# Sabarna07-tech/Multimodal-RAG-for-Image-Text-Search

Measured on NVIDIA B200. Metric: queries/sec, exact top-10 over 10Mx512 bf16 (flat cosine scan + top-k), higher is better.
Workload: dtype bf16

## Files before the change

include/mmr_b200.h:

```cpp
#ifndef MMR_B200_H_
#define MMR_B200_H_

#include <stddef.h>
#include <stdint.h>

#ifdef __cplusplus
extern "C" {
#endif

#define MMR_ABI_VERSION 2

enum mmr_status {
  MMR_OK = 0,
  MMR_ERR_INVALID = 1,
  MMR_ERR_CUDA = 2,
  MMR_ERR_UNSUPPORTED = 3,
  MMR_ERR_WORKSPACE = 4
};

enum mmr_dtype {
  MMR_BF16 = 0,
  MMR_F32 = 1,
  MMR_F16 = 2
};

enum mmr_query_precision {
  MMR_QP_AUTO = 0,
  MMR_QP_F32 = 1,
  MMR_QP_RESCORE = 2
};

#define MMR_MAX_K 64

typedef struct mmr_index mmr_index;

int mmr_abi_version(void);
const char* mmr_last_error(void);
int mmr_set_option(const char* name, const char* value);
int mmr_get_option(const char* name);

int mmr_index_create(int device, int dim, int dtype, int64_t n_rows, const void* rows_dev,
                     const int64_t* seg_offsets_host, int32_t n_segments, int64_t row_base, mmr_index** out);
int mmr_index_destroy(mmr_index* index);
int mmr_index_set_query_precision(mmr_index* index, int mode);
int mmr_index_update(mmr_index* index, int64_t n_rows, const void* rows_dev, const int64_t* seg_offsets_host,
                     int32_t n_segments);

int mmr_convert_rows_f32(const float* src_dev, void* dst_dev, int dtype, int64_t n_rows, int dim, int normalize,
                         void* stream);
int mmr_load_rows_f32_host(int device, const float* src_host, void* dst_dev, int dtype, int64_t n_rows, int dim,
                           int normalize, void* stream);

int mmr_load_rows_f32_host_scatter(int device, const float* src_host, void* dst_dev, int dtype, int64_t n_rows, int dim,
                                   int normalize, const int64_t* dst_row_host, void* stream);
int mmr_hash_strings(const uint8_t* data, const int32_t* offsets, int64_t n, uint64_t* out);

size_t mmr_search_workspace_bytes(const mmr_index* index, int32_t B, int32_t k);
size_t mmr_search_ranges_workspace_bytes(const mmr_index* index, int32_t B, int32_t k, int64_t n_ranges);
int mmr_search(const mmr_index* index, const float* queries_dev, const int32_t* query_seg_host, int32_t B,
               int32_t k, float* out_scores_dev, int64_t* out_rows_dev, void* workspace_dev, size_t workspace_bytes,
               void* stream);
int mmr_search_ranges(const mmr_index* index, const float* queries_dev, int32_t B, int32_t k,
                      const int32_t* range_off_host, const int64_t* ranges_host, float* out_scores_dev,
                      int64_t* out_rows_dev, void* workspace_dev, size_t workspace_bytes, void* stream);
int mmr_search_host(mmr_index* index, const float* queries_host, const int32_t* query_seg_host, int32_t B,
                    int32_t k, float* out_scores_host, int64_t* out_rows_host, void* stream);

int mmr_merge_topk(const float* scores_dev, const int64_t* rows_dev, int32_t G, int32_t B, int32_t k,
                   float* out_scores_dev, int64_t* out_rows_dev, void* stream);
int mmr_merge_topk_strided(const float* scores_dev, const int64_t* rows_dev, int64_t score_shard_stride,
                           int64_t row_shard_stride, int32_t G, int32_t B, int32_t k, float* out_scores_dev,
                           int64_t* out_rows_dev, void* stream);

size_t mmr_exchange_buffer_bytes(int32_t G, int32_t B, int32_t k);
size_t mmr_search_exchange_workspace_bytes(const mmr_index* index, int32_t B, int32_t k);
int mmr_search_exchange(const mmr_index* index, const float* queries_dev, const int32_t* query_seg_host, int32_t B,
                        int32_t k, const uint64_t* peer_bufs_host, int32_t G, int32_t rank, uint32_t seq,
                        float* out_scores_dev, int64_t* out_rows_dev, void* workspace_dev, size_t workspace_bytes,
                        void* stream);

int mmr_search_exchange_host(mmr_index* index, const float* queries_host, const int32_t* query_seg_host, int32_t B,
                             int32_t k, const uint64_t* peer_bufs_host, int32_t G, int32_t rank, uint32_t seq,
                             float* out_scores_host, int64_t* out_rows_host, void* stream);

typedef struct mmr_multi mmr_multi;
int mmr_multi_create(mmr_index** shards, int32_t G, mmr_multi** out);
int mmr_multi_destroy(mmr_multi* multi);
int mmr_multi_search_host(mmr_multi* multi, const float* queries_host, int32_t B, int32_t k,
                          const int32_t* range_off_host, const int64_t* ranges_host, float* out_scores_host,
                          int64_t* out_rows_host);

int mmr_fuse(const float* text_scores_dev, const int64_t* text_rows_dev, int32_t kt, const float* img_scores_dev,
             const int64_t* img_rows_dev, int32_t ki, int32_t B, int32_t final_n, double tau,
             double* out_combined_dev, double* out_score_dev, int64_t* out_rows_dev, int8_t* out_modality_dev,
             uint8_t* out_low_conf_dev, void* stream);

int mmr_fuse_f64(const double* text_scores_dev, const int32_t* text_count_dev, const double* text_rerank_dev,
                 const int32_t* rerank_count_dev, const double* img_scores_dev, const int32_t* img_count_dev,
                 int32_t kt, int32_t ki, int32_t B, int32_t final_n, double tau, double* out_combined_dev,
                 int32_t* out_index_dev, uint8_t* out_low_conf_dev, void* stream);

enum mmr_encoder_kind { MMR_ENC_MINILM = 0, MMR_ENC_CLIP_TEXT = 1, MMR_ENC_CROSS = 2 };
typedef struct mmr_encoder_config {
  int32_t kind;
  int32_t vocab_size;
  int32_t hidden;
  int32_t layers;
  int32_t heads;
  int32_t intermediate;
  int32_t max_positions;
  int32_t type_vocab;
  int32_t proj_dim;
  int32_t eos_token_id;
  float ln_eps;
} mmr_encoder_config;
typedef struct mmr_encoder mmr_encoder;
int mmr_encoder_create(int device, const mmr_encoder_config* config, mmr_encoder** out);
int mmr_encoder_destroy(mmr_encoder* encoder);
int mmr_encoder_out_dim(const mmr_encoder* encoder);
int mmr_encoder_set_weight(mmr_encoder* encoder, const char* name, const float* data_dev, int64_t numel, void* stream);
int mmr_encoder_forward(mmr_encoder* encoder, const int32_t* input_ids_host, const int32_t* attention_mask_host,
                        const int32_t* token_type_host, int32_t B, int32_t S, float* out_dev, void* stream);

int mmr_debug_umma_scores(const mmr_index* index, const float* queries_dev, int32_t B, int64_t row_begin,
                          int64_t row_end, float* out_scores_dev, int64_t out_ld, void* workspace_dev,
                          size_t workspace_bytes, void* stream);

int64_t mmr_launch_count(void);
int mmr_device_sm_count(int device, int* out_sms);
int mmr_last_kernel(void);
int64_t mmr_rescore_reruns(void);

#ifdef __cplusplus
}
#endif
#endif
```

multimodal-rag-for-image-text-search_b200/_native.py:

```python
from __future__ import annotations

import ctypes as C
import os
from typing import Optional

HERE = os.path.dirname(os.path.abspath(__file__))
LIB_PATH = os.environ.get("MMR_LIB_PATH") or os.path.join(HERE, "libmmr_b200.so")

MMR_OK = 0
MMR_BF16, MMR_F32, MMR_F16 = 0, 1, 2
MMR_MAX_K = 64
ABI_VERSION = 2
MMR_QP_AUTO, MMR_QP_F32, MMR_QP_RESCORE = 0, 1, 2

_i32, _i64, _sz, _p, _f64 = C.c_int32, C.c_int64, C.c_size_t, C.c_void_p, C.c_double
SYMBOLS = [
    ("mmr_abi_version", C.c_int, []),
    ("mmr_last_error", C.c_char_p, []),
    ("mmr_set_option", C.c_int, [C.c_char_p, C.c_char_p]),
    ("mmr_get_option", C.c_int, [C.c_char_p]),
    ("mmr_index_set_query_precision", C.c_int, [_p, C.c_int]),
    ("mmr_search_ranges_workspace_bytes", _sz, [_p, _i32, _i32, _i64]),
    ("mmr_search_exchange_host", C.c_int, [_p, _p, _p, _i32, _i32, _p, _i32, _i32, C.c_uint32, _p, _p, _p]),
    ("mmr_index_create", C.c_int, [C.c_int, C.c_int, C.c_int, _i64, _p, _p, _i32, _i64, C.POINTER(_p)]),
    ("mmr_index_destroy", C.c_int, [_p]),
    ("mmr_index_update", C.c_int, [_p, _i64, _p, _p, _i32]),
    ("mmr_convert_rows_f32", C.c_int, [_p, _p, C.c_int, _i64, C.c_int, C.c_int, _p]),
    ("mmr_load_rows_f32_host", C.c_int, [C.c_int, _p, _p, C.c_int, _i64, C.c_int, C.c_int, _p]),
    ("mmr_load_rows_f32_host_scatter", C.c_int, [C.c_int, _p, _p, C.c_int, _i64, C.c_int, C.c_int, _p, _p]),
    ("mmr_hash_strings", C.c_int, [_p, _p, _i64, _p]),
    ("mmr_search_workspace_bytes", _sz, [_p, _i32, _i32]),
    ("mmr_search", C.c_int, [_p, _p, _p, _i32, _i32, _p, _p, _p, _sz, _p]),
    ("mmr_search_ranges", C.c_int, [_p, _p, _i32, _i32, _p, _p, _p, _p, _p, _sz, _p]),
    ("mmr_search_host", C.c_int, [_p, _p, _p, _i32, _i32, _p, _p, _p]),
    ("mmr_merge_topk", C.c_int, [_p, _p, _i32, _i32, _i32, _p, _p, _p]),
    ("mmr_merge_topk_strided", C.c_int, [_p, _p, _i64, _i64, _i32, _i32, _i32, _p, _p, _p]),
    ("mmr_exchange_buffer_bytes", _sz, [_i32, _i32, _i32]),
    ("mmr_search_exchange_workspace_bytes", _sz, [_p, _i32, _i32]),
    ("mmr_search_exchange", C.c_int, [_p, _p, _p, _i32, _i32, _p, _i32, _i32, C.c_uint32, _p, _p, _p, _sz, _p]),
    ("mmr_multi_create", C.c_int, [_p, _i32, C.POINTER(_p)]),
    ("mmr_multi_destroy", C.c_int, [_p]),
    ("mmr_multi_search_host", C.c_int, [_p, _p, _i32, _i32, _p, _p, _p, _p]),
    ("mmr_encoder_create", C.c_int, [C.c_int, _p, C.POINTER(_p)]),
    ("mmr_encoder_destroy", C.c_int, [_p]),
    ("mmr_encoder_out_dim", C.c_int, [_p]),
    ("mmr_encoder_set_weight", C.c_int, [_p, C.c_char_p, _p, _i64, _p]),
    ("mmr_encoder_forward", C.c_int, [_p, _p, _p, _p, _i32, _i32, _p, _p]),
    ("mmr_fuse", C.c_int, [_p, _p, _i32, _p, _p, _i32, _i32, _i32, _f64, _p, _p, _p, _p, _p, _p]),
    ("mmr_fuse_f64", C.c_int, [_p, _p, _p, _p, _p, _p, _i32, _i32, _i32, _i32, _f64, _p, _p, _p, _p]),
    ("mmr_debug_umma_scores", C.c_int, [_p, _p, _i32, _i64, _i64, _p, _i64, _p, _sz, _p]),
    ("mmr_launch_count", _i64, []),
    ("mmr_device_sm_count", C.c_int, [C.c_int, C.POINTER(C.c_int)]),
    ("mmr_last_kernel", C.c_int, []),
    ("mmr_rescore_reruns", _i64, []),
]


MMR_ENC_MINILM, MMR_ENC_CLIP_TEXT, MMR_ENC_CROSS = 0, 1, 2


class EncoderConfig(C.Structure):
    _fields_ = [("kind", _i32), ("vocab_size", _i32), ("hidden", _i32), ("layers", _i32), ("heads", _i32),
                ("intermediate", _i32), ("max_positions", _i32), ("type_vocab", _i32), ("proj_dim", _i32),
                ("eos_token_id", _i32), ("ln_eps", C.c_float)]


class NativeError(RuntimeError):
    """Raised for every non-zero status from the C ABI (propagates like the reference's search errors,
    app/storage/lancedb_store.py:103-123 has no try/except)."""


_lib: Optional[C.CDLL] = None


def lib() -> C.CDLL:
    global _lib
    if _lib is None:
        if not os.path.exists(LIB_PATH):
            raise NativeError(
                f"{LIB_PATH} is missing. Build it with `python -c 'import __graft_entry__ as g; g.build()'` "
                "(nvcc, sm_100a). This package has no CPU or eager fallback."
            )
        handle = C.CDLL(LIB_PATH)
        for name, res, args in SYMBOLS:
            fn = getattr(handle, name)
            fn.restype = res
            fn.argtypes = args
        if handle.mmr_abi_version() != ABI_VERSION:
            raise NativeError(f"ABI version mismatch: library {handle.mmr_abi_version()} != binding {ABI_VERSION}")
        _lib = handle
    return _lib


def check(status: int) -> None:
    if status != MMR_OK:
        msg = lib().mmr_last_error()
        raise NativeError(f"mmr status {status}: {msg.decode() if msg else '?'}")


def set_option(name: str, value) -> None:
    check(lib().mmr_set_option(name.encode(), None if value is None else str(value).encode()))


def get_option(name: str) -> int:
    return int(lib().mmr_get_option(name.encode()))
```

multimodal-rag-for-image-text-search_b200/csrc/aux_kernels.cuh:

```cuda
#pragma once
#include "common.cuh"
#include "topk.cuh"

namespace mmr {

template <typename E>
__device__ __forceinline__ E cast_elem(float x);
template <>
__device__ __forceinline__ __nv_bfloat16 cast_elem<__nv_bfloat16>(float x) { return __float2bfloat16_rn(x); }
template <>
__device__ __forceinline__ __half cast_elem<__half>(float x) { return __float2half_rn(x); }
template <>
__device__ __forceinline__ float cast_elem<float>(float x) { return x; }

template <typename E>
__global__ void convert_rows_kernel(const float* __restrict__ src, E* __restrict__ dst, int64_t n_rows, int dim,
                                    int normalize, const int64_t* __restrict__ dst_row = nullptr) {
  const int lane = threadIdx.x & 31;
  const int64_t warps = int64_t(gridDim.x) * (blockDim.x >> 5);
  for (int64_t row = int64_t(blockIdx.x) * (blockDim.x >> 5) + (threadIdx.x >> 5); row < n_rows; row += warps) {
    const int64_t drow = dst_row ? dst_row[row] : row;
    if (drow < 0) continue;
    const float* s = src + row * dim;
    E* d = dst + drow * dim;
    float inv = 1.f;
    bool scale = false;
    if (normalize) {
      float ss = 0.f;
      for (int i = lane; i < dim; i += 32) {
        const float x = s[i];
        ss = fmaf(x, x, ss);
      }
      ss = warp_allreduce_sum(ss);
      const float nrm = sqrtf(ss);
      scale = nrm > 0.f;
      inv = nrm;
    }
    for (int i = lane; i < dim; i += 32) {
      const float x = s[i];
      d[i] = cast_elem<E>(scale ? x / inv : x);
    }
  }
}

template <int KPL>
__global__ void merge_shards_kernel(const float* __restrict__ scores, const int64_t* __restrict__ rows,
                                    int64_t score_stride, int64_t row_stride, int G, int B, int k,
                                    float* __restrict__ out_scores, int64_t* __restrict__ out_rows) {
  const int lane = threadIdx.x & 31;
  const int qi = blockIdx.x * (blockDim.x >> 5) + (threadIdx.x >> 5);
  if (qi >= B) return;
  WarpTopK<KPL> m;
  m.clear();
  uint64_t thr = 0ull;
  const int per = k;
  const int total = G * per;
  for (int i0 = 0; i0 < total; i0 += 32) {
    const int i = i0 + lane;
    bool valid = i < total;
    uint64_t key = 0ull;
    if (valid) {
      const int g = i / per, j = i % per;
      const size_t o = size_t(qi) * k + j;
      const int64_t r = rows[size_t(g) * row_stride + o];
      valid = r >= 0;
      if (valid) key = make_key(scores[size_t(g) * score_stride + o], uint32_t(r));
    }
    thr = m.offer_batch(key, valid, thr, k, lane);
  }
#pragma unroll
  for (int j = 0; j < KPL; ++j) {
    const int pos = j * 32 + lane;
    if (pos < k) {
      const uint64_t key = m.key[j];
      out_scores[size_t(qi) * k + pos] = key ? key_score(key) : -INFINITY;
      out_rows[size_t(qi) * k + pos] = key ? int64_t(key_row(key)) : int64_t(-1);
    }
  }
}

constexpr int MMR_XCHG_MAX_PEERS = 16;
constexpr int MMR_XCHG_HEADER = 256;

struct PeerPtrs {
  uint64_t slot[MMR_XCHG_MAX_PEERS];
  uint64_t flag[MMR_XCHG_MAX_PEERS];
};

__global__ void push_wire_kernel(const uint8_t* __restrict__ wire, uint32_t wire_bytes, const PeerPtrs peers, uint32_t seq) {
  const int g = blockIdx.x;
  const uint64_t* peer_slot = peers.slot;
  const uint64_t* peer_flag = peers.flag;
  const uint4* src = reinterpret_cast<const uint4*>(wire);
  uint4* dst = reinterpret_cast<uint4*>(peer_slot[g]);
  const uint32_t n16 = wire_bytes / 16;
  for (uint32_t i = threadIdx.x; i < n16; i += blockDim.x) dst[i] = src[i];
  for (uint32_t i = n16 * 16 + threadIdx.x; i < wire_bytes; i += blockDim.x)
    reinterpret_cast<uint8_t*>(peer_slot[g])[i] = wire[i];
  __threadfence_system();
  __syncthreads();
  if (threadIdx.x == 0) asm volatile("st.release.sys.global.u32 [%0], %1;" ::"l"(peer_flag[g]), "r"(seq) : "memory");
}

__device__ __forceinline__ uint32_t ld_acquire_sys_u32(const uint32_t* p) {
  uint32_t v;
  asm volatile("ld.acquire.sys.global.u32 %0, [%1];" : "=r"(v) : "l"(p) : "memory");
  return v;
}
__device__ __forceinline__ uint64_t globaltimer_ns() {
  uint64_t t;
  asm volatile("mov.u64 %0, %%globaltimer;" : "=l"(t));
  return t;
}

template <int KPL>
__device__ __forceinline__ void merge_wait_body(const uint8_t* __restrict__ xbuf, int parity, uint32_t seq,
                                                uint32_t wire_bytes, uint32_t score_bytes, int G, int B, int k,
                                                float* __restrict__ out_scores, int64_t* __restrict__ out_rows,
                                                uint64_t timeout_ns, int qi, int lane);

template <int KPL>
__global__ void merge_wait_kernel(const uint8_t* __restrict__ xbuf, int parity, uint32_t seq, uint32_t wire_bytes,
                                  uint32_t score_bytes, int G, int B, int k, float* __restrict__ out_scores,
                                  int64_t* __restrict__ out_rows, uint64_t timeout_ns, uint32_t* done_flag,
                                  uint32_t done_seq) {
  const int lane = threadIdx.x & 31;
  const int qi = blockIdx.x * (blockDim.x >> 5) + (threadIdx.x >> 5);
  asm volatile("griddepcontrol.launch_dependents;" ::: "memory");
  if (done_flag != nullptr) {
    merge_wait_body<KPL>(xbuf, parity, seq, wire_bytes, score_bytes, G, B, k, out_scores, out_rows, timeout_ns, qi, lane);
    __threadfence_system();
    __syncthreads();
    if (threadIdx.x == 0) asm volatile("st.release.sys.global.u32 [%0], %1;" ::"l"(done_flag), "r"(done_seq) : "memory");
    return;
  }
  merge_wait_body<KPL>(xbuf, parity, seq, wire_bytes, score_bytes, G, B, k, out_scores, out_rows, timeout_ns, qi, lane);
}

template <int KPL>
__device__ __forceinline__ void merge_wait_body(const uint8_t* __restrict__ xbuf, int parity, uint32_t seq,
                                                uint32_t wire_bytes, uint32_t score_bytes, int G, int B, int k,
                                                float* __restrict__ out_scores, int64_t* __restrict__ out_rows,
                                                uint64_t timeout_ns, int qi, int lane) {
  if (qi >= B) return;
  const uint32_t* flags = reinterpret_cast<const uint32_t*>(xbuf) + parity * MMR_XCHG_MAX_PEERS;
  bool ok = true;
  if (lane < G) {
    const uint64_t t0 = globaltimer_ns();
    while (ld_acquire_sys_u32(flags + lane) < seq) {
      if (globaltimer_ns() - t0 > timeout_ns) {
        ok = false;
        break;
      }
    }
  }
  ok = __all_sync(0xffffffffu, ok);
  if (!ok) {
    if (lane == 0) {
      out_rows[size_t(qi) * k] = -2;
      out_scores[size_t(qi) * k] = -INFINITY;
    }
    return;
  }
  const uint8_t* slots = xbuf + MMR_XCHG_HEADER + size_t(parity) * G * wire_bytes;
  WarpTopK<KPL> m;
  m.clear();
  uint64_t thr = 0ull;
  const int total = G * k;
  for (int i0 = 0; i0 < total; i0 += 32) {
    const int i = i0 + lane;
    bool valid = i < total;
    uint64_t key = 0ull;
    if (valid) {
      const int g = i / k, j = i % k;
      const uint8_t* slot = slots + size_t(g) * wire_bytes;
      const size_t o = size_t(qi) * k + j;
      const long long r = __ldcg(reinterpret_cast<const long long*>(slot + score_bytes) + o);
      valid = r >= 0;
      if (valid) key = make_key(__ldcg(reinterpret_cast<const float*>(slot) + o), uint32_t(r));
    }
    thr = m.offer_batch(key, valid, thr, k, lane);
  }
#pragma unroll
  for (int j = 0; j < KPL; ++j) {
    const int pos = j * 32 + lane;
    if (pos < k) {
      const uint64_t key = m.key[j];
      out_scores[size_t(qi) * k + pos] = key ? key_score(key) : -INFINITY;
      out_rows[size_t(qi) * k + pos] = key ? int64_t(key_row(key)) : int64_t(-1);
    }
  }
}

__device__ __forceinline__ float np_pairwise_sum_f32(const float* a, int n) {
  if (n < 8) {
    float res = 0.f;
    for (int i = 0; i < n; ++i) res = __fadd_rn(res, a[i]);
    return res;
  }
  float r[8];
#pragma unroll
  for (int j = 0; j < 8; ++j) r[j] = a[j];
  int i = 8;
  const int lim = n - (n % 8);
  for (; i < lim; i += 8) {
#pragma unroll
    for (int j = 0; j < 8; ++j) r[j] = __fadd_rn(r[j], a[i + j]);
  }
  float res = __fadd_rn(__fadd_rn(__fadd_rn(r[0], r[1]), __fadd_rn(r[2], r[3])),
                        __fadd_rn(__fadd_rn(r[4], r[5]), __fadd_rn(r[6], r[7])));
  for (; i < n; ++i) res = __fadd_rn(res, a[i]);
  return res;
}

constexpr int FUSE_MAXK = 64;

__device__ __forceinline__ void np_z_scores(const float* cos, int n, double* v, double* z) {
  float arr[FUSE_MAXK], sq[FUSE_MAXK];
  for (int i = 0; i < n; ++i) {
    const float d = __fsub_rn(1.0f, cos[i]);
    v[i] = __dsub_rn(1.0, double(d));
    arr[i] = __double2float_rn(v[i]);
  }
  const float fn = float(n);
  const float mean = __fdiv_rn(np_pairwise_sum_f32(arr, n), fn);
  for (int i = 0; i < n; ++i) {
    const float x = __fsub_rn(arr[i], mean);
    sq[i] = __fmul_rn(x, x);
  }
  const float var = __fdiv_rn(np_pairwise_sum_f32(sq, n), fn);
  const float sd = __fsqrt_rn(var);
  if (sd == 0.f) {
    for (int i = 0; i < n; ++i) z[i] = 0.0;
  } else {
    const double dm = double(mean), ds = double(sd);
    for (int i = 0; i < n; ++i) z[i] = __ddiv_rn(__dsub_rn(v[i], dm), ds);
  }
}

__device__ __forceinline__ void np_z_scores_f64(const double* v, int n, double* z) {
  float arr[FUSE_MAXK], sq[FUSE_MAXK];
  for (int i = 0; i < n; ++i) arr[i] = __double2float_rn(v[i]);
  const float fn = float(n);
  const float mean = __fdiv_rn(np_pairwise_sum_f32(arr, n), fn);
  for (int i = 0; i < n; ++i) {
    const float x = __fsub_rn(arr[i], mean);
    sq[i] = __fmul_rn(x, x);
  }
  const float sd = __fsqrt_rn(__fdiv_rn(np_pairwise_sum_f32(sq, n), fn));
  if (sd == 0.f) {
    for (int i = 0; i < n; ++i) z[i] = 0.0;
  } else {
    const double dm = double(mean), ds = double(sd);
    for (int i = 0; i < n; ++i) z[i] = __ddiv_rn(__dsub_rn(v[i], dm), ds);
  }
}

__device__ __forceinline__ void stable_desc_order(const double* key, int n, int* idx) {
  for (int i = 0; i < n; ++i) {
    int j = i;
    while (j > 0 && key[idx[j - 1]] < key[i]) {
      idx[j] = idx[j - 1];
      --j;
    }
    idx[j] = i;
  }
}

__global__ void fuse_full_kernel(const double* __restrict__ text_scores, const int32_t* __restrict__ text_count,
                                 const double* __restrict__ rerank, const int32_t* __restrict__ rr_count,
                                 const double* __restrict__ img_scores, const int32_t* __restrict__ img_count, int kt,
                                 int ki, int B, int final_n, double tau, double* __restrict__ out_combined,
                                 int32_t* __restrict__ out_index, uint8_t* __restrict__ out_low_conf) {
  const int b = blockIdx.x * blockDim.x + threadIdx.x;
  if (b >= B) return;
  const int nt = text_count ? min(text_count[b], kt) : 0;
  const int ni = img_count ? min(img_count[b], ki) : 0;
  const int nr = (rr_count && rerank) ? min(rr_count[b], nt) : 0;
  double key[FUSE_MAXK], v[FUSE_MAXK], z[FUSE_MAXK], rr[FUSE_MAXK], zr[FUSE_MAXK];
  double comb[2 * FUSE_MAXK];
  int order[FUSE_MAXK], src[2 * FUSE_MAXK], fin[2 * FUSE_MAXK];
  for (int j = 0; j < nt; ++j) {
    key[j] = j < nr ? rerank[size_t(b) * kt + j] : text_scores[size_t(b) * kt + j];
    order[j] = j;
  }
  if (nr > 0) stable_desc_order(key, nt, order);
  int nrr = 0;
  for (int j = 0; j < nt; ++j) {
    v[j] = text_scores[size_t(b) * kt + order[j]];
    if (order[j] < nr) rr[nrr++] = rerank[size_t(b) * kt + order[j]];
  }
  if (nt) np_z_scores_f64(v, nt, z);
  if (nrr) np_z_scores_f64(rr, nrr, zr);
  for (int j = 0; j < nt; ++j) {
    comb[j] = j < nrr ? __ddiv_rn(__dadd_rn(__dadd_rn(0.0, z[j]), zr[j]), 2.0) : __ddiv_rn(__dadd_rn(0.0, z[j]), 1.0);
    src[j] = order[j];
  }
  if (ni) {
    for (int j = 0; j < ni; ++j) v[j] = img_scores[size_t(b) * ki + j];
    np_z_scores_f64(v, ni, z);
    for (int j = 0; j < ni; ++j) {
      comb[nt + j] = z[j];
      src[nt + j] = kt + j;
    }
  }
  const int n = nt + ni;
  stable_desc_order(comb, n, fin);
  for (int o = 0; o < final_n; ++o) {
    const size_t oo = size_t(b) * final_n + o;
    out_combined[oo] = o < n ? comb[fin[o]] : 0.0;
    out_index[oo] = o < n ? src[fin[o]] : -1;
  }
  out_low_conf[b] = (n == 0 || final_n <= 0) ? 1 : (comb[fin[0]] < tau ? 1 : 0);
}

__global__ void fuse_kernel(const float* __restrict__ text_scores, const int64_t* __restrict__ text_rows, int kt,
                            const float* __restrict__ img_scores, const int64_t* __restrict__ img_rows, int ki, int B,
                            int final_n, double tau, double* __restrict__ out_combined,
                            double* __restrict__ out_score, int64_t* __restrict__ out_rows,
                            int8_t* __restrict__ out_modality, uint8_t* __restrict__ out_low_conf) {
  const int qi = blockIdx.x * blockDim.x + threadIdx.x;
  if (qi >= B) return;
  double v[2 * FUSE_MAXK], z[2 * FUSE_MAXK];
  int nt = 0, ni = 0;
  if (text_rows) {
    while (nt < kt && text_rows[size_t(qi) * kt + nt] >= 0) ++nt;
  }
  if (img_rows) {
    while (ni < ki && img_rows[size_t(qi) * ki + ni] >= 0) ++ni;
  }
  if (nt) np_z_scores(text_scores + size_t(qi) * kt, nt, v, z);
  if (ni) np_z_scores(img_scores + size_t(qi) * ki, ni, v + nt, z + nt);
  const int n = nt + ni;
  unsigned long long taken_lo = 0ull, taken_hi = 0ull;
  double best0 = 0.0;
  for (int o = 0; o < final_n; ++o) {
    int bi = -1;
    double bz = 0.0;
    for (int i = 0; i < n; ++i) {
      const bool taken = i < 64 ? ((taken_lo >> i) & 1ull) : ((taken_hi >> (i - 64)) & 1ull);
      if (taken) continue;
      if (bi < 0 || z[i] > bz) {
        bi = i;
        bz = z[i];
      }
    }
    const size_t oo = size_t(qi) * final_n + o;
// ... 20 lines not shown
```

multimodal-rag-for-image-text-search_b200/csrc/common.cuh:

```cuda
#pragma once
#include <cuda_runtime.h>
#include <cuda_bf16.h>
#include <cuda_fp16.h>
#include <stdint.h>

namespace mmr {

__host__ __device__ __forceinline__ uint32_t f32_orderable(float f) {
#ifdef __CUDA_ARCH__
  uint32_t u = __float_as_uint(f + 0.0f);
#else
  f = f + 0.0f;
  uint32_t u;
  memcpy(&u, &f, 4);
#endif
  return u ^ ((u >> 31) ? 0xFFFFFFFFu : 0x80000000u);
}
__host__ __device__ __forceinline__ float f32_from_orderable(uint32_t o) {
  uint32_t u = o ^ ((o >> 31) ? 0x80000000u : 0xFFFFFFFFu);
#ifdef __CUDA_ARCH__
  return __uint_as_float(u);
#else
  float f;
  memcpy(&f, &u, 4);
  return f;
#endif
}
__host__ __device__ __forceinline__ uint64_t make_key(float score, uint32_t row) {
  return (uint64_t(f32_orderable(score)) << 32) | uint64_t(0xFFFFFFFFu - row);
}
__host__ __device__ __forceinline__ float key_score(uint64_t key) { return f32_from_orderable(uint32_t(key >> 32)); }
__host__ __device__ __forceinline__ uint32_t key_row(uint64_t key) { return 0xFFFFFFFFu - uint32_t(key); }

struct Options {
  int pdl = 0;
  int umma_mode = 0;
  int umma_pair = 1;
  int umma_noprobe = 0;
  int umma_stages = 0;
  int force_family = 0;
  int umma_lockstep = 0;
  int umma_fused_probe = 0;
  int umma_skip_epi = 0;
  int enc_fuse_ln = 0;
  int enc_att_mma = 1;
  int enc_gemm_smem_kb = 100;
  int enc_narrow_tiles = 1;
  int inline_query = 1;
  int mailbox = 0;
};
inline Options& options() {
  static Options o;
  return o;
}

#ifdef __CUDACC__
__device__ __forceinline__ uint64_t shfl_u64(uint64_t v, int src) {
  uint32_t lo = __shfl_sync(0xffffffffu, uint32_t(v), src);
  uint32_t hi = __shfl_sync(0xffffffffu, uint32_t(v >> 32), src);
  return (uint64_t(hi) << 32) | lo;
}
__device__ __forceinline__ uint64_t shfl_u64_xor(uint64_t v, int mask) {
  uint32_t lo = __shfl_xor_sync(0xffffffffu, uint32_t(v), mask);
  uint32_t hi = __shfl_xor_sync(0xffffffffu, uint32_t(v >> 32), mask);
  return (uint64_t(hi) << 32) | lo;
}
__device__ __forceinline__ uint64_t shfl_up_u64(uint64_t v, int d) {
  uint32_t lo = __shfl_up_sync(0xffffffffu, uint32_t(v), d);
  uint32_t hi = __shfl_up_sync(0xffffffffu, uint32_t(v >> 32), d);
  return (uint64_t(hi) << 32) | lo;
}
__device__ __forceinline__ float warp_allreduce_sum(float v) {
#pragma unroll
  for (int o = 16; o > 0; o >>= 1) v += __shfl_xor_sync(0xffffffffu, v, o);
  return v;
}

__device__ __forceinline__ uint32_t smem_u32(const void* p) { return uint32_t(__cvta_generic_to_shared(p)); }

__device__ __forceinline__ void mbar_init(uint32_t bar, uint32_t count) {
  asm volatile("mbarrier.init.shared::cta.b64 [%0], %1;" ::"r"(bar), "r"(count) : "memory");
}
__device__ __forceinline__ void fence_mbar_init() {
  asm volatile("fence.mbarrier_init.release.cluster;" ::: "memory");
}
__device__ __forceinline__ void fence_proxy_async() {
  asm volatile("fence.proxy.async.shared::cta;" ::: "memory");
}
__device__ __forceinline__ void mbar_arrive_expect_tx(uint32_t bar, uint32_t bytes) {
  asm volatile("mbarrier.arrive.expect_tx.shared::cta.b64 _, [%0], %1;" ::"r"(bar), "r"(bytes) : "memory");
}
__device__ __forceinline__ void mbar_arrive(uint32_t bar) {
  asm volatile("mbarrier.arrive.shared::cta.b64 _, [%0];" ::"r"(bar) : "memory");
}
__device__ __forceinline__ bool mbar_try_wait(uint32_t bar, uint32_t parity) {
  uint32_t ok;
  asm volatile(
      "{\n\t.reg .pred p;\n\t"
      "mbarrier.try_wait.parity.shared::cta.b64 p, [%1], %2;\n\t"
      "selp.b32 %0, 1, 0, p;\n\t}"
      : "=r"(ok)
      : "r"(bar), "r"(parity)
      : "memory");
  return ok != 0;
}
__device__ __forceinline__ void mbar_wait(uint32_t bar, uint32_t parity) {
  while (!mbar_try_wait(bar, parity)) {
  }
}
__device__ __forceinline__ void bulk_g2s(uint32_t dst_smem, const void* src, uint32_t bytes, uint32_t bar) {
  asm volatile("cp.async.bulk.shared::cluster.global.mbarrier::complete_tx::bytes [%0], [%1], %2, [%3];" ::"r"(dst_smem),
               "l"(src), "r"(bytes), "r"(bar)
               : "memory");
}
__device__ __forceinline__ uint64_t l2_policy_evict_first() {
  uint64_t pol;
  asm volatile("createpolicy.fractional.L2::evict_first.b64 %0, 1.0;" : "=l"(pol));
  return pol;
}
__device__ __forceinline__ uint64_t l2_policy_evict_last() {
  uint64_t pol;
  asm volatile("createpolicy.fractional.L2::evict_last.b64 %0, 1.0;" : "=l"(pol));
  return pol;
}
__device__ __forceinline__ void bulk_g2s_hint(uint32_t dst_smem, const void* src, uint32_t bytes, uint32_t bar,
                                              uint64_t policy) {
  asm volatile(
      "cp.async.bulk.shared::cluster.global.mbarrier::complete_tx::bytes.L2::cache_hint [%0], [%1], %2, [%3], %4;" ::"r"(
          dst_smem),
      "l"(src), "r"(bytes), "r"(bar), "l"(policy)
      : "memory");
}

__device__ __forceinline__ void lds_v4(uint32_t addr, uint32_t (&r)[4]) {
  asm volatile("ld.shared.v4.u32 {%0,%1,%2,%3}, [%4];" : "=r"(r[0]), "=r"(r[1]), "=r"(r[2]), "=r"(r[3]) : "r"(addr));
}
__device__ __forceinline__ void lds_v2(uint32_t addr, uint32_t (&r)[2]) {
  asm volatile("ld.shared.v2.u32 {%0,%1}, [%2];" : "=r"(r[0]), "=r"(r[1]) : "r"(addr));
}
__device__ __forceinline__ void pdl_chain_prologue() {
  asm volatile("griddepcontrol.launch_dependents;" ::: "memory");
  asm volatile("griddepcontrol.wait;" ::: "memory");
}

__device__ __forceinline__ void pdl_launch_dependents() { asm volatile("griddepcontrol.launch_dependents;" ::: "memory"); }
__device__ __forceinline__ void pdl_wait_prior_grid() { asm volatile("griddepcontrol.wait;" ::: "memory"); }

template <typename... KArgs, typename... Args>
inline cudaError_t launch_pdl(void (*kernel)(KArgs...), dim3 grid, dim3 block, size_t smem, cudaStream_t st, Args&&... args) {
  cudaLaunchConfig_t cfg = {};
  cfg.gridDim = grid;
  cfg.blockDim = block;
  cfg.dynamicSmemBytes = smem;
  cfg.stream = st;
  cudaLaunchAttribute attr[1];
  attr[0].id = cudaLaunchAttributeProgrammaticStreamSerialization;
  attr[0].val.programmaticStreamSerializationAllowed = 1;
  cfg.attrs = attr;
  cfg.numAttrs = 1;
  return cudaLaunchKernelEx(&cfg, kernel, static_cast<KArgs>(args)...);
}
#endif

}
```

multimodal-rag-for-image-text-search_b200/csrc/mmr_b200.cu:

```cuda
#include "abi_common.h"

#include <algorithm>
#include <atomic>
#include <chrono>
#include <cstdarg>
#include <cstdio>
#include <cstdlib>
#include <cstring>
#include <condition_variable>
#include <map>
#include <mutex>
#include <string>
#include <thread>
#include <vector>
#if defined(__x86_64__)
#include <immintrin.h>
#endif

#include "aux_kernels.cuh"
#include "common.cuh"
#include "scan_stream.cuh"
#ifdef MMR_WITH_UMMA
#include "scan_umma2.cuh"
#endif

using namespace mmr;

thread_local std::string mmr_g_err;
std::atomic<int64_t> mmr_g_launches{0};
static thread_local int g_last_kernel = 0;
static std::atomic<int64_t> g_rescore_reruns{0};
#define g_err mmr_g_err
#define g_launches mmr_g_launches
#define fail mmr_fail

int mmr_fail(int code, const char* fmt, ...) {
  char buf[512];
  va_list ap;
  va_start(ap, fmt);
  vsnprintf(buf, sizeof(buf), fmt, ap);
  va_end(ap);
  mmr_g_err = buf;
  return code;
}

struct mmr_index {
  int device = 0;
  int dim = 0;
  int dtype = MMR_BF16;
  int64_t n_rows = 0;
  const void* rows = nullptr;
  int64_t row_base = 0;
  std::vector<int64_t> seg;
  int sm_count = 0;
  int query_precision = MMR_QP_AUTO;
  mutable uint8_t* h_flags = nullptr;
  mutable int flags_cap = 0;
  std::mutex host_mu;
  float* h_q = nullptr;
  float* d_q = nullptr;
  uint8_t* h_box = nullptr;
  uint8_t* d_box = nullptr;
  uint32_t box_seq = 0;
  void* d_ws = nullptr;
  size_t ws_bytes = 0;
  int cap_b = 0, cap_k = 0;
#ifdef MMR_WITH_UMMA
  mutable UmmaIndexState umma;
  mutable Umma2IndexState umma2;
#endif
};

static int elem_bytes(int dtype) { return dtype == MMR_F32 ? 4 : 2; }

static int set_segments(mmr_index* ix, const int64_t* seg, int32_t nseg) {
  ix->seg.clear();
  if (seg == nullptr || nseg <= 0) {
    ix->seg = {0, ix->n_rows};
    return MMR_OK;
  }
  ix->seg.assign(seg, seg + nseg + 1);
  if (ix->seg.front() < 0 || ix->seg.back() > ix->n_rows) return fail(MMR_ERR_INVALID, "segment offsets out of range");
  for (int i = 0; i < nseg; ++i)
    if (ix->seg[i] > ix->seg[i + 1]) return fail(MMR_ERR_INVALID, "segment offsets must be ascending");
  return MMR_OK;
}

static int* option_slot(const char* name) {
  Options& o = options();
  if (!name) return nullptr;
  if (!strcmp(name, "MMR_PDL")) return &o.pdl;
  if (!strcmp(name, "MMR_UMMA_MODE")) return &o.umma_mode;
  if (!strcmp(name, "MMR_UMMA_PAIR")) return &o.umma_pair;
  if (!strcmp(name, "MMR_UMMA_NOPROBE")) return &o.umma_noprobe;
  if (!strcmp(name, "MMR_FORCE_FAMILY")) return &o.force_family;
  if (!strcmp(name, "MMR_UMMA_LOCKSTEP")) return &o.umma_lockstep;
  if (!strcmp(name, "MMR_UMMA_SKIP_EPI")) return &o.umma_skip_epi;
  if (!strcmp(name, "MMR_UMMA_FUSED_PROBE")) return &o.umma_fused_probe;
  if (!strcmp(name, "MMR_UMMA_STAGES")) return &o.umma_stages;
  if (!strcmp(name, "MMR_ENC_FUSE_LN")) return &o.enc_fuse_ln;
  if (!strcmp(name, "MMR_ENC_ATT_MMA")) return &o.enc_att_mma;
  if (!strcmp(name, "MMR_ENC_GEMM_SMEM_KB")) return &o.enc_gemm_smem_kb;
  if (!strcmp(name, "MMR_ENC_NARROW_TILES")) return &o.enc_narrow_tiles;
  if (!strcmp(name, "MMR_INLINE_QUERY")) return &o.inline_query;
  if (!strcmp(name, "MMR_MAILBOX")) return &o.mailbox;
  return nullptr;
}
static int parse_option(const char* name, const char* v, int dflt) {
  if (!v || !v[0]) return dflt;
  if (!strcmp(name, "MMR_UMMA_MODE")) return v[0] == 's' ? 1 : (v[0] == 't' ? 2 : 0);
  return atoi(v);
}
static const char* kOptionNames[] = {"MMR_PDL", "MMR_UMMA_MODE", "MMR_UMMA_PAIR", "MMR_UMMA_NOPROBE", "MMR_FORCE_FAMILY",
                                     "MMR_UMMA_LOCKSTEP", "MMR_INLINE_QUERY", "MMR_MAILBOX", "MMR_UMMA_SKIP_EPI", "MMR_UMMA_FUSED_PROBE", "MMR_ENC_FUSE_LN", "MMR_ENC_ATT_MMA", "MMR_ENC_GEMM_SMEM_KB", "MMR_UMMA_STAGES", "MMR_ENC_NARROW_TILES"};
namespace {
struct OptionsFromEnv {
  OptionsFromEnv() {
    for (const char* name : kOptionNames) {
      int* slot = option_slot(name);
      *slot = parse_option(name, getenv(name), *slot);
    }
  }
} g_options_from_env;
}

extern "C" int mmr_set_option(const char* name, const char* value) {
  int* slot = option_slot(name);
  if (!slot) return fail(MMR_ERR_INVALID, "unknown option %s", name ? name : "(null)");
  Options defaults;
  Options& o = options();
  const int dflt = *(reinterpret_cast<int*>(&defaults) + (slot - reinterpret_cast<int*>(&o)));
  *slot = parse_option(name, value, dflt);
  return MMR_OK;
}
extern "C" int mmr_get_option(const char* name) {
  int* slot = option_slot(name);
  return slot ? *slot : -1;
}

extern "C" int mmr_abi_version(void) { return MMR_ABI_VERSION; }
extern "C" const char* mmr_last_error(void) { return g_err.c_str(); }
extern "C" int64_t mmr_launch_count(void) { return g_launches.load(); }
extern "C" int mmr_last_kernel(void) { return g_last_kernel; }
extern "C" int64_t mmr_rescore_reruns(void) { return g_rescore_reruns.load(); }

extern "C" int mmr_device_sm_count(int device, int* out_sms) {
  if (!out_sms) return fail(MMR_ERR_INVALID, "out_sms is NULL");
  CUDA_TRY(cudaDeviceGetAttribute(out_sms, cudaDevAttrMultiProcessorCount, device));
  return MMR_OK;
}

extern "C" int mmr_index_create(int device, int dim, int dtype, int64_t n_rows, const void* rows_dev,
                                const int64_t* seg_offsets_host, int32_t n_segments, int64_t row_base,
                                mmr_index** out) {
  if (!out) return fail(MMR_ERR_INVALID, "out is NULL");
  *out = nullptr;
  if (dtype != MMR_BF16 && dtype != MMR_F32 && dtype != MMR_F16) return fail(MMR_ERR_INVALID, "unknown dtype %d", dtype);
  if (dim <= 0 || n_rows < 0) return fail(MMR_ERR_INVALID, "bad shape [%lld, %d]", (long long)n_rows, dim);
  if (n_rows >= (int64_t(1) << 32)) return fail(MMR_ERR_UNSUPPORTED, "at most 2^32-1 rows per resident index");
  if (n_rows > 0 && rows_dev == nullptr) return fail(MMR_ERR_INVALID, "rows_dev is NULL");
  if ((reinterpret_cast<uintptr_t>(rows_dev) & 15) != 0) return fail(MMR_ERR_INVALID, "rows_dev must be 16-byte aligned");
  if (dim != 384 && dim != 512)
    return fail(MMR_ERR_UNSUPPORTED, "dim %d: kernels are built for 384 (MiniLM) and 512 (CLIP)", dim);
  int major = 0, minor = 0, sms = 0;
  CUDA_TRY(cudaDeviceGetAttribute(&major, cudaDevAttrComputeCapabilityMajor, device));
  CUDA_TRY(cudaDeviceGetAttribute(&minor, cudaDevAttrComputeCapabilityMinor, device));
  CUDA_TRY(cudaDeviceGetAttribute(&sms, cudaDevAttrMultiProcessorCount, device));
  if (major != 10) return fail(MMR_ERR_CUDA, "device %d is sm_%d%d; this library is sm_100a only", device, major, minor);
  mmr_index* ix = new mmr_index();
  ix->device = device;
  ix->dim = dim;
  ix->dtype = dtype;
  ix->n_rows = n_rows;
  ix->rows = rows_dev;
  ix->row_base = row_base;
  ix->sm_count = sms;
  int rc = set_segments(ix, seg_offsets_host, n_segments);
  if (rc != MMR_OK) {
    delete ix;
    return rc;
  }
  *out = ix;
  return MMR_OK;
}

extern "C" int mmr_index_update(mmr_index* ix, int64_t n_rows, const void* rows_dev, const int64_t* seg, int32_t nseg) {
  if (!ix) return fail(MMR_ERR_INVALID, "index is NULL");
  if (n_rows < 0 || n_rows >= (int64_t(1) << 32)) return fail(MMR_ERR_INVALID, "bad n_rows");
  if (n_rows > 0 && rows_dev == nullptr) return fail(MMR_ERR_INVALID, "rows_dev is NULL");
  if ((reinterpret_cast<uintptr_t>(rows_dev) & 15) != 0) return fail(MMR_ERR_INVALID, "rows_dev must be 16-byte aligned");
  ix->n_rows = n_rows;
  ix->rows = rows_dev;
#ifdef MMR_WITH_UMMA
  ix->umma.valid = false;
  ix->umma2.valid = false;
#endif
  return set_segments(ix, seg, nseg);
}

static void free_staging(mmr_index* ix) {
  if (ix->h_flags) cudaFreeHost(ix->h_flags);
  ix->h_flags = nullptr;
  ix->flags_cap = 0;
  if (ix->h_q) cudaFreeHost(ix->h_q);
  if (ix->h_box) cudaFreeHost(ix->h_box);
  if (ix->d_q) cudaFree(ix->d_q);
  if (ix->d_ws) cudaFree(ix->d_ws);
  ix->h_q = ix->d_q = nullptr;
  ix->h_box = ix->d_box = nullptr;
  ix->d_ws = nullptr;
  ix->cap_b = ix->cap_k = 0;
}

extern "C" int mmr_index_destroy(mmr_index* ix) {
  if (!ix) return MMR_OK;
  cudaSetDevice(ix->device);
  free_staging(ix);
  delete ix;
  return MMR_OK;
}

extern "C" int mmr_index_set_query_precision(mmr_index* ix, int mode) {
  if (!ix) return fail(MMR_ERR_INVALID, "index is NULL");
  if (mode != MMR_QP_AUTO && mode != MMR_QP_F32 && mode != MMR_QP_RESCORE)
    return fail(MMR_ERR_INVALID, "unknown query precision %d", mode);
  ix->query_precision = mode;
  return MMR_OK;
}

template <typename E>
static int launch_convert(const float* src, void* dst, int64_t n, int dim, int normalize, cudaStream_t st,
                          const int64_t* dst_row = nullptr) {
  if (n == 0) return MMR_OK;
  const int threads = 256;
  const int64_t blocks = std::min<int64_t>((n + 7) / 8, 148 * 16);
  convert_rows_kernel<E><<<(unsigned)blocks, threads, 0, st>>>(src, reinterpret_cast<E*>(dst), n, dim, normalize, dst_row);
  g_launches++;
  CUDA_TRY(cudaGetLastError());
  return MMR_OK;
}

static int convert_dispatch(const float* src_dev, void* dst_dev, int dtype, int64_t n_rows, int dim, int normalize,
                            cudaStream_t st, const int64_t* dst_row_dev) {
  switch (dtype) {
    case MMR_BF16: return launch_convert<__nv_bfloat16>(src_dev, dst_dev, n_rows, dim, normalize, st, dst_row_dev);
    case MMR_F16: return launch_convert<__half>(src_dev, dst_dev, n_rows, dim, normalize, st, dst_row_dev);
    case MMR_F32: return launch_convert<float>(src_dev, dst_dev, n_rows, dim, normalize, st, dst_row_dev);
  }
  return fail(MMR_ERR_INVALID, "unknown dtype %d", dtype);
}

extern "C" int mmr_convert_rows_f32(const float* src_dev, void* dst_dev, int dtype, int64_t n_rows, int dim,
                                    int normalize, void* stream) {
  if (n_rows < 0 || dim <= 0) return fail(MMR_ERR_INVALID, "bad shape");
  if (n_rows > 0 && (!src_dev || !dst_dev)) return fail(MMR_ERR_INVALID, "NULL buffer");
  return convert_dispatch(src_dev, dst_dev, dtype, n_rows, dim, normalize, static_cast<cudaStream_t>(stream), nullptr);
}

static void parallel_memcpy(void* dst, const void* src, size_t bytes, int threads) {
  if (threads <= 1 || bytes < (size_t(4) << 20)) {
    memcpy(dst, src, bytes);
    return;
  }
  std::vector<std::thread> pool;
  const size_t per = (bytes / threads + 4095) / 4096 * 4096;
  for (int t = 0; t < threads; ++t) {
    const size_t o = size_t(t) * per;
    if (o >= bytes) break;
    const size_t len = std::min(per, bytes - o);
    pool.emplace_back([=]() { memcpy(static_cast<uint8_t*>(dst) + o, static_cast<const uint8_t*>(src) + o, len); });
  }
  for (auto& th : pool) th.join();
}

extern "C" int mmr_load_rows_f32_host_scatter(int device, const float* src_host, void* dst_dev, int dtype, int64_t n_rows,
                                              int dim, int normalize, const int64_t* dst_row_host, void* stream) {
  if (n_rows < 0 || dim <= 0) return fail(MMR_ERR_INVALID, "bad shape");
  if (n_rows == 0) return MMR_OK;
  if (!src_host || !dst_dev) return fail(MMR_ERR_INVALID, "NULL buffer");
  if (dtype != MMR_BF16 && dtype != MMR_F32 && dtype != MMR_F16) return fail(MMR_ERR_INVALID, "unknown dtype %d", dtype);
  CUDA_TRY(cudaSetDevice(device));
  cudaStream_t st = static_cast<cudaStream_t>(stream);
  const int64_t chunk_rows = std::max<int64_t>(1, (int64_t(64) << 20) / (int64_t(dim) * 4));
  const size_t chunk_bytes = size_t(chunk_rows) * dim * 4;
  const size_t map_bytes = dst_row_host ? size_t(chunk_rows) * 8 : 0;
  uint8_t* h[2] = {nullptr, nullptr};
  uint8_t* d[2] = {nullptr, nullptr};
  cudaEvent_t done[2] = {nullptr, nullptr};
  int rc = MMR_OK;
  auto cleanup = [&]() {
    for (int i = 0; i < 2; ++i) {
      if (h[i]) cudaFreeHost(h[i]);
      if (d[i]) cudaFree(d[i]);
      if (done[i]) cudaEventDestroy(done[i]);
    }
  };
  for (int i = 0; i < 2; ++i) {
    if (cudaMallocHost(&h[i], chunk_bytes + map_bytes) != cudaSuccess ||
        cudaMalloc(&d[i], chunk_bytes + map_bytes) != cudaSuccess ||
        cudaEventCreateWithFlags(&done[i], cudaEventDisableTiming) != cudaSuccess) {
      cleanup();
      return fail(MMR_ERR_CUDA, "staging allocation of %zu bytes failed", chunk_bytes + map_bytes);
    }
  }
  const int threads = int(std::min<unsigned>(8u, std::max(1u, std::thread::hardware_concurrency() / 2)));
  int slot = 0;
  for (int64_t r0 = 0; r0 < n_rows && rc == MMR_OK; r0 += chunk_rows, slot ^= 1) {
    const int64_t nr = std::min(chunk_rows, n_rows - r0);
    const size_t bytes = size_t(nr) * dim * 4;
    cudaEventSynchronize(done[slot]);
    parallel_memcpy(h[slot], src_host + r0 * dim, bytes, threads);
    if (dst_row_host) memcpy(h[slot] + chunk_bytes, dst_row_host + r0, size_t(nr) * 8);
    const size_t copy_bytes = dst_row_host ? chunk_bytes + size_t(nr) * 8 : bytes;
    if (cudaMemcpyAsync(d[slot], h[slot], copy_bytes, cudaMemcpyHostToDevice, st) != cudaSuccess) {
      rc = fail(MMR_ERR_CUDA, "H2D copy failed");
      break;
    }
    const int64_t* map_dev = dst_row_host ? reinterpret_cast<const int64_t*>(d[slot] + chunk_bytes) : nullptr;
    const int eb = elem_bytes(dtype);
    void* dst = dst_row_host ? dst_dev : static_cast<void*>(static_cast<uint8_t*>(dst_dev) + size_t(r0) * dim * eb);
    rc = convert_dispatch(reinterpret_cast<const float*>(d[slot]), dst, dtype, nr, dim, normalize, st, map_dev);
    cudaEventRecord(done[slot], st);
  }
  cudaStreamSynchronize(st);
  cleanup();
  return rc;
}

extern "C" int mmr_load_rows_f32_host(int device, const float* src_host, void* dst_dev, int dtype, int64_t n_rows,
                                      int dim, int normalize, void* stream) {
  return mmr_load_rows_f32_host_scatter(device, src_host, dst_dev, dtype, n_rows, dim, normalize, nullptr, stream);
}

extern "C" int mmr_hash_strings(const uint8_t* data, const int32_t* offsets, int64_t n, uint64_t* out) {
  if (n < 0 || (n > 0 && (!offsets || !out))) return fail(MMR_ERR_INVALID, "bad arguments");
  for (int64_t i = 0; i < n; ++i) {
    const uint8_t* p = data + offsets[i];
    const int32_t len = offsets[i + 1] - offsets[i];
    uint64_t h = 0xcbf29ce484222325ull ^ (uint64_t(uint32_t(len)) * 0x9E3779B97F4A7C15ull);
    int32_t j = 0;
    for (; j + 8 <= len; j += 8) {
      uint64_t w;
      memcpy(&w, p + j, 8);
      h = (h ^ w) * 0x100000001b3ull;
      h ^= h >> 29;
    }
    uint64_t tail = 0;
    if (j < len) memcpy(&tail, p + j, size_t(len - j));
    h = (h ^ tail) * 0x100000001b3ull;
    h ^= h >> 32;
    h *= 0xff51afd7ed558ccdull;
    h ^= h >> 33;
    h *= 0xc4ceb9fe1a85ec53ull;
    h ^= h >> 33;
    out[i] = h;
  }
  return MMR_OK;
}

template <typename E, int D, int NQ, int KPL>
static int launch_stream_t(const StreamParams& p, int grid, cudaStream_t st) {
  using C = StreamCfg<E, D, NQ, KPL>;
  static bool attr_set[64] = {};
  int dev = 0;
  cudaGetDevice(&dev);
  if (dev >= 0 && dev < 64 && !attr_set[dev]) {
    CUDA_TRY(cudaFuncSetAttribute(scan_stream_kernel<E, D, NQ, KPL>, cudaFuncAttributeMaxDynamicSharedMemorySize,
                                  C::SMEM_BYTES));
    attr_set[dev] = true;
  }
  cudaLaunchConfig_t cfg = {};
  cfg.gridDim = dim3(grid);
  cfg.blockDim = dim3(C::THREADS);
  cfg.dynamicSmemBytes = C::SMEM_BYTES;
  cfg.stream = st;
  cudaLaunchAttribute attr[1];
  attr[0].id = cudaLaunchAttributeProgrammaticStreamSerialization;
  attr[0].val.programmaticStreamSerializationAllowed = (p.items == nullptr && options().pdl) ? 1 : 0;
  cfg.attrs = attr;
  cfg.numAttrs = 1;
  CUDA_TRY(cudaLaunchKernelEx(&cfg, scan_stream_kernel<E, D, NQ, KPL>, p));
  g_launches++;
  return MMR_OK;
}

template <typename E, int D>
static int launch_stream_ed(const StreamParams& p, int nq_pad, int kpl, int grid, cudaStream_t st) {
#define MMR_CASE(NQ_, KPL_) \
  if (nq_pad == NQ_ && kpl == KPL_) return launch_stream_t<E, D, NQ_, KPL_>(p, grid, st);
  MMR_CASE(1, 1) MMR_CASE(1, 2) MMR_CASE(2, 1) MMR_CASE(2, 2) MMR_CASE(4, 1) MMR_CASE(4, 2)
  if constexpr (sizeof(E) == 4) {
    MMR_CASE(8, 1) MMR_CASE(8, 2)
  }
#undef MMR_CASE
  return fail(MMR_ERR_UNSUPPORTED, "no stream kernel for nq=%d kpl=%d", nq_pad, kpl);
}

static int launch_stream(const mmr_index* ix, const StreamParams& p, int nq_pad, int kpl, int grid, cudaStream_t st) {
  const int key = ix->dtype * 1000 + ix->dim;
  switch (key) {
    case MMR_BF16 * 1000 + 512: return launch_stream_ed<__nv_bfloat16, 512>(p, nq_pad, kpl, grid, st);
    case MMR_BF16 * 1000 + 384: return launch_stream_ed<__nv_bfloat16, 384>(p, nq_pad, kpl, grid, st);
    case MMR_F16 * 1000 + 512: return launch_stream_ed<__half, 512>(p, nq_pad, kpl, grid, st);
    case MMR_F16 * 1000 + 384: return launch_stream_ed<__half, 384>(p, nq_pad, kpl, grid, st);
    case MMR_F32 * 1000 + 512: return launch_stream_ed<float, 512>(p, nq_pad, kpl, grid, st);
    case MMR_F32 * 1000 + 384: return launch_stream_ed<float, 384>(p, nq_pad, kpl, grid, st);
  }
  return fail(MMR_ERR_UNSUPPORTED, "no stream kernel for dtype %d dim %d", ix->dtype, ix->dim);
}

static constexpr size_t WS_CTRL = 256;
#ifndef MMR_VARLEN_ITEMS_PER_CTA
#define MMR_VARLEN_ITEMS_PER_CTA 8
#endif
static constexpr int VARLEN_ITEMS_PER_CTA = MMR_VARLEN_ITEMS_PER_CTA;
static constexpr int RANGES_PER_QUERY_BUDGET = 8;

static size_t align_up(size_t v, size_t a) { return (v + a - 1) / a * a; }

static int64_t varlen_item_cap(const mmr_index* ix, int64_t n_ranges) {
  return int64_t(ix->sm_count) * VARLEN_ITEMS_PER_CTA + n_ranges + 64;
}

static size_t rescore_extra_bytes(int B) {
  return align_up(size_t(B) * MMR_MAX_K * 4, 256) + align_up(size_t(B) * MMR_MAX_K * 8, 256) + align_up(size_t(B) * 4, 256) +
         align_up(size_t(B), 256);
}
static size_t k2_slice_bytes(const mmr_index* ix, int B) {
#ifdef MMR_WITH_UMMA
  return umma_workspace_bytes(ix->sm_count, ix->dim, B, MMR_MAX_K) + rescore_extra_bytes(B);
#else
  return 0;
#endif
}

static size_t workspace_bytes_for(const mmr_index* ix, int32_t B, int32_t k, int64_t n_ranges) {
  if (!ix || B <= 0 || k <= 0) return 0;
  const size_t kk = size_t(std::min<int32_t>(k, MMR_MAX_K));
  const size_t uniform = size_t(ix->sm_count) * 8 * kk * 8;
  const size_t items = size_t(varlen_item_cap(ix, n_ranges));
  const size_t varlen = align_up(items * K1_ITEM_NQ * kk * 8, 256) + align_up(items * sizeof(ScanItem), 256) +
                        align_up(size_t(B) * sizeof(QuerySlot), 256);
  size_t total = WS_CTRL + align_up(std::max(uniform, varlen), 256);
  total += k2_slice_bytes(ix, B);
  return total;
}

extern "C" size_t mmr_search_workspace_bytes(const mmr_index* ix, int32_t B, int32_t k) {
  return workspace_bytes_for(ix, B, k, int64_t(RANGES_PER_QUERY_BUDGET) * std::max(B, 0));
}
extern "C" size_t mmr_search_ranges_workspace_bytes(const mmr_index* ix, int32_t B, int32_t k, int64_t n_ranges) {
  return workspace_bytes_for(ix, B, k, std::max<int64_t>(n_ranges, 0));
}

struct ExchangeInfo {
  int n_peers = 0;
  uint32_t seq = 0;
  uint32_t wire_score_bytes = 0;
  uint64_t slot[MMR_MAX_PEERS] = {};
  uint64_t flag[MMR_MAX_PEERS] = {};
};

struct QuerySrc {
  const float* dev = nullptr;
  const float* host = nullptr;
};
struct Completion {
  uint32_t* flag_dev = nullptr;
  uint32_t seq = 0;
  bool armed = false;
};

static int k1_group(const mmr_index* ix) { return ix->dtype == MMR_F32 ? 8 : 4; }

static bool can_inline(const mmr_index* ix, int B) {
  return options().inline_query && B * ix->dim <= K1_INLINE_FLOATS && B <= 2;
}

static int search_uniform_stream(const mmr_index* ix, QuerySrc q, int B, int k, uint32_t r0, uint32_t r1,
                                 float* out_s, int64_t* out_r, uint8_t* ws, cudaStream_t st,
                                 const ExchangeInfo* xi = nullptr, Completion* done = nullptr) {
  const int kpl = k <= 32 ? 1 : 2;
  const int R = MMR_K1_ROWS;
  const int64_t nchunks = (int64_t(r1) - r0 + R - 1) / R;
  int grid = int(std::min<int64_t>(ix->sm_count, std::max<int64_t>(1, (nchunks + K1_NW - 1) / K1_NW)));
  const int group = k1_group(ix);
  if (q.dev == nullptr && !(q.host && can_inline(ix, B))) return fail(MMR_ERR_INVALID, "queries must be device-resident for this batch size");
  for (int q0 = 0; q0 < B; q0 += group) {
    const int nq = std::min(group, B - q0);
    const int nq_pad = nq <= 2 ? nq : (nq <= 4 ? 4 : 8);
    StreamParams p;
    memset(&p, 0, offsetof(StreamParams, qinline));
    p.rows = ix->rows;
    p.queries = q.dev;
    if (q.dev == nullptr) memcpy(p.qinline, q.host, size_t(B) * ix->dim * sizeof(float));
    p.q_first = q0;
    p.nq = nq;
    p.k = k;
    p.row_begin = r0;
    p.row_end = r1;
    p.partial = reinterpret_cast<uint64_t*>(ws + WS_CTRL);
    p.ticket = reinterpret_cast<unsigned int*>(ws);
    p.out_scores = out_s;
    p.out_rows = out_r;
    p.row_base = ix->row_base;
    if (B <= group) {
      if (xi) {
        p.n_peers = xi->n_peers;
        p.seq = xi->seq;
        p.wire_score_bytes = xi->wire_score_bytes;
        for (int g = 0; g < xi->n_peers; ++g) {
          p.peer_slot[g] = xi->slot[g];
          p.peer_flag[g] = xi->flag[g];
        }
      }
      if (done && done->flag_dev && options().mailbox) {
        p.done_flag = done->flag_dev;
        p.done_seq = done->seq;
        done->armed = true;
      }
    }
    int rc = launch_stream(ix, p, nq_pad, kpl, grid, st);
    if (rc != MMR_OK) return rc;
  }
  g_last_kernel = 1;
  return MMR_OK;
}

typedef std::vector<std::pair<uint32_t, uint32_t>> RangeList;

static int search_varlen_stream(const mmr_index* ix, const float* q, const std::vector<RangeList>& ranges, int k,
                                float* out_s, int64_t* out_r, uint8_t* ws, size_t ws_bytes, cudaStream_t st) {
  const int B = int(ranges.size());
  const int kpl = k <= 32 ? 1 : 2;
  const int R = MMR_K1_ROWS;
  std::map<RangeList, int> tenant_of;
  std::vector<std::vector<int>> members;
  std::vector<const RangeList*> tenant_ranges;
  for (int b = 0; b < B; ++b) {
    auto it = tenant_of.find(ranges[b]);
    if (it == tenant_of.end()) {
      it = tenant_of.emplace(ranges[b], int(members.size())).first;
      members.emplace_back();
      tenant_ranges.push_back(&it->first);
    }
    members[it->second].push_back(b);
  }
  int64_t total_rows = 0, n_group_ranges = 0;
  for (size_t t = 0; t < members.size(); ++t) {
    const int64_t ngroups = (int64_t(members[t].size()) + K1_ITEM_NQ - 1) / K1_ITEM_NQ;
    for (auto& r : *tenant_ranges[t]) total_rows += (int64_t(r.second) - r.first) * ngroups;
    n_group_ranges += int64_t(tenant_ranges[t]->size()) * ngroups;
  }
  const int64_t target = int64_t(ix->sm_count) * VARLEN_ITEMS_PER_CTA;
  int64_t item_rows = std::max<int64_t>(64 * K1_NW, (total_rows + target - 1) / target);
  item_rows = (item_rows + R - 1) / R * R;
  constexpr int N_CLS = 3;
  static const int cls_nq[N_CLS] = {1, 2, K1_ITEM_NQ};
  std::vector<ScanItem> cls_items[N_CLS];
  std::vector<QuerySlot> slots(B);
  std::vector<int> slot_cls(B, 0);
  cls_items[0].reserve(size_t(std::min<int64_t>(target + n_group_ranges, 1 << 22)));
  for (size_t t = 0; t < members.size(); ++t) {
    const std::vector<int>& m = members[t];
    for (size_t g0 = 0; g0 < m.size(); g0 += K1_ITEM_NQ) {
      const int nq = int(std::min<size_t>(K1_ITEM_NQ, m.size() - g0));
      const int cls = nq == 1 ? 0 : nq == 2 ? 1 : 2;
      std::vector<ScanItem>& dst = cls_items[cls];
      const int item0 = int(dst.size());
      for (auto& r : *tenant_ranges[t]) {
        for (int64_t s = r.first; s < int64_t(r.second); s += item_rows) {
          ScanItem it;
          it.row_begin = uint32_t(s);
          it.row_end = uint32_t(std::min<int64_t>(s + item_rows, r.second));
          for (int j = 0; j < K1_ITEM_NQ; ++j) it.query[j] = m[g0 + std::min(j, nq - 1)];
          it.nq = nq;
          it.out = int(dst.size());
          dst.push_back(it);
        }
      }
      for (int j = 0; j < nq; ++j) {
        slots[m[g0 + j]] = QuerySlot{item0, int(dst.size()) - item0, j, 0};
        slot_cls[m[g0 + j]] = cls;
      }
    }
  }
  int cls_first[N_CLS + 1] = {0};
  for (int c = 0; c < N_CLS; ++c) cls_first[c + 1] = cls_first[c] + int(cls_items[c].size());
  for (int b = 0; b < B; ++b) slots[b].item0 += cls_first[slot_cls[b]];
  auto by_size = [](const ScanItem& a, const ScanItem& b) { return a.row_end - a.row_begin > b.row_end - b.row_begin; };
  std::vector<ScanItem> items;
  items.reserve(size_t(cls_first[N_CLS]));
  for (int c = 0; c < N_CLS; ++c) {
    for (auto& it : cls_items[c]) it.out += cls_first[c];
    std::stable_sort(cls_items[c].begin(), cls_items[c].end(), by_size);
    items.insert(items.end(), cls_items[c].begin(), cls_items[c].end());
  }
  const int n_items = int(items.size());
  const size_t part_bytes = align_up(size_t(std::max(n_items, 1)) * K1_ITEM_NQ * k * 8, 256);
  const size_t item_bytes = align_up(size_t(std::max(n_items, 1)) * sizeof(ScanItem), 256);
  const size_t slot_bytes = align_up(size_t(B) * sizeof(QuerySlot), 256);
  const size_t k2_bytes = k2_slice_bytes(ix, B);
  if (WS_CTRL + part_bytes + item_bytes + slot_bytes + k2_bytes > ws_bytes)
    return fail(MMR_ERR_WORKSPACE,
                "workspace too small for %d work items over %lld row ranges: size it with "
                "mmr_search_ranges_workspace_bytes(index, B, k, n_ranges)", n_items, (long long)n_group_ranges);
  uint64_t* d_part = reinterpret_cast<uint64_t*>(ws + WS_CTRL);
  ScanItem* d_items = reinterpret_cast<ScanItem*>(ws + WS_CTRL + part_bytes);
  QuerySlot* d_slots = reinterpret_cast<QuerySlot*>(ws + WS_CTRL + part_bytes + item_bytes);
  if (n_items > 0) CUDA_TRY(cudaMemcpyAsync(d_items, items.data(), size_t(n_items) * sizeof(ScanItem), cudaMemcpyHostToDevice, st));
  CUDA_TRY(cudaMemcpyAsync(d_slots, slots.data(), size_t(B) * sizeof(QuerySlot), cudaMemcpyHostToDevice, st));
  for (int cls = 0; cls < N_CLS; ++cls) {
    const int first = cls_first[cls];
    const int count = cls_first[cls + 1] - first;
    if (count <= 0) continue;
    const int nq_launch = cls_nq[cls];
    StreamParams p;
    memset(&p, 0, offsetof(StreamParams, qinline));
    p.rows = ix->rows;
    p.queries = q;
    p.nq = nq_launch;
    p.k = k;
    p.partial = d_part;
    p.ticket = reinterpret_cast<unsigned int*>(ws);
    p.row_base = ix->row_base;
    p.items = d_items + first;
    p.n_items = count;
    p.item_nq = K1_ITEM_NQ;
    const int grid = int(std::min<int64_t>(ix->sm_count, count));
    int rc = launch_stream(ix, p, nq_launch, kpl, grid, st);
    if (rc != MMR_OK) return rc;
  }
  const int wpb = 4;
  if (kpl == 1)
    merge_items_kernel<1><<<(B + wpb - 1) / wpb, wpb * 32, 0, st>>>(d_part, d_slots, B, K1_ITEM_NQ, k, out_s, out_r, ix->row_base);
  else
    merge_items_kernel<2><<<(B + wpb - 1) / wpb, wpb * 32, 0, st>>>(d_part, d_slots, B, K1_ITEM_NQ, k, out_s, out_r, ix->row_base);
  g_launches++;
  CUDA_TRY(cudaGetLastError());
  g_last_kernel = 3;
  return MMR_OK;
}

#ifdef MMR_WITH_UMMA
template <typename E, int D>
static void launch_rescore_ed(const mmr_index* ix, const float* q, const float* cs, const int64_t* cr, const float* qerr, int B,
                              int kc, int k, float* out_s, int64_t* out_r, uint8_t* flags, cudaStream_t st) {
  if (k <= 32)
    rescore_kernel<E, D, 1><<<B, 256, 0, st>>>(ix->rows, q, cs, cr, qerr, kc, k, ix->row_base, out_s, out_r, flags);
  else
    rescore_kernel<E, D, 2><<<B, 256, 0, st>>>(ix->rows, q, cs, cr, qerr, kc, k, ix->row_base, out_s, out_r, flags);
}

static int search_rescored(const mmr_index* ix, const float* q, int B, int k, uint32_t r0, uint32_t r1, float* out_s,
                           int64_t* out_r, uint8_t* ws, size_t ws_total, cudaStream_t st) {
  const int kc = k <= 16 ? 32 : MMR_MAX_K;
  uint8_t* slice = ws + ws_total - k2_slice_bytes(ix, B);
  uint8_t* extra = slice + umma_workspace_bytes(ix->sm_count, ix->dim, B, MMR_MAX_K);
  float* cand_s = reinterpret_cast<float*>(extra);
  int64_t* cand_r = reinterpret_cast<int64_t*>(extra + align_up(size_t(B) * MMR_MAX_K * 4, 256));
  float* qerr = reinterpret_cast<float*>(reinterpret_cast<uint8_t*>(cand_r) + align_up(size_t(B) * MMR_MAX_K * 8, 256));
  uint8_t* flags = reinterpret_cast<uint8_t*>(qerr) + align_up(size_t(B) * 4, 256);
  int rc = umma_search(ix->umma, ix->umma2, ix->rows, ix->n_rows, ix->dim, ix->dtype, ix->sm_count, q, B, kc, r0, r1,
                       ix->row_base, cand_s, cand_r, slice, st, g_err, nullptr, 0, qerr);
  if (rc != MMR_OK) return rc;
  g_launches += umma_launches_per_search();
  if (ix->dtype == MMR_BF16 && ix->dim == 512) launch_rescore_ed<__nv_bfloat16, 512>(ix, q, cand_s, cand_r, qerr, B, kc, k, out_s, out_r, flags, st);
  else if (ix->dtype == MMR_BF16) launch_rescore_ed<__nv_bfloat16, 384>(ix, q, cand_s, cand_r, qerr, B, kc, k, out_s, out_r, flags, st);
  else if (ix->dim == 512) launch_rescore_ed<__half, 512>(ix, q, cand_s, cand_r, qerr, B, kc, k, out_s, out_r, flags, st);
  else launch_rescore_ed<__half, 384>(ix, q, cand_s, cand_r, qerr, B, kc, k, out_s, out_r, flags, st);
  g_launches++;
  CUDA_TRY(cudaGetLastError());
  if (ix->flags_cap < B) {
    if (ix->h_flags) cudaFreeHost(ix->h_flags);
    ix->h_flags = nullptr;
    CUDA_TRY(cudaMallocHost(&ix->h_flags, size_t(std::max(B, 1024))));
    ix->flags_cap = std::max(B, 1024);
  }
  CUDA_TRY(cudaMemcpyAsync(ix->h_flags, flags, size_t(B), cudaMemcpyDeviceToHost, st));
  CUDA_TRY(cudaStreamSynchronize(st));
  g_last_kernel = 2;
  int reruns = 0;
  for (int b = 0; b < B; ++b) {
    if (ix->h_flags[b]) continue;
    QuerySrc one;
    one.dev = q + size_t(b) * ix->dim;
    rc = search_uniform_stream(ix, one, 1, k, r0, r1, out_s + size_t(b) * k, out_r + size_t(b) * k, ws, st);
    if (rc != MMR_OK) return rc;
    ++reruns;
  }
  g_last_kernel = 2;
  g_rescore_reruns += reruns;
  return MMR_OK;
}
#endif

static int search_uniform(const mmr_index* ix, QuerySrc q, int B, int k, uint32_t r0, uint32_t r1, float* out_s,
                          int64_t* out_r, uint8_t* ws, size_t ws_total, cudaStream_t st, const ExchangeInfo* xi = nullptr,
                          Completion* done = nullptr) {
#ifdef MMR_WITH_UMMA
  if (q.dev != nullptr && ix->query_precision != MMR_QP_F32 &&
      umma_preferred(ix->dtype, ix->dim, B, k, int64_t(r1) - r0)) {
    if (ix->query_precision == MMR_QP_RESCORE)
      return search_rescored(ix, q.dev, B, k, r0, r1, out_s, out_r, ws, ws_total, st);
    int rc = umma_search(ix->umma, ix->umma2, ix->rows, ix->n_rows, ix->dim, ix->dtype, ix->sm_count, q.dev, B, k, r0, r1,
                         ix->row_base, out_s, out_r, ws + ws_total - k2_slice_bytes(ix, B), st, g_err);
    if (rc == MMR_OK) {
      g_launches += umma_launches_per_search();
      g_last_kernel = 2;
    }
    return rc;
  }
#endif
  return search_uniform_stream(ix, q, B, k, r0, r1, out_s, out_r, ws, st, xi, done);
}

static bool uniform_takes_k2(const mmr_index* ix, int B, int k, int64_t nrows) {
#ifdef MMR_WITH_UMMA
  return ix->query_precision != MMR_QP_F32 && umma_preferred(ix->dtype, ix->dim, B, k, nrows);
#else
  return false;
#endif
}

static int check_search_args(const mmr_index* ix, int32_t B, int32_t k) {
  if (!ix) return fail(MMR_ERR_INVALID, "index is NULL");
  if (B <= 0) return fail(MMR_ERR_INVALID, "B must be >= 1");
  if (k < 1 || k > MMR_MAX_K) return fail(MMR_ERR_INVALID, "k must be in [1, %d]", MMR_MAX_K);
  return MMR_OK;
}

static int ranges_from_segments(const mmr_index* ix, const int32_t* query_seg_host, int B, std::vector<RangeList>& out,
                                bool& uniform) {
  const int nseg = int(ix->seg.size()) - 1;
  out.assign(B, RangeList(1));
  uniform = true;
  for (int b = 0; b < B; ++b) {
    const int s = query_seg_host ? query_seg_host[b] : -1;
    if (s < -1 || s >= nseg) return fail(MMR_ERR_INVALID, "query %d: segment %d out of range [0, %d)", b, s, nseg);
    out[b][0] = s < 0 ? std::make_pair(uint32_t(0), uint32_t(ix->n_rows))
                      : std::make_pair(uint32_t(ix->seg[s]), uint32_t(ix->seg[s + 1]));
    if (out[b][0] != out[0][0]) uniform = false;
  }
  return MMR_OK;
}

extern "C" int mmr_search(const mmr_index* ix, const float* queries_dev, const int32_t* query_seg_host, int32_t B,
                          int32_t k, float* out_scores_dev, int64_t* out_rows_dev, void* workspace_dev,
                          size_t workspace_bytes, void* stream) {
  int rc = check_search_args(ix, B, k);
  if (rc != MMR_OK) return rc;
  if (!queries_dev || !out_scores_dev || !out_rows_dev || !workspace_dev) return fail(MMR_ERR_INVALID, "NULL buffer");
  const size_t need = workspace_bytes_for(ix, B, k, B);
  if (workspace_bytes < need) return fail(MMR_ERR_WORKSPACE, "workspace too small");
  cudaStream_t st = static_cast<cudaStream_t>(stream);
  uint8_t* ws = static_cast<uint8_t*>(workspace_dev);
  std::vector<RangeList> ranges;
  bool uniform = true;
  rc = ranges_from_segments(ix, query_seg_host, B, ranges, uniform);
  if (rc != MMR_OK) return rc;
  QuerySrc q;
  q.dev = queries_dev;
  if (uniform)
    return search_uniform(ix, q, B, k, ranges[0][0].first, ranges[0][0].second, out_scores_dev, out_rows_dev, ws,
                          workspace_bytes, st);
  return search_varlen_stream(ix, queries_dev, ranges, k, out_scores_dev, out_rows_dev, ws, workspace_bytes, st);
}

static int parse_ranges(const mmr_index* ix, int B, const int32_t* range_off_host, const int64_t* ranges_host,
                        std::vector<RangeList>& per_query, bool& single_shared) {
  per_query.assign(B, RangeList());
  single_shared = true;
  for (int b = 0; b < B; ++b) {
    if (range_off_host[b + 1] < range_off_host[b]) return fail(MMR_ERR_INVALID, "range offsets must be ascending");
    for (int32_t r = range_off_host[b]; r < range_off_host[b + 1]; ++r) {
      const int64_t lo = ranges_host[2 * r], hi = ranges_host[2 * r + 1];
      if (lo < 0 || hi < lo || hi > ix->n_rows)
        return fail(MMR_ERR_INVALID, "query %d: bad row range [%lld, %lld)", b, (long long)lo, (long long)hi);
      if (hi > lo) per_query[b].push_back({uint32_t(lo), uint32_t(hi)});
    }
    RangeList sorted = per_query[b];
    std::sort(sorted.begin(), sorted.end());
    for (size_t i = 1; i < sorted.size(); ++i)
      if (sorted[i].first < sorted[i - 1].second)
        return fail(MMR_ERR_INVALID, "query %d: row ranges [%u, %u) and [%u, %u) overlap", b, sorted[i - 1].first,
                    sorted[i - 1].second, sorted[i].first, sorted[i].second);
    if (per_query[b].size() != 1 || per_query[b] != per_query[0]) single_shared = false;
  }
  return MMR_OK;
}

extern "C" int mmr_search_ranges(const mmr_index* ix, const float* queries_dev, int32_t B, int32_t k,
                                 const int32_t* range_off_host, const int64_t* ranges_host, float* out_scores_dev,
                                 int64_t* out_rows_dev, void* workspace_dev, size_t workspace_bytes, void* stream) {
  int rc = check_search_args(ix, B, k);
  if (rc != MMR_OK) return rc;
  if (!queries_dev || !range_off_host || !out_scores_dev || !out_rows_dev || !workspace_dev)
    return fail(MMR_ERR_INVALID, "NULL buffer");
  if (workspace_bytes < workspace_bytes_for(ix, B, k, 0)) return fail(MMR_ERR_WORKSPACE, "workspace too small");
  std::vector<RangeList> per_query;
  bool single_shared = true;
  rc = parse_ranges(ix, B, range_off_host, ranges_host, per_query, single_shared);
  if (rc != MMR_OK) return rc;
  cudaStream_t st = static_cast<cudaStream_t>(stream);
  uint8_t* ws = static_cast<uint8_t*>(workspace_dev);
  QuerySrc q;
  q.dev = queries_dev;
  if (single_shared)
    return search_uniform(ix, q, B, k, per_query[0][0].first, per_query[0][0].second, out_scores_dev, out_rows_dev, ws,
                          workspace_bytes, st);
  return search_varlen_stream(ix, queries_dev, per_query, k, out_scores_dev, out_rows_dev, ws, workspace_bytes, st);
}

static constexpr size_t BOX_HEADER = 64;
static size_t box_rows_off(int B, int k) { return BOX_HEADER + align_up(size_t(B) * k * 4, 16); }

static int ensure_staging(mmr_index* ix, int B, int k) {
  if (B <= ix->cap_b && k <= ix->cap_k) return MMR_OK;
  free_staging(ix);
  const int cb = std::max(B, 8), ck = std::max(k, 16);
  const size_t box_bytes = box_rows_off(cb, ck) + size_t(cb) * ck * 8;
  CUDA_TRY(cudaMallocHost(&ix->h_q, size_t(cb) * ix->dim * 4));
  CUDA_TRY(cudaMalloc(&ix->d_q, size_t(cb) * ix->dim * 4));
  CUDA_TRY(cudaHostAlloc(&ix->h_box, box_bytes, cudaHostAllocMapped));
  CUDA_TRY(cudaHostGetDevicePointer(reinterpret_cast<void**>(&ix->d_box), ix->h_box, 0));
  memset(ix->h_box, 0, box_bytes);
  ix->ws_bytes = workspace_bytes_for(ix, cb, ck, int64_t(RANGES_PER_QUERY_BUDGET) * cb);
  CUDA_TRY(cudaMalloc(&ix->d_ws, ix->ws_bytes));
  CUDA_TRY(cudaMemset(ix->d_ws, 0, ix->ws_bytes));
  ix->cap_b = cb;
  ix->cap_k = ck;
  return MMR_OK;
}

static inline void cpu_relax() {
#if defined(__x86_64__)
  _mm_pause();
#endif
}

static int wait_mailbox(mmr_index* ix, uint32_t seq, cudaStream_t st) {
  volatile uint32_t* flag = reinterpret_cast<volatile uint32_t*>(ix->h_box);
  for (uint64_t spins = 1;; ++spins) {
    if (*flag == seq) break;
    if ((spins & 4095) == 0) {
      cudaError_t e = cudaStreamQuery(st);
      if (e == cudaSuccess) {
        if (*flag == seq) break;
        return fail(MMR_ERR_CUDA, "search finished without ringing its mailbox");
      }
      if (e != cudaErrorNotReady) return fail(MMR_ERR_CUDA, "search failed: %s", cudaGetErrorString(e));
    }
    cpu_relax();
  }
  std::atomic_thread_fence(std::memory_order_acquire);
  return MMR_OK;
}

static int finish_host_call(mmr_index* ix, const Completion& done, int B, int k, float* out_scores_host,
                            int64_t* out_rows_host, cudaStream_t st) {
  if (done.armed) {
    int rc = wait_mailbox(ix, done.seq, st);
    if (rc != MMR_OK) return rc;
  } else {
    CUDA_TRY(cudaStreamSynchronize(st));
  }
  memcpy(out_scores_host, ix->h_box + BOX_HEADER, size_t(B) * k * 4);
  memcpy(out_rows_host, ix->h_box + box_rows_off(B, k), size_t(B) * k * 8);
  return MMR_OK;
}

extern "C" int mmr_search_host(mmr_index* ix, const float* queries_host, const int32_t* query_seg_host, int32_t B,
                               int32_t k, float* out_scores_host, int64_t* out_rows_host, void* stream) {
  int rc = check_search_args(ix, B, k);
  if (rc != MMR_OK) return rc;
  if (!queries_host || !out_scores_host || !out_rows_host) return fail(MMR_ERR_INVALID, "NULL buffer");
  std::lock_guard<std::mutex> guard(ix->host_mu);
  CUDA_TRY(cudaSetDevice(ix->device));
  rc = ensure_staging(ix, B, k);
  if (rc != MMR_OK) return rc;
  cudaStream_t st = static_cast<cudaStream_t>(stream);
  std::vector<RangeList> ranges;
  bool uniform = true;
  rc = ranges_from_segments(ix, query_seg_host, B, ranges, uniform);
  if (rc != MMR_OK) return rc;
  float* box_s = reinterpret_cast<float*>(ix->d_box + BOX_HEADER);
  int64_t* box_r = reinterpret_cast<int64_t*>(ix->d_box + box_rows_off(B, k));
  Completion done;
  done.flag_dev = reinterpret_cast<uint32_t*>(ix->d_box);
  done.seq = ++ix->box_seq ? ix->box_seq : ++ix->box_seq;
  const uint32_t r0 = ranges[0][0].first, r1 = ranges[0][0].second;
  if (uniform && can_inline(ix, B) && !uniform_takes_k2(ix, B, k, int64_t(r1) - r0)) {
    QuerySrc q;
    q.host = queries_host;
    rc = search_uniform_stream(ix, q, B, k, r0, r1, box_s, box_r, static_cast<uint8_t*>(ix->d_ws), st, nullptr, &done);
  } else {
    memcpy(ix->h_q, queries_host, size_t(B) * ix->dim * 4);
    CUDA_TRY(cudaMemcpyAsync(ix->d_q, ix->h_q, size_t(B) * ix->dim * 4, cudaMemcpyHostToDevice, st));
    QuerySrc q;
    q.dev = ix->d_q;
    if (uniform)
      rc = search_uniform(ix, q, B, k, r0, r1, box_s, box_r, static_cast<uint8_t*>(ix->d_ws), ix->ws_bytes, st, nullptr, &done);
    else
      rc = search_varlen_stream(ix, ix->d_q, ranges, k, box_s, box_r, static_cast<uint8_t*>(ix->d_ws), ix->ws_bytes, st);
  }
  if (rc != MMR_OK) return rc;
  return finish_host_call(ix, done, B, k, out_scores_host, out_rows_host, st);
}

static uint32_t xchg_score_bytes(int B, int k) { return uint32_t((size_t(B) * k * 4 + 7) / 8 * 8); }
static uint32_t xchg_wire_bytes(int B, int k) { return uint32_t((xchg_score_bytes(B, k) + size_t(B) * k * 8 + 15) / 16 * 16); }

extern "C" size_t mmr_exchange_buffer_bytes(int32_t G, int32_t B, int32_t k) {
  if (G <= 0 || G > MMR_XCHG_MAX_PEERS || B <= 0 || k <= 0) return 0;
  return size_t(MMR_XCHG_HEADER) + size_t(2) * G * xchg_wire_bytes(B, k);
}

extern "C" size_t mmr_search_exchange_workspace_bytes(const mmr_index* ix, int32_t B, int32_t k) {
  const size_t base = mmr_search_workspace_bytes(ix, B, k);
  return base ? base + align_up(xchg_wire_bytes(B, std::min<int32_t>(k, MMR_MAX_K)), 256) : 0;
}

static int exchange_impl(const mmr_index* ix, QuerySrc q, int B, int k, bool uniform, uint32_t r0, uint32_t r1,
                         const std::vector<RangeList>* per_query, const uint64_t* peer_bufs, int G, int rank, uint32_t seq,
                         uint32_t push_mask, bool do_merge, float* out_s, int64_t* out_r, uint8_t* ws, size_t base_ws,
                         cudaStream_t st, Completion* done) {
  const uint32_t score_bytes = xchg_score_bytes(B, k), wire_bytes = xchg_wire_bytes(B, k);
  const int parity = int(seq & 1u);
  uint8_t* wire = ws + base_ws;
  float* w_scores = reinterpret_cast<float*>(wire);
  int64_t* w_rows = reinterpret_cast<int64_t*>(wire + score_bytes);
  ExchangeInfo xi;
  xi.seq = seq;
  xi.wire_score_bytes = score_bytes;
  for (int g = 0; g < G; ++g) {
    if (!(push_mask >> g & 1u)) continue;
    xi.slot[xi.n_peers] = peer_bufs[g] + MMR_XCHG_HEADER + (size_t(parity) * G + rank) * wire_bytes;
    xi.flag[xi.n_peers] = peer_bufs[g] + (size_t(parity) * MMR_XCHG_MAX_PEERS + rank) * 4;
    ++xi.n_peers;
  }
  bool pushed = false;
  const bool k2 = uniform && q.dev != nullptr && uniform_takes_k2(ix, B, k, int64_t(r1) - r0);
  if (uniform && !k2 && B <= k1_group(ix) && (q.dev != nullptr || can_inline(ix, B))) {
    int rc = search_uniform_stream(ix, q, B, k, r0, r1, w_scores, w_rows, ws, st, &xi);
    if (rc != MMR_OK) return rc;
    pushed = true;
  } else {
    if (q.dev == nullptr) return fail(MMR_ERR_INVALID, "this batch needs device-resident queries");
    int rc = uniform ? search_uniform(ix, q, B, k, r0, r1, w_scores, w_rows, ws, base_ws, st)
                     : search_varlen_stream(ix, q.dev, *per_query, k, w_scores, w_rows, ws, base_ws, st);
    if (rc != MMR_OK) return rc;
  }
  if (!pushed && xi.n_peers > 0) {
    PeerPtrs pp;
    for (int g = 0; g < MMR_XCHG_MAX_PEERS; ++g) {
      pp.slot[g] = g < xi.n_peers ? xi.slot[g] : 0;
      pp.flag[g] = g < xi.n_peers ? xi.flag[g] : 0;
    }
    push_wire_kernel<<<xi.n_peers, 256, 0, st>>>(wire, wire_bytes, pp, seq);
    g_launches++;
  }
  if (!do_merge) return MMR_OK;
  const uint8_t* local = reinterpret_cast<const uint8_t*>(peer_bufs[rank]);
  const int wpb = 4;
  const uint64_t timeout_ns = 5000000000ull;
  cudaLaunchConfig_t cfg = {};
  cfg.gridDim = dim3((B + wpb - 1) / wpb);
  cfg.blockDim = dim3(wpb * 32);
  cfg.dynamicSmemBytes = 0;
  cfg.stream = st;
  cudaLaunchAttribute attr[1];
  attr[0].id = cudaLaunchAttributeProgrammaticStreamSerialization;
  attr[0].val.programmaticStreamSerializationAllowed = (pushed && options().pdl) ? 1 : 0;
  cfg.attrs = attr;
  cfg.numAttrs = 1;
  uint32_t* done_flag = nullptr;
  uint32_t done_seq = 0;
  if (done && done->flag_dev && cfg.gridDim.x == 1 && options().mailbox) {
    done_flag = done->flag_dev;
    done_seq = done->seq;
    done->armed = true;
  }
  if (k <= 32)
    CUDA_TRY(cudaLaunchKernelEx(&cfg, merge_wait_kernel<1>, local, parity, seq, wire_bytes, score_bytes, int(G), int(B),
                                int(k), out_s, out_r, timeout_ns, done_flag, done_seq));
  else
    CUDA_TRY(cudaLaunchKernelEx(&cfg, merge_wait_kernel<2>, local, parity, seq, wire_bytes, score_bytes, int(G), int(B),
                                int(k), out_s, out_r, timeout_ns, done_flag, done_seq));
  g_launches++;
  return MMR_OK;
}

static int check_exchange_args(const mmr_index* ix, int B, int k, const uint64_t* peer_bufs_host, int G, int rank, uint32_t seq) {
  int rc = check_search_args(ix, B, k);
  if (rc != MMR_OK) return rc;
  if (!peer_bufs_host || G < 1 || G > MMR_XCHG_MAX_PEERS || rank < 0 || rank >= G)
    return fail(MMR_ERR_INVALID, "bad peer table (G=%d, rank=%d)", G, rank);
  if (seq == 0) return fail(MMR_ERR_INVALID, "seq must start at 1 and grow by 1 per search");
  return MMR_OK;
}

extern "C" int mmr_search_exchange(const mmr_index* ix, const float* queries_dev, const int32_t* query_seg_host,
                                   int32_t B, int32_t k, const uint64_t* peer_bufs_host, int32_t G, int32_t rank,
                                   uint32_t seq, float* out_scores_dev, int64_t* out_rows_dev, void* workspace_dev,
                                   size_t workspace_bytes, void* stream) {
  int rc = check_exchange_args(ix, B, k, peer_bufs_host, G, rank, seq);
  if (rc != MMR_OK) return rc;
  if (!queries_dev || !out_scores_dev || !out_rows_dev || !workspace_dev) return fail(MMR_ERR_INVALID, "NULL buffer");
  const size_t base_ws = mmr_search_workspace_bytes(ix, B, k);
  if (workspace_bytes < mmr_search_exchange_workspace_bytes(ix, B, k)) return fail(MMR_ERR_WORKSPACE, "workspace too small");
  std::vector<RangeList> ranges;
  bool uniform = true;
  rc = ranges_from_segments(ix, query_seg_host, B, ranges, uniform);
  if (rc != MMR_OK) return rc;
  QuerySrc q;
  q.dev = queries_dev;
  return exchange_impl(ix, q, B, k, uniform, ranges[0][0].first, ranges[0][0].second, &ranges, peer_bufs_host, G, rank, seq,
                       (G >= 32 ? 0xFFFFFFFFu : ((1u << G) - 1u)), true, out_scores_dev, out_rows_dev,
                       static_cast<uint8_t*>(workspace_dev), base_ws, static_cast<cudaStream_t>(stream), nullptr);
}

extern "C" int mmr_search_exchange_host(mmr_index* ix, const float* queries_host, const int32_t* query_seg_host, int32_t B,
                                        int32_t k, const uint64_t* peer_bufs_host, int32_t G, int32_t rank, uint32_t seq,
                                        float* out_scores_host, int64_t* out_rows_host, void* stream) {
  int rc = check_exchange_args(ix, B, k, peer_bufs_host, G, rank, seq);
  if (rc != MMR_OK) return rc;
  if (!queries_host || !out_scores_host || !out_rows_host) return fail(MMR_ERR_INVALID, "NULL buffer");
  std::lock_guard<std::mutex> guard(ix->host_mu);
  CUDA_TRY(cudaSetDevice(ix->device));
  rc = ensure_staging(ix, B, k);
  if (rc != MMR_OK) return rc;
  cudaStream_t st = static_cast<cudaStream_t>(stream);
  std::vector<RangeList> ranges;
  bool uniform = true;
  rc = ranges_from_segments(ix, query_seg_host, B, ranges, uniform);
  if (rc != MMR_OK) return rc;
  const size_t base_ws = workspace_bytes_for(ix, ix->cap_b, ix->cap_k, int64_t(RANGES_PER_QUERY_BUDGET) * ix->cap_b);
  const size_t need = base_ws + align_up(xchg_wire_bytes(ix->cap_b, ix->cap_k), 256);
  if (ix->ws_bytes < need) {
    if (ix->d_ws) cudaFree(ix->d_ws);
    ix->d_ws = nullptr;
    CUDA_TRY(cudaMalloc(&ix->d_ws, need));
    CUDA_TRY(cudaMemset(ix->d_ws, 0, need));
    ix->ws_bytes = need;
  }
  float* box_s = reinterpret_cast<float*>(ix->d_box + BOX_HEADER);
  int64_t* box_r = reinterpret_cast<int64_t*>(ix->d_box + box_rows_off(B, k));
  Completion done;
  done.flag_dev = reinterpret_cast<uint32_t*>(ix->d_box);
  done.seq = ++ix->box_seq ? ix->box_seq : ++ix->box_seq;
  QuerySrc q;
  const uint32_t r0 = ranges[0][0].first, r1 = ranges[0][0].second;
  if (uniform && can_inline(ix, B) && !uniform_takes_k2(ix, B, k, int64_t(r1) - r0)) {
    q.host = queries_host;
  } else {
    memcpy(ix->h_q, queries_host, size_t(B) * ix->dim * 4);
    CUDA_TRY(cudaMemcpyAsync(ix->d_q, ix->h_q, size_t(B) * ix->dim * 4, cudaMemcpyHostToDevice, st));
    q.dev = ix->d_q;
  }
  rc = exchange_impl(ix, q, B, k, uniform, r0, r1, &ranges, peer_bufs_host, G, rank, seq,
                     (G >= 32 ? 0xFFFFFFFFu : ((1u << G) - 1u)), true, box_s, box_r, static_cast<uint8_t*>(ix->d_ws),
                     base_ws, st, &done);
  if (rc != MMR_OK) return rc;
  return finish_host_call(ix, done, B, k, out_scores_host, out_rows_host, st);
}

struct mmr_multi {
  int G = 0;
  std::vector<mmr_index*> shard;
  std::vector<cudaStream_t> stream;
  std::vector<uint8_t*> xbuf;
  std::vector<uint64_t> peer_ptrs;
  int cap_b = 0, cap_k = 0;
  uint32_t seq = 0;
  uint32_t mail_seq = 0;
  std::mutex call_mu;
  std::vector<std::thread> workers;
  std::mutex mu;
  std::condition_variable cv;
  std::atomic<uint64_t> job_seq{0};
  std::atomic<int> pending{0};
  std::atomic<bool> stop{false};
  const float* q_host = nullptr;
  const std::vector<RangeList>* ranges = nullptr;
  int B = 0, k = 0;
  std::vector<int> rc;
  std::vector<std::string> err;
};

static void multi_free_xbuf(mmr_multi* m) {
  for (int g = 0; g < m->G; ++g) {
    if (m->xbuf[g]) {
      cudaSetDevice(m->shard[g]->device);
      cudaFree(m->xbuf[g]);
      m->xbuf[g] = nullptr;
    }
  }
}

static int multi_run_shard(mmr_multi* m, int g) {
  mmr_index* ix = m->shard[g];
  const int B = m->B, k = m->k;
  std::lock_guard<std::mutex> guard(ix->host_mu);
  int rc = ensure_staging(ix, std::max(B, m->cap_b), std::max(k, m->cap_k));
  if (rc != MMR_OK) return rc;
  const size_t base_ws = workspace_bytes_for(ix, ix->cap_b, ix->cap_k, int64_t(RANGES_PER_QUERY_BUDGET) * ix->cap_b);
  const size_t need = base_ws + align_up(xchg_wire_bytes(ix->cap_b, ix->cap_k), 256);
  if (ix->ws_bytes < need) {
    if (ix->d_ws) cudaFree(ix->d_ws);
    ix->d_ws = nullptr;
    CUDA_TRY(cudaMalloc(&ix->d_ws, need));
    CUDA_TRY(cudaMemset(ix->d_ws, 0, need));
    ix->ws_bytes = need;
  }
  const int64_t lo_g = ix->row_base, hi_g = ix->row_base + ix->n_rows;
  std::vector<RangeList> local(B);
  bool uniform = true;
  for (int b = 0; b < B; ++b) {
    for (auto& r : (*m->ranges)[b]) {
      const int64_t lo = std::max<int64_t>(r.first, lo_g), hi = std::min<int64_t>(r.second, hi_g);
      if (hi > lo) local[b].push_back({uint32_t(lo - lo_g), uint32_t(hi - lo_g)});
    }
    if (local[b].size() > 1 || local[b] != local[0]) uniform = false;
  }
  const uint32_t r0 = (uniform && !local[0].empty()) ? local[0][0].first : 0u;
  const uint32_t r1 = (uniform && !local[0].empty()) ? local[0][0].second : 0u;
  cudaStream_t st = m->stream[g];
  QuerySrc q;
  if (uniform && can_inline(ix, B) && !uniform_takes_k2(ix, B, k, int64_t(r1) - r0)) {
    q.host = m->q_host;
  } else {
    memcpy(ix->h_q, m->q_host, size_t(B) * ix->dim * 4);
    CUDA_TRY(cudaMemcpyAsync(ix->d_q, ix->h_q, size_t(B) * ix->dim * 4, cudaMemcpyHostToDevice, st));
    q.dev = ix->d_q;
  }
  Completion done;
  float* box_s = nullptr;
  int64_t* box_r = nullptr;
  if (g == 0) {
    box_s = reinterpret_cast<float*>(ix->d_box + BOX_HEADER);
    box_r = reinterpret_cast<int64_t*>(ix->d_box + box_rows_off(B, k));
    done.flag_dev = reinterpret_cast<uint32_t*>(ix->d_box);
    done.seq = m->mail_seq;
  }
  rc = exchange_impl(ix, q, B, k, uniform, r0, r1, &local, m->peer_ptrs.data(), m->G, g, m->seq, 1u ,
                     g == 0, box_s, box_r, static_cast<uint8_t*>(ix->d_ws), base_ws, st, g == 0 ? &done : nullptr);
  if (rc == MMR_OK && g == 0 && !done.armed) {
    CUDA_TRY(cudaStreamSynchronize(st));
    *reinterpret_cast<volatile uint32_t*>(ix->h_box) = m->mail_seq;
  }
  return rc;
}

static void multi_worker(mmr_multi* m, int g) {
  cudaSetDevice(m->shard[g]->device);
  uint64_t seen = 0;
  for (;;) {
    int spins = 0;
    while (m->job_seq.load(std::memory_order_acquire) == seen && !m->stop.load(std::memory_order_relaxed)) {
      if (++spins < 20000) {
        cpu_relax();
      } else {
        std::unique_lock<std::mutex> lk(m->mu);
        m->cv.wait_for(lk, std::chrono::milliseconds(50), [&] {
          return m->job_seq.load(std::memory_order_acquire) != seen || m->stop.load(std::memory_order_relaxed);
        });
      }
    }
    if (m->stop.load(std::memory_order_relaxed)) return;
    seen = m->job_seq.load(std::memory_order_acquire);
    m->rc[g] = multi_run_shard(m, g);
    if (m->rc[g] != MMR_OK) m->err[g] = g_err;
    m->pending.fetch_sub(1, std::memory_order_acq_rel);
  }
}

extern "C" int mmr_multi_create(mmr_index** shards, int32_t G, mmr_multi** out) {
  if (!out) return fail(MMR_ERR_INVALID, "out is NULL");
  *out = nullptr;
  if (!shards || G < 1 || G > MMR_XCHG_MAX_PEERS) return fail(MMR_ERR_INVALID, "need 1..%d shards", MMR_XCHG_MAX_PEERS);
  for (int g = 0; g < G; ++g) {
    if (!shards[g]) return fail(MMR_ERR_INVALID, "shard %d is NULL", g);
    if (shards[g]->dim != shards[0]->dim || shards[g]->dtype != shards[0]->dtype)
      return fail(MMR_ERR_INVALID, "shards must share dim and dtype");
    for (int h = 0; h < g; ++h)
      if (shards[h]->device == shards[g]->device) return fail(MMR_ERR_INVALID, "one shard per device");
  }
  mmr_multi* m = new mmr_multi();
  m->G = G;
  m->shard.assign(shards, shards + G);
  m->stream.assign(G, nullptr);
  m->xbuf.assign(G, nullptr);
  m->peer_ptrs.assign(G, 0);
  m->rc.assign(G, MMR_OK);
  m->err.assign(G, std::string());
  const int collector = shards[0]->device;
  for (int g = 0; g < G; ++g) {
    const int dev = shards[g]->device;
// ... 204 lines not shown
```

multimodal-rag-for-image-text-search_b200/csrc/scan_stream.cuh:

```cuda
#pragma once
#include "common.cuh"
#include "topk.cuh"

namespace mmr {

#ifndef MMR_K1_NW
#define MMR_K1_NW 8
#endif
#ifndef MMR_K1_STAGES
#define MMR_K1_STAGES 2
#endif
#ifndef MMR_K1_ROWS
#define MMR_K1_ROWS 4
#endif
#ifndef MMR_K1_STAGES_NQ2
#define MMR_K1_STAGES_NQ2 3
#endif
#ifndef MMR_K1_STAGES_NQ4
#define MMR_K1_STAGES_NQ4 MMR_K1_STAGES
#endif
#ifndef MMR_K1_NW_NQ4
#define MMR_K1_NW_NQ4 12
#endif
constexpr int K1_NW = MMR_K1_NW;
constexpr int MMR_MAX_PEERS = 16;

constexpr int MMR_MAX_K_DEVICE = 64;
constexpr int K1_ITEM_NQ = 4;
constexpr int K1_INLINE_FLOATS = 1024;

struct ScanItem {
  uint32_t row_begin;
  uint32_t row_end;
  int32_t query[K1_ITEM_NQ];
  int32_t nq;
  int32_t out;
};

struct QuerySlot {
  int32_t item0;
  int32_t n_items;
  int32_t slot;
  int32_t pad;
};

struct StreamParams {
  const void* rows;
  const float* queries;
  int32_t q_first;
  int32_t nq;
  int32_t k;
  uint32_t row_begin, row_end;
  uint64_t* partial;
  unsigned int* ticket;
  float* out_scores;
  int64_t* out_rows;
  int64_t row_base;
  const ScanItem* items;
  int32_t n_items;
  int32_t item_nq;
  int32_t n_peers;
  uint32_t seq;
  uint32_t wire_score_bytes;
  uint64_t peer_slot[MMR_MAX_PEERS];
  uint64_t peer_flag[MMR_MAX_PEERS];
  uint32_t* done_flag;
  uint32_t done_seq;
  float qinline[K1_INLINE_FLOATS];
};

template <typename E>
struct ElemTraits;
template <>
struct ElemTraits<__nv_bfloat16> {
  static constexpr int BYTES = 2;
  static __device__ __forceinline__ void unpack(uint32_t w, float& a, float& b) {
    a = __uint_as_float(w << 16);
    b = __uint_as_float(w & 0xFFFF0000u);
  }
};
template <>
struct ElemTraits<__half> {
  static constexpr int BYTES = 2;
  static __device__ __forceinline__ void unpack(uint32_t w, float& a, float& b) {
    const __half2 h = *reinterpret_cast<const __half2*>(&w);
    const float2 f = __half22float2(h);
    a = f.x;
    b = f.y;
  }
};
template <>
struct ElemTraits<float> {
  static constexpr int BYTES = 4;
};

template <int N, int OFF>
__device__ __forceinline__ void transpose_reduce_step(float* v, int lane) {
  if constexpr (OFF >= 1) {
    if constexpr (N > 1) {
      constexpr int H = N / 2;
      const bool upper = (lane & OFF) != 0;
#pragma unroll
      for (int i = 0; i < H; ++i) {
        const float send = upper ? v[i] : v[i + H];
        const float keep = upper ? v[i + H] : v[i];
        v[i] = keep + __shfl_xor_sync(0xffffffffu, send, OFF);
      }
      transpose_reduce_step<H, OFF / 2>(v, lane);
    } else {
      v[0] += __shfl_xor_sync(0xffffffffu, v[0], OFF);
      transpose_reduce_step<1, OFF / 2>(v, lane);
    }
  }
}
template <int V>
__device__ __forceinline__ float transpose_reduce(float (&v)[V], int lane) {
  static_assert(V >= 1 && V <= 32 && (V & (V - 1)) == 0, "V must be a power of two <= 32");
  transpose_reduce_step<V, 16>(v, lane);
  return v[0];
}

template <typename E, int D, int NQ, int KPL>
struct StreamCfg {
  static constexpr int EB = ElemTraits<E>::BYTES;
  static constexpr int ROW_BYTES = D * EB;
  static constexpr int R = MMR_K1_ROWS;
  static constexpr int V = R * NQ;
  static constexpr int STAGE_BYTES = R * ROW_BYTES;
  static constexpr int S_WANT = NQ >= 4 ? MMR_K1_STAGES_NQ4 : NQ >= 2 ? MMR_K1_STAGES_NQ2 : MMR_K1_STAGES;
  static constexpr int NW = (NQ >= 4 && EB == 2) ? MMR_K1_NW_NQ4 : K1_NW;
  static constexpr int THREADS = NW * 32;
  static constexpr int S_FIT = (160 * 1024) / (NW * STAGE_BYTES);
  static constexpr int S = S_WANT < S_FIT ? S_WANT : (S_FIT < 2 ? 2 : S_FIT);
  static constexpr int VECB = (ROW_BYTES % 512 == 0) ? 16 : 8;
  static constexpr int NV = ROW_BYTES / (32 * VECB);
  static constexpr int RPV = VECB / 4;
  static constexpr int EPR = 4 / EB;
  static constexpr int EPL = D / 32;
  static constexpr int KSLOTS = 32 * KPL;
  static constexpr int RING_BYTES = NW * S * STAGE_BYTES;
  static constexpr int SMEM_BYTES = RING_BYTES + NW * S * 8 + 64;
  static_assert(ROW_BYTES % (32 * 8) == 0, "D * sizeof(elem) must be a multiple of 256 bytes");
  static_assert(S >= 2, "ring too shallow");
  static_assert(V <= 32, "too many dot products per stage");
  static_assert(NW * NQ * KSLOTS * 8 <= RING_BYTES, "merge scratch must fit in the ring");
};

template <typename E, int D, int NQ, int KPL>
__global__ void __launch_bounds__((StreamCfg<E, D, NQ, KPL>::THREADS), 1) scan_stream_kernel(const __grid_constant__ StreamParams p) {
  using C = StreamCfg<E, D, NQ, KPL>;
  extern __shared__ __align__(1024) uint8_t smem[];
  uint64_t* bars = reinterpret_cast<uint64_t*>(smem + C::RING_BYTES);
  __shared__ int s_last;

  const int lane = threadIdx.x & 31;
  const int warp = threadIdx.x >> 5;
  const int k = p.k;

  asm volatile("griddepcontrol.launch_dependents;" ::: "memory");
  if (p.items != nullptr) asm volatile("griddepcontrol.wait;" ::: "memory");

  const uint32_t ring0 = smem_u32(smem) + uint32_t(warp) * (C::S * C::STAGE_BYTES);
  const uint32_t bar0 = smem_u32(bars) + uint32_t(warp) * (C::S * 8);
  if (lane == 0) {
#pragma unroll
    for (int s = 0; s < C::S; ++s) mbar_init(bar0 + s * 8, 1);
    fence_mbar_init();
  }
  __syncwarp();

  float q[NQ][C::EPL];
#pragma unroll
  for (int qi = 0; qi < NQ; ++qi) {
    const bool live = qi < p.nq;
    const float* qbase = p.queries ? p.queries : p.qinline;
    const float* qsrc = qbase + size_t(p.items ? 0 : (p.q_first + (live ? qi : 0))) * D;
    float ss = 0.f;
#pragma unroll
    for (int t = 0; t < C::NV; ++t)
#pragma unroll
      for (int j = 0; j < C::RPV * C::EPR; ++j) {
        const int e = (t * 32 + lane) * (C::RPV * C::EPR) + j;
        const float x = (live && !p.items) ? qsrc[e] : 0.f;
        q[qi][t * C::RPV * C::EPR + j] = x;
        ss += x * x;
      }
    ss = warp_allreduce_sum(ss);
    const float nrm = sqrtf(ss);
    if (nrm > 0.f) {
#pragma unroll
      for (int e = 0; e < C::EPL; ++e) q[qi][e] = q[qi][e] / nrm;
    }
  }

  WarpTopK<KPL> list[NQ];
  uint64_t thr[NQ];
#pragma unroll
  for (int qi = 0; qi < NQ; ++qi) {
    list[qi].clear();
    thr[qi] = 0ull;
  }

  const int gwarp = blockIdx.x * C::NW + warp;
  const int twarps = gridDim.x * C::NW;
  const uint8_t* rows8 = reinterpret_cast<const uint8_t*>(p.rows);

  int stage = 0;
  uint32_t phase = 0;
  int nq_live = p.nq;

  auto scan_range = [&](uint32_t row_begin, uint32_t row_end, int first, int stride) {
    const uint32_t nrows = row_end > row_begin ? row_end - row_begin : 0u;
    const int nchunks = int((nrows + C::R - 1) / C::R);
    auto issue = [&](int c, int s) {
      const uint32_t r0 = row_begin + uint32_t(c) * C::R;
      const uint32_t nr = min(uint32_t(C::R), row_end - r0);
      const uint32_t bytes = nr * C::ROW_BYTES;
      const uint32_t bar = bar0 + s * 8;
      mbar_arrive_expect_tx(bar, bytes);
      bulk_g2s(ring0 + s * C::STAGE_BYTES, rows8 + size_t(r0) * C::ROW_BYTES, bytes, bar);
    };
    if (lane == 0) {
      int sj = stage;
#pragma unroll
      for (int j = 0; j < C::S; ++j) {
        const int c = first + j * stride;
        if (c < nchunks) issue(c, sj);
        sj = (sj + 1 == C::S) ? 0 : sj + 1;
      }
    }
    for (int c = first; c < nchunks; c += stride) {
      const int s = stage;
      mbar_wait(bar0 + s * 8, phase);

      const uint32_t base = ring0 + s * C::STAGE_BYTES + lane * C::VECB;
      float acc[C::V];
#pragma unroll
      for (int i = 0; i < C::V; ++i) acc[i] = 0.f;
#pragma unroll
      for (int r = 0; r < C::R; ++r) {
#pragma unroll
        for (int t = 0; t < C::NV; ++t) {
          uint32_t w[C::RPV];
          const uint32_t addr = base + r * C::ROW_BYTES + t * (32 * C::VECB);
          if constexpr (C::VECB == 16) {
            lds_v4(addr, reinterpret_cast<uint32_t(&)[4]>(w));
          } else {
            lds_v2(addr, reinterpret_cast<uint32_t(&)[2]>(w));
          }
#pragma unroll
          for (int j = 0; j < C::RPV; ++j) {
            if constexpr (C::EB == 2) {
              float a, b;
              ElemTraits<E>::unpack(w[j], a, b);
#pragma unroll
              for (int qi = 0; qi < NQ; ++qi) {
                acc[r * NQ + qi] = fmaf(a, q[qi][(t * C::RPV + j) * 2 + 0], acc[r * NQ + qi]);
                acc[r * NQ + qi] = fmaf(b, q[qi][(t * C::RPV + j) * 2 + 1], acc[r * NQ + qi]);
              }
            } else {
              const float a = __uint_as_float(w[j]);
#pragma unroll
              for (int qi = 0; qi < NQ; ++qi)
                acc[r * NQ + qi] = fmaf(a, q[qi][t * C::RPV + j], acc[r * NQ + qi]);
            }
          }
        }
      }
      __syncwarp();
      if (lane == 0) {
        const int cn = c + C::S * stride;
        if (cn < nchunks) {
          fence_proxy_async();
          issue(cn, s);
        }
      }

      const float score = transpose_reduce<C::V>(acc, lane);
      constexpr int LPV = 32 / C::V;
      const int vi = lane / LPV;
      const int r = vi / NQ;
      const int myq = vi % NQ;
      const uint32_t row = row_begin + uint32_t(c) * C::R + uint32_t(r);
      const bool owner = (lane % LPV == 0) && row < row_end && score == score;
      const uint64_t key = make_key(score, row);
#pragma unroll
      for (int qi = 0; qi < NQ; ++qi) {
        if (qi < nq_live) thr[qi] = list[qi].offer(key, owner && myq == qi, thr[qi], k, lane);
      }
      if (++stage == C::S) {
        stage = 0;
        phase ^= 1u;
      }
    }
  };

  if (p.items == nullptr) {
    scan_range(p.row_begin, p.row_end, gwarp, twarps);

    asm volatile("griddepcontrol.wait;" ::: "memory");
    __syncthreads();
    uint64_t* wk = reinterpret_cast<uint64_t*>(smem);
#pragma unroll
    for (int qi = 0; qi < NQ; ++qi) {
#pragma unroll
      for (int j = 0; j < KPL; ++j) wk[(warp * NQ + qi) * C::KSLOTS + j * 32 + lane] = list[qi].key[j];
    }
    __syncthreads();
    if (warp < p.nq) {
      const int qi = warp;
      WarpTopK<KPL> m;
      m.clear();
      uint64_t t = 0ull;
      t = m.template merge_batched<4>(
          [&](int i) -> uint64_t { return wk[((i % C::NW) * NQ + qi) * C::KSLOTS + i / C::NW]; }, C::NW * k, t, k, lane);
      m.store(p.partial + (size_t(blockIdx.x) * NQ + qi) * k, k, lane);
    }
    __threadfence();
    __syncthreads();
    if (threadIdx.x == 0) {
      const unsigned int prev = atomicAdd(p.ticket, 1u);
      s_last = (prev == gridDim.x - 1);
    }
    __syncthreads();
    if (!s_last) return;
    __threadfence();
    const int nparts = gridDim.x;
    for (int qi = 0; qi < p.nq; ++qi) {
      WarpTopK<KPL> m;
      m.clear();
      uint64_t t = 0ull;
      {
        const int nmine = (nparts - warp + C::NW - 1) / C::NW;
        const uint64_t* base = p.partial;
        t = m.template merge_batched<8>(
            [&](int i) -> uint64_t {
              const int pos = i / nmine, part = warp + (i % nmine) * C::NW;
              return __ldcg(reinterpret_cast<const unsigned long long*>(base) + (size_t(part) * NQ + qi) * k + pos);
            },
            nmine * k, t, k, lane);
      }
      __syncthreads();
#pragma unroll
      for (int j = 0; j < KPL; ++j) wk[warp * C::KSLOTS + j * 32 + lane] = m.key[j];
      __syncthreads();
      if (warp == 0) {
        WarpTopK<KPL> f;
        f.clear();
        uint64_t tf = 0ull;
        tf = f.template merge_batched<4>(
            [&](int i) -> uint64_t { return wk[(i % C::NW) * C::KSLOTS + i / C::NW]; }, C::NW * k, tf, k, lane);
#pragma unroll
        for (int j = 0; j < KPL; ++j) {
          const int pos = j * 32 + lane;
          if (pos < k) {
            const uint64_t key = f.key[j];
            const size_t o = size_t(p.q_first + qi) * k + pos;
            const float sc = key ? key_score(key) : -INFINITY;
            const int64_t rw = key ? int64_t(key_row(key)) + p.row_base : int64_t(-1);
            p.out_scores[o] = sc;
            p.out_rows[o] = rw;
            for (int g = 0; g < p.n_peers; ++g) {
              reinterpret_cast<float*>(p.peer_slot[g])[o] = sc;
              reinterpret_cast<int64_t*>(p.peer_slot[g] + p.wire_score_bytes)[o] = rw;
            }
          }
        }
      }
    }
    if (threadIdx.x == 0) *p.ticket = 0u;
    if (p.n_peers > 0 || p.done_flag != nullptr) {
      __threadfence_system();
      __syncthreads();
      if (int(threadIdx.x) < p.n_peers)
        asm volatile("st.release.sys.global.u32 [%0], %1;" ::"l"(p.peer_flag[threadIdx.x]), "r"(p.seq) : "memory");
      if (threadIdx.x == 0 && p.done_flag != nullptr)
        asm volatile("st.release.sys.global.u32 [%0], %1;" ::"l"(p.done_flag), "r"(p.done_seq) : "memory");
    }
  } else {
    uint64_t* wk = reinterpret_cast<uint64_t*>(smem);
    __shared__ int s_claim[2];
    int it = blockIdx.x;
    for (int round = 0; it < p.n_items; ++round) {
      if (threadIdx.x == 0) s_claim[round & 1] = int(gridDim.x + atomicAdd(p.ticket, 1u));
      const ScanItem item = p.items[it];
      nq_live = min(item.nq, NQ);
#pragma unroll
      for (int qi = 0; qi < NQ; ++qi) {
        const float* qsrc = p.queries + size_t(item.query[qi < nq_live ? qi : 0]) * D;
        float ss = 0.f;
#pragma unroll
        for (int t = 0; t < C::NV; ++t)
#pragma unroll
          for (int j = 0; j < C::RPV * C::EPR; ++j) {
            const float x = qsrc[(t * 32 + lane) * (C::RPV * C::EPR) + j];
            q[qi][t * C::RPV * C::EPR + j] = x;
            ss += x * x;
          }
        ss = warp_allreduce_sum(ss);
        const float nrm = sqrtf(ss);
        if (nrm > 0.f) {
#pragma unroll
          for (int e = 0; e < C::EPL; ++e) q[qi][e] = q[qi][e] / nrm;
        }
        list[qi].clear();
        thr[qi] = 0ull;
      }
      scan_range(item.row_begin, item.row_end, warp, C::NW);
      __syncthreads();
#pragma unroll
      for (int qi = 0; qi < NQ; ++qi) {
#pragma unroll
        for (int j = 0; j < KPL; ++j) wk[(warp * NQ + qi) * C::KSLOTS + j * 32 + lane] = list[qi].key[j];
      }
      __syncthreads();
      if (warp < nq_live) {
        const int qi = warp;
        WarpTopK<KPL> m;
        m.clear();
        uint64_t t = 0ull;
        t = m.template merge_batched<4>(
            [&](int i) -> uint64_t { return wk[((i % C::NW) * NQ + qi) * C::KSLOTS + i / C::NW]; }, C::NW * k, t, k, lane);
        m.store(p.partial + (size_t(item.out) * p.item_nq + qi) * k, k, lane);
      }
      __syncthreads();
      it = s_claim[round & 1];
    }
    if (threadIdx.x == 0) {
      __threadfence();
      if (atomicAdd(p.ticket + 1, 1u) == gridDim.x - 1) {
        p.ticket[0] = 0u;
        p.ticket[1] = 0u;
      }
    }
  }
}

template <typename E, int D>
__device__ __forceinline__ void k1_load_unit_query(const float* __restrict__ qsrc, int lane, float (&q)[D / 32]) {
  using C = StreamCfg<E, D, 1, 1>;
  float ss = 0.f;
#pragma unroll
  for (int t = 0; t < C::NV; ++t)
#pragma unroll
    for (int j = 0; j < C::RPV * C::EPR; ++j) {
      const float x = qsrc[(t * 32 + lane) * (C::RPV * C::EPR) + j];
      q[t * C::RPV * C::EPR + j] = x;
      ss += x * x;
    }
  ss = warp_allreduce_sum(ss);
  const float nrm = sqrtf(ss);
  if (nrm > 0.f) {
#pragma unroll
    for (int e = 0; e < C::EPL; ++e) q[e] = q[e] / nrm;
  }
}

template <typename E, int D>
__device__ __forceinline__ float k1_row_score(const uint8_t* __restrict__ row, const float (&q)[D / 32], int lane) {
  using C = StreamCfg<E, D, 1, 1>;
  float acc = 0.f;
#pragma unroll
  for (int t = 0; t < C::NV; ++t) {
    uint32_t w[C::RPV];
    const uint8_t* src = row + lane * C::VECB + t * (32 * C::VECB);
    if constexpr (C::VECB == 16) {
      const uint4 v = __ldg(reinterpret_cast<const uint4*>(src));
      w[0] = v.x; w[1] = v.y; w[2] = v.z; w[3] = v.w;
    } else {
      const uint2 v = __ldg(reinterpret_cast<const uint2*>(src));
      w[0] = v.x; w[1] = v.y;
    }
#pragma unroll
    for (int j = 0; j < C::RPV; ++j) {
      if constexpr (C::EB == 2) {
        float a, b;
        ElemTraits<E>::unpack(w[j], a, b);
        acc = fmaf(a, q[(t * C::RPV + j) * 2 + 0], acc);
        acc = fmaf(b, q[(t * C::RPV + j) * 2 + 1], acc);
      } else {
        acc = fmaf(__uint_as_float(w[j]), q[t * C::RPV + j], acc);
      }
    }
  }
#pragma unroll
  for (int o = 16; o > 0; o >>= 1) acc += __shfl_xor_sync(0xffffffffu, acc, o);
  return acc;
}

template <typename E, int D, int KPL>
__global__ void __launch_bounds__(256) rescore_kernel(const void* __restrict__ rows, const float* __restrict__ queries,
                                                      const float* __restrict__ cand_scores, const int64_t* __restrict__ cand_rows,
                                                      const float* __restrict__ qerr, int kc, int k, int64_t row_base,
                                                      float* __restrict__ out_scores, int64_t* __restrict__ out_rows,
                                                      uint8_t* __restrict__ exact_flag) {
  __shared__ uint64_t keys[MMR_MAX_K_DEVICE];
  const int b = blockIdx.x, lane = threadIdx.x & 31, warp = threadIdx.x >> 5;
  float q[D / 32];
  k1_load_unit_query<E, D>(queries + size_t(b) * D, lane, q);
  const uint8_t* rows8 = reinterpret_cast<const uint8_t*>(rows);
  for (int c = warp; c < kc; c += 8) {
    const int64_t r = cand_rows[size_t(b) * kc + c];
    uint64_t key = 0ull;
    if (r >= 0) {
      const uint32_t local = uint32_t(r - row_base);
      const float s = k1_row_score<E, D>(rows8 + size_t(local) * (D * sizeof(E)), q, lane);
      key = make_key(s, local);
    }
    if (lane == 0) keys[c] = key;
  }
  __syncthreads();
  if (warp == 0) {
    WarpTopK<KPL> m;
    m.clear();
    uint64_t thr = 0ull;
    thr = m.template merge_batched<2>([&](int i) -> uint64_t { return keys[i]; }, kc, thr, k, lane);
#pragma unroll
    for (int j = 0; j < KPL; ++j) {
      const int pos = j * 32 + lane;
      if (pos < k) {
        const uint64_t key = m.key[j];
        out_scores[size_t(b) * k + pos] = key ? key_score(key) : -INFINITY;
        out_rows[size_t(b) * k + pos] = key ? int64_t(key_row(key)) + row_base : int64_t(-1);
      }
    }
    if (lane == 0) {
      const bool all_rows = cand_rows[size_t(b) * kc + kc - 1] < 0;
      const float c_min = cand_scores[size_t(b) * kc + kc - 1];
      const float eps = 1.01f * qerr[b] + 2e-5f;
      const float kth32 = thr ? key_score(thr) : -INFINITY;
      exact_flag[b] = (all_rows || (thr != 0ull && kth32 > c_min + eps)) ? 1 : 0;
    }
  }
}

template <int KPL>
__global__ void merge_items_kernel(const uint64_t* __restrict__ partial, const QuerySlot* __restrict__ slots, int nq,
                                   int nq_per_item, int k, float* __restrict__ out_scores,
                                   int64_t* __restrict__ out_rows, int64_t row_base) {
  const int lane = threadIdx.x & 31;
  const int qi = blockIdx.x * (blockDim.x >> 5) + (threadIdx.x >> 5);
  if (qi >= nq) return;
  WarpTopK<KPL> m;
  m.clear();
  uint64_t t = 0ull;
  const QuerySlot sl = slots[qi];
  const uint64_t* base = partial + (size_t(sl.item0) * nq_per_item + sl.slot) * k;
  const size_t item_stride = size_t(nq_per_item) * k;
  t = m.template merge_batched<4>(
      [&](int i) -> uint64_t {
        const int item = i % sl.n_items, pos = i / sl.n_items;
        return __ldcg(reinterpret_cast<const unsigned long long*>(base) + size_t(item) * item_stride + pos);
      },
      sl.n_items * k, t, k, lane);
#pragma unroll
  for (int j = 0; j < KPL; ++j) {
    const int pos = j * 32 + lane;
    if (pos < k) {
      const uint64_t key = m.key[j];
      out_scores[size_t(qi) * k + pos] = key ? key_score(key) : -INFINITY;
      out_rows[size_t(qi) * k + pos] = key ? int64_t(key_row(key)) + row_base : int64_t(-1);
    }
  }
}

}
```

multimodal-rag-for-image-text-search_b200/index.py:

```python
from __future__ import annotations

import ctypes as C
from typing import Optional, Sequence, Tuple

import numpy as np
import torch

from . import _native as N

_DTYPES = {
    "bf16": (N.MMR_BF16, torch.bfloat16),
    "f16": (N.MMR_F16, torch.float16),
    "f32": (N.MMR_F32, torch.float32),
}


def _ptr(t: Optional[torch.Tensor]) -> Optional[int]:
    return None if t is None else t.data_ptr()


def _stream_ptr(device: torch.device) -> int:
    return torch.cuda.current_stream(device).cuda_stream


class ResidentIndex:

    def __init__(self, rows: torch.Tensor, seg_offsets: Optional[Sequence[int]] = None, row_base: int = 0):
        if not rows.is_cuda:
            raise N.NativeError("ResidentIndex needs CUDA rows: this package has no CPU path")
        if rows.dim() != 2 or not rows.is_contiguous():
            raise ValueError("rows must be a contiguous [n, dim] tensor")
        kinds = {v[1]: (k, v[0]) for k, v in _DTYPES.items()}
        if rows.dtype not in kinds:
            raise ValueError(f"unsupported row dtype {rows.dtype}")
        self.dtype_name, self._dtype_code = kinds[rows.dtype]
        self.rows = rows
        self.device = rows.device
        self.n_rows, self.dim = int(rows.shape[0]), int(rows.shape[1])
        self.row_base = int(row_base)
        self.seg_offsets = None if seg_offsets is None else np.ascontiguousarray(seg_offsets, dtype=np.int64)
        self._handle = C.c_void_p()
        self._ws: Optional[torch.Tensor] = None
        self._one: dict = {}
        self._ws_key = (0, 0, 0)
        lib = N.lib()
        nseg = 0 if self.seg_offsets is None else len(self.seg_offsets) - 1
        segp = None if self.seg_offsets is None else self.seg_offsets.ctypes.data
        N.check(lib.mmr_index_create(self.device.index or 0, self.dim, self._dtype_code, self.n_rows,
                                     rows.data_ptr() if self.n_rows else None, segp, nseg, self.row_base,
                                     C.byref(self._handle)))

    @classmethod
    def from_f32(cls, rows_f32, seg_offsets=None, dtype: str = "bf16", device="cuda:0", normalize: bool = False,
                 row_base: int = 0) -> "ResidentIndex":
        code, tdt = _DTYPES[dtype]
        device = torch.device(device)
        lib = N.lib()
        if isinstance(rows_f32, np.ndarray):
            src = np.ascontiguousarray(rows_f32, dtype=np.float32)
            n, d = src.shape
            dst = torch.empty((n, d), dtype=tdt, device=device)
            with torch.cuda.device(device):
                N.check(lib.mmr_load_rows_f32_host(device.index or 0, src.ctypes.data, _ptr(dst) if n else None, code,
                                                   n, d, int(normalize), _stream_ptr(device)))
        else:
            src = rows_f32.to(device=device, dtype=torch.float32).contiguous()
            n, d = src.shape
            dst = torch.empty((n, d), dtype=tdt, device=device)
            with torch.cuda.device(device):
                N.check(lib.mmr_convert_rows_f32(_ptr(src) if n else None, _ptr(dst) if n else None, code, n, d,
                                                 int(normalize), _stream_ptr(device)))
        return cls(dst, seg_offsets, row_base)

    @staticmethod
    def alloc_rows(n: int, dim: int, dtype: str, device) -> torch.Tensor:
        return torch.empty((int(n), int(dim)), dtype=_DTYPES[dtype][1], device=torch.device(device))

    @staticmethod
    def load_rows_into(buf: torch.Tensor, src_f32: np.ndarray, dst_rows: Optional[np.ndarray] = None,
                       dst_offset: int = 0, normalize: bool = False) -> None:
        kinds = {v[1]: v[0] for v in _DTYPES.values()}
        src = np.ascontiguousarray(src_f32, dtype=np.float32)
        n, d = src.shape
        if n == 0:
            return
        if d != buf.shape[1]:
            raise ValueError(f"row length {d} != resident row length {buf.shape[1]}")
        dev = buf.device
        esize = buf.element_size()
        if dst_rows is not None:
            m = np.ascontiguousarray(dst_rows, dtype=np.int64)
            if m.shape != (n,) or (m.size and int(m.max()) >= buf.shape[0]):
                raise ValueError("dst_rows must hold one in-range resident row per source row")
            dst_ptr, mp = buf.data_ptr(), m.ctypes.data
        else:
            if dst_offset < 0 or dst_offset + n > buf.shape[0]:
                raise ValueError("rows do not fit the resident buffer")
            dst_ptr, mp = buf.data_ptr() + dst_offset * d * esize, None
        with torch.cuda.device(dev):
            N.check(N.lib().mmr_load_rows_f32_host_scatter(dev.index or 0, src.ctypes.data, dst_ptr, kinds[buf.dtype], n, d,
                                                           int(normalize), mp, _stream_ptr(dev)))

    def update(self, rows: torch.Tensor, n_rows: Optional[int] = None, seg_offsets=None) -> None:
        if rows.dtype != self.rows.dtype or rows.shape[1] != self.dim or not rows.is_contiguous():
            raise ValueError("update needs a contiguous tensor of the same dtype and dim")
        n = int(rows.shape[0]) if n_rows is None else int(n_rows)
        self.seg_offsets = None if seg_offsets is None else np.ascontiguousarray(seg_offsets, dtype=np.int64)
        nseg = 0 if self.seg_offsets is None else len(self.seg_offsets) - 1
        segp = None if self.seg_offsets is None else self.seg_offsets.ctypes.data
        N.check(N.lib().mmr_index_update(self._handle, n, rows.data_ptr() if n else None, segp, nseg))
        self.rows, self.n_rows = rows, n

    def search_ranges(self, queries: torch.Tensor, k: int, ranges) -> Tuple[torch.Tensor, torch.Tensor]:
        if queries.dim() == 1:
            queries = queries[None, :]
        b = int(queries.shape[0])
        k = max(int(k), 1)
        off = np.zeros(b + 1, dtype=np.int32)
        flat = []
        for i, rq in enumerate(ranges):
            flat.extend(rq)
            off[i + 1] = len(flat)
        arr = np.ascontiguousarray(flat, dtype=np.int64).reshape(-1, 2) if flat else np.zeros((1, 2), np.int64)
        scores = torch.empty((b, k), dtype=torch.float32, device=self.device)
        rows = torch.empty((b, k), dtype=torch.int64, device=self.device)
        ws = self._workspace(b, k, n_ranges=len(flat))
        with torch.cuda.device(self.device):
            N.check(N.lib().mmr_search_ranges(self._handle, queries.data_ptr(), b, k, off.ctypes.data, arr.ctypes.data,
                                              scores.data_ptr(), rows.data_ptr(), ws.data_ptr(), ws.numel(),
                                              _stream_ptr(self.device)))
        return scores, rows

    def close(self) -> None:
        if self._handle:
            N.lib().mmr_index_destroy(self._handle)
            self._handle = C.c_void_p()

    def __del__(self):
        try:
            self.close()
        except Exception:
            pass

    def _workspace(self, b: int, k: int, n_ranges: int = 0) -> torch.Tensor:
        key = (b, k, n_ranges)
        if key != self._ws_key or self._ws is None:
            lib = N.lib()
            need = max(lib.mmr_search_workspace_bytes(self._handle, b, k),
                       lib.mmr_search_ranges_workspace_bytes(self._handle, b, k, n_ranges) if n_ranges else 0)
            if self._ws is None or self._ws.numel() < need:
                self._ws = torch.zeros(int(need), dtype=torch.uint8, device=self.device)
            self._ws_key = key
        return self._ws

    def set_query_precision(self, mode: str) -> None:
        N.check(N.lib().mmr_index_set_query_precision(
            self._handle, {"auto": N.MMR_QP_AUTO, "f32": N.MMR_QP_F32, "rescore": N.MMR_QP_RESCORE}[mode]))

    def search(self, queries: torch.Tensor, k: int, segments: Optional[Sequence[int]] = None,
               out: Optional[Tuple[torch.Tensor, torch.Tensor]] = None) -> Tuple[torch.Tensor, torch.Tensor]:
        if queries.dim() == 1:
            queries = queries[None, :]
        if not queries.is_cuda or queries.dtype != torch.float32 or not queries.is_contiguous():
            raise ValueError("queries must be a contiguous float32 CUDA tensor")
        if queries.shape[1] != self.dim:
            raise ValueError(f"query dim {queries.shape[1]} != index dim {self.dim}")
        b = int(queries.shape[0])
        k = max(int(k), 1)
        if out is None:
            scores = torch.empty((b, k), dtype=torch.float32, device=self.device)
            rows = torch.empty((b, k), dtype=torch.int64, device=self.device)
        else:
            scores, rows = out
        seg_arr = None
        if segments is not None:
            seg_arr = np.ascontiguousarray(segments, dtype=np.int32)
            if seg_arr.shape != (b,):
                raise ValueError("segments must have one entry per query")
        ws = self._workspace(b, k)
        args = (self._handle, queries.data_ptr(), None if seg_arr is None else seg_arr.ctypes.data, b, k, scores.data_ptr(),
                rows.data_ptr(), ws.data_ptr(), ws.numel(), _stream_ptr(self.device))
        if torch.cuda.current_device() == (self.device.index or 0):
            N.check(N.lib().mmr_search(*args))
        else:
            with torch.cuda.device(self.device):
                N.check(N.lib().mmr_search(*args))
        return scores, rows

    def debug_umma_scores(self, queries: torch.Tensor, row_begin: int, row_end: int) -> torch.Tensor:
        b = int(queries.shape[0])
        n = int(row_end - row_begin)
        out = torch.full((b, n), float("nan"), dtype=torch.float32, device=self.device)
        ws = self._workspace(max(b, 8), 10)
        with torch.cuda.device(self.device):
            N.check(N.lib().mmr_debug_umma_scores(self._handle, queries.contiguous().data_ptr(), b, int(row_begin),
                                                  int(row_end), out.data_ptr(), n, ws.data_ptr(), ws.numel(),
                                                  _stream_ptr(self.device)))
        return out

    def search_host(self, queries: np.ndarray, k: int, segments: Optional[Sequence[int]] = None):
        q = np.ascontiguousarray(np.atleast_2d(queries), dtype=np.float32)
        if q.shape[1] != self.dim:
            raise ValueError(f"query dim {q.shape[1]} != index dim {self.dim}")
        b = q.shape[0]
        k = max(int(k), 1)
        scores = np.empty((b, k), dtype=np.float32)
        rows = np.empty((b, k), dtype=np.int64)
        seg_arr = None if segments is None else np.ascontiguousarray(segments, dtype=np.int32)
        if torch.cuda.current_device() == (self.device.index or 0):
            N.check(N.lib().mmr_search_host(self._handle, q.ctypes.data, None if seg_arr is None else seg_arr.ctypes.data,
                                            b, k, scores.ctypes.data, rows.ctypes.data, _stream_ptr(self.device)))
        else:
            with torch.cuda.device(self.device):
                N.check(N.lib().mmr_search_host(self._handle, q.ctypes.data, None if seg_arr is None else seg_arr.ctypes.data,
                                                b, k, scores.ctypes.data, rows.ctypes.data, _stream_ptr(self.device)))
        return scores, rows


    def search_host_one(self, q: np.ndarray, k: int, segment: int = 0):
        k = max(int(k), 1)
        slot = self._one.get(k)
        if slot is None:
            scores = np.empty((1, k), dtype=np.float32)
            rows = np.empty((1, k), dtype=np.int64)
            seg = np.zeros(1, dtype=np.int32)
            slot = self._one[k] = (scores, rows, seg, scores.ctypes.data, rows.ctypes.data, seg.ctypes.data)
        scores, rows, seg, p_s, p_r, p_seg = slot
        if q.dtype != np.float32 or not q.flags.c_contiguous or q.size != self.dim:
            raise ValueError(f"search_host_one needs one contiguous float32 query of dim {self.dim}")
        seg[0] = segment
        fn = N.lib().mmr_search_host
        if torch.cuda.current_device() == (self.device.index or 0):
            N.check(fn(self._handle, q.ctypes.data, p_seg, 1, k, p_s, p_r, _stream_ptr(self.device)))
        else:
            with torch.cuda.device(self.device):
                N.check(fn(self._handle, q.ctypes.data, p_seg, 1, k, p_s, p_r, _stream_ptr(self.device)))
        return scores, rows


class MultiIndex:

    def __init__(self, shards: Sequence[ResidentIndex]) -> None:
        self.shards = list(shards)
        self._handle = C.c_void_p()
        arr = (C.c_void_p * len(self.shards))(*[s._handle for s in self.shards])
        N.check(N.lib().mmr_multi_create(arr, len(self.shards), C.byref(self._handle)))
        self.dim = self.shards[0].dim
        self.n_rows = max(s.row_base + s.n_rows for s in self.shards)

    def search_host(self, queries: np.ndarray, k: int, ranges=None):
        q = np.ascontiguousarray(np.atleast_2d(queries), dtype=np.float32)
        if q.shape[1] != self.dim:
            raise ValueError(f"query dim {q.shape[1]} != index dim {self.dim}")
        b = q.shape[0]
        k = max(int(k), 1)
        if ranges is None:
            ranges = [[(0, self.n_rows)]] * b
        off = np.zeros(b + 1, dtype=np.int32)
        flat = []
        for i, rq in enumerate(ranges):
            flat.extend(rq)
            off[i + 1] = len(flat)
        arr = np.ascontiguousarray(flat, dtype=np.int64).reshape(-1, 2) if flat else np.zeros((1, 2), np.int64)
        scores = np.empty((b, k), dtype=np.float32)
        rows = np.empty((b, k), dtype=np.int64)
        with torch.cuda.device(self.shards[0].device):
            N.check(N.lib().mmr_multi_search_host(self._handle, q.ctypes.data, b, k, off.ctypes.data, arr.ctypes.data,
                                                  scores.ctypes.data, rows.ctypes.data))
        return scores, rows

    def close(self) -> None:
        if self._handle:
            N.lib().mmr_multi_destroy(self._handle)
            self._handle = C.c_void_p()

    def __del__(self):
        try:
            self.close()
        except Exception:
            pass


def merge_topk(scores: torch.Tensor, rows: torch.Tensor) -> Tuple[torch.Tensor, torch.Tensor]:
    g, b, k = scores.shape
    out_s = torch.empty((b, k), dtype=torch.float32, device=scores.device)
    out_r = torch.empty((b, k), dtype=torch.int64, device=scores.device)
    with torch.cuda.device(scores.device):
        N.check(N.lib().mmr_merge_topk(scores.contiguous().data_ptr(), rows.contiguous().data_ptr(), g, b, k,
                                       out_s.data_ptr(), out_r.data_ptr(), _stream_ptr(scores.device)))
    return out_s, out_r


def fuse(text: Optional[Tuple[torch.Tensor, torch.Tensor]], image: Optional[Tuple[torch.Tensor, torch.Tensor]],
         final_n: int, tau: float):
    ref = text if text is not None else image
    if ref is None:
        raise ValueError("need at least one modality")
    dev = ref[0].device
    b = int(ref[0].shape[0])
    kt = 0 if text is None else int(text[0].shape[1])
    ki = 0 if image is None else int(image[0].shape[1])
    comb = torch.empty((b, final_n), dtype=torch.float64, device=dev)
    score = torch.empty((b, final_n), dtype=torch.float64, device=dev)
    rows = torch.empty((b, final_n), dtype=torch.int64, device=dev)
    mod = torch.empty((b, final_n), dtype=torch.int8, device=dev)
    low = torch.empty((b,), dtype=torch.uint8, device=dev)
    with torch.cuda.device(dev):
        N.check(N.lib().mmr_fuse(_ptr(text[0].contiguous()) if kt else None, _ptr(text[1].contiguous()) if kt else None, kt,
                                 _ptr(image[0].contiguous()) if ki else None, _ptr(image[1].contiguous()) if ki else None, ki,
                                 b, int(final_n), float(tau), comb.data_ptr(), score.data_ptr(), rows.data_ptr(),
                                 mod.data_ptr(), low.data_ptr(), _stream_ptr(dev)))
    return {"combined": comb, "score": score, "rows": rows, "modality": mod, "low_conf": low}


def fuse_f64(text_scores, text_count, img_scores, img_count, final_n: int, tau: float, rerank=None, rerank_count=None):
    ref = text_scores if text_scores is not None else img_scores
    dev = ref.device
    b = int(ref.shape[0])
    kt = 0 if text_scores is None else int(text_scores.shape[1])
    ki = 0 if img_scores is None else int(img_scores.shape[1])
    comb = torch.empty((b, final_n), dtype=torch.float64, device=dev)
    index = torch.empty((b, final_n), dtype=torch.int32, device=dev)
    low = torch.empty((b,), dtype=torch.uint8, device=dev)

    def p(t, dt):
        return None if t is None else t.to(device=dev, dtype=dt).contiguous()

    ts, tc, rr, rc = p(text_scores, torch.float64), p(text_count, torch.int32), p(rerank, torch.float64), p(rerank_count, torch.int32)
    is_, ic = p(img_scores, torch.float64), p(img_count, torch.int32)
    with torch.cuda.device(dev):
        N.check(N.lib().mmr_fuse_f64(_ptr(ts), _ptr(tc), _ptr(rr), _ptr(rc), _ptr(is_), _ptr(ic), kt, ki, b, int(final_n),
                                     float(tau), comb.data_ptr(), index.data_ptr(), low.data_ptr(), _stream_ptr(dev)))
    return {"combined": comb, "index": index, "low_conf": low}
```

multimodal-rag-for-image-text-search_b200/store.py:

```python
from __future__ import annotations

import json
from array import array
import os
import threading
from dataclasses import dataclass
from typing import Any, Dict, Iterable, List, Optional, Sequence

import numpy as np
import torch

from . import _native as N
from .durable import DurableLog
from .hosttable import HostTable, make_arrow_table, rows_to_arrow
from .index import MultiIndex, ResidentIndex
from .versions import VersionFile


@dataclass
class VectorRow:

    chunk_id: str
    user_id: str
    document_id: str
    modality: str
    embedding: Sequence[float]
    meta: Dict[str, Any]


def _unit_f32(vector: Sequence[float]) -> np.ndarray:
    arr = np.asarray(vector, dtype=np.float32)
    norm = np.linalg.norm(arr)
    if norm <= 0:
        return arr
    return arr / norm


def _grow_filled(arr: np.ndarray, need: int, fill) -> np.ndarray:
    if need <= arr.shape[0]:
        return arr
    out = np.full(max(need, int(arr.shape[0] * 1.5) + 1024), fill, dtype=arr.dtype)
    out[: arr.shape[0]] = arr
    return out


class _Collection:

    MAX_RANGES = 8
    MAX_TOMB_FRACTION = 0.25

    def __init__(self, name: str, device: torch.device, dtype: str, log: Optional[DurableLog] = None,
                 query_precision: str = "f32", devices: Optional[Sequence[torch.device]] = None) -> None:
        self.devices = [torch.device(d) for d in devices] if devices else [device]
        self.query_precision = query_precision
        self.name = name
        self.device = device
        self.dtype = dtype
        self.host = HostTable(name)
        self._lock = threading.RLock()
        self._log = log
        self._gen: Optional[int] = None
        self._n_deltas = 0
        self._stamp = None
        self.rebuilds = 0
        self.appends = 0
        self.refreshes = 0
        self.last_load_gbs: Optional[float] = None
        self._reset_resident()

    def _reset_resident(self) -> None:
        old = getattr(self, "_resident", None)
        if old is not None:
            old.close()
        for sh in getattr(self, "_shards", []) or []:
            sh.close()
        multi = getattr(self, "_multi", None)
        if multi is not None:
            multi.close()
        self._multi: Optional[MultiIndex] = None
        self._shards: List[ResidentIndex] = []
        self._bufs: List[torch.Tensor] = []
        self._bounds: List[int] = []
        self._resident: Optional[ResidentIndex] = None
        self._buf: Optional[torch.Tensor] = None
        self._n_res = 0
        self._perm = np.empty(0, np.int64)
        self._res_of = np.empty(0, np.int64)
        self._ranges: Dict[str, List[List[int]]] = {}
        self._tomb = 0
        self._synced_upto = 0
        self._pending_tomb: List[int] = []
        self._force_rebuild = True
        self._seg_key = None

    def __len__(self) -> int:
        return len(self.host)

    def host_row_of(self, chunk_id: str) -> int:
        return int(self.host.find_alive([chunk_id])[0])

    def _host_rows(self, idx: np.ndarray) -> np.ndarray:
        return self.host.gather(np.asarray(idx, dtype=np.int64))

    def _ingest(self, table) -> List[str]:
        _, n, killed, users = self.host.append_table(table)
        if n == 0:
            return []
        self._res_of = _grow_filled(self._res_of, self.host.n_total, -1)
        if killed.size:
            res = self._res_of[killed]
            self._pending_tomb.extend(int(r) for r in res[res >= 0])
            self._res_of[killed] = -1
        return users

    def upsert(self, rows: Iterable[VectorRow]) -> List[str]:
        rows = list(rows)
        if not rows:
            return []
        try:
            table = rows_to_arrow(rows, _unit_f32)
        except ValueError as exc:
            raise ValueError(f"{self.name}: {exc}") from None
        return self.add_table(table)

    def add_table(self, table) -> List[str]:
        if table.num_rows == 0:
            return []
        with self._lock:
            if self._log is None:
                return self._ingest(table)
            with self._log.locked():
                self.refresh()
                users = self._ingest(table)
                self._log.append_delta(table)
                self._n_deltas += 1
                self._stamp = self._log.stamp()
            return users

    def refresh(self, force: bool = False, _depth: int = 0) -> List[str]:
        if self._log is None:
            return []
        stamp = self._log.stamp()
        if stamp == self._stamp and not force and self._gen is not None:
            return []
        users: List[str] = []
        with self._lock:
            m = self._log.manifest()
            try:
                if m["generation"] != self._gen:
                    if self._gen is not None or self.host.n_total:
                        self.host = HostTable(self.name)
                        self._reset_resident()
                    if m["base"]:
                        users += self._ingest(self._log.read_table(m["base"]))
                    self._gen, self._n_deltas = m["generation"], 0
                for fname in m["deltas"][self._n_deltas:]:
                    users += self._ingest(self._log.read_table(fname))
                    self._n_deltas += 1
            except FileNotFoundError:
                if _depth >= 3:
                    raise
                self._gen = None
                return self.refresh(force=True, _depth=_depth + 1)
            self._stamp = stamp
            self.refreshes += 1
        return sorted(set(users))

    def persist(self) -> None:
        if self._log is None:
            raise ValueError("collection has no durable log")
        with self._lock, self._log.locked():
            self.refresh()
            m = self._log.write_base(self.host.to_arrow())
            self._gen, self._n_deltas = m["generation"], 0
            self._stamp = self._log.stamp()

    def _rebuild(self) -> None:
        import time

        host = self.host
        alive = host.alive_rows()
        self._reset_resident()
        self._force_rebuild = False
        self._synced_upto = host.n_total
        self._res_of = np.full(host.n_total, -1, dtype=np.int64)
        n = int(alive.size)
        if n == 0:
            return
        tenant = host.tenant[alive]
        order = np.argsort(tenant, kind="stable")
        perm = alive[order]
        counts = np.bincount(tenant, minlength=len(host.tenants))
        seg = np.zeros(len(host.tenants) + 1, dtype=np.int64)
        np.cumsum(counts, out=seg[1:])
        self._res_of[perm] = np.arange(n, dtype=np.int64)
        cap = max(n + 4096, int(n * 1.25))
        self._perm = np.full(cap, -1, dtype=np.int64)
        self._perm[:n] = perm
        G = len(self.devices)
        self._bounds = [int(round(g * n / G)) for g in range(G)] + [n]
        self._bufs = [ResidentIndex.alloc_rows((self._bounds[g + 1] - self._bounds[g]) if g < G - 1 else cap - self._bounds[g],
                                               host.dim, self.dtype, self.devices[g]) for g in range(G)]
        self._buf = self._bufs[-1]
        t0 = time.perf_counter()
        moved = 0
        jobs = []
        for blk in host.blocks:
            dst = self._res_of[blk.start:blk.start + blk.n]
            if G == 1:
                if (dst >= 0).any():
                    jobs.append((0, blk.emb, dst))
            else:
                for g in range(G):
                    lo, hi = self._bounds[g], self._bounds[g + 1]
                    hit = np.nonzero((dst >= lo) & (dst < hi))[0]
                    if hit.size == 0:
                        continue
                    i0, i1 = int(hit[0]), int(hit[-1]) + 1
                    sub = dst[i0:i1]
                    jobs.append((g, blk.emb[i0:i1], np.where((sub >= lo) & (sub < hi), sub - lo, -1)))
            moved += blk.n
        if G == 1:
            for g, src, local in jobs:
                ResidentIndex.load_rows_into(self._bufs[g], src, dst_rows=local)
        else:
            from concurrent.futures import ThreadPoolExecutor

            def upload(g):
                for gg, src, local in jobs:
                    if gg == g:
                        ResidentIndex.load_rows_into(self._bufs[g], src, dst_rows=local)

            with ThreadPoolExecutor(G) as pool:
                list(pool.map(upload, range(G)))
        dt = time.perf_counter() - t0
        self.last_load_gbs = moved * host.dim * 4 / dt / 1e9 if dt > 0 else None
        self._n_res = n
        self._shards = []
        for g in range(G):
            ng = self._bounds[g + 1] - self._bounds[g]
            sh = ResidentIndex(self._bufs[g][:ng], row_base=self._bounds[g])
            sh.update(self._bufs[g], ng)
            sh.set_query_precision(self.query_precision)
            self._shards.append(sh)
        self._resident = self._shards[-1]
        self._multi = MultiIndex(self._shards) if G > 1 else None
        self._ranges = {host.tenants[i]: [[int(seg[i]), int(seg[i + 1])]] for i in range(len(host.tenants)) if counts[i]}
        self.rebuilds += 1

    def _pending_rows(self) -> np.ndarray:
        lo, hi = self._synced_upto, self.host.n_total
        return np.nonzero(self.host.alive[lo:hi])[0] + lo

    def _apply_deltas(self) -> None:
        if self._pending_tomb:
            tomb = np.asarray(self._pending_tomb, dtype=np.int64)
            G = len(self._bufs)
            which = np.minimum(np.searchsorted(np.asarray(self._bounds[:G]), tomb, side="right") - 1, G - 1)
            for g in np.unique(which):
                idx = torch.as_tensor(tomb[which == g] - self._bounds[int(g)], dtype=torch.int64, device=self._bufs[int(g)].device)
                self._bufs[int(g)].index_fill_(0, idx, float("nan"))
            self._tomb += len(self._pending_tomb)
            self._pending_tomb = []
        rows = self._pending_rows()
        self._synced_upto = self.host.n_total
        if rows.size:
            tenant = self.host.tenant[rows]
            order = np.argsort(tenant, kind="stable")
            rows, tenant = rows[order], tenant[order]
            m = int(rows.size)
            lo = self._n_res
            ResidentIndex.load_rows_into(self._buf, self.host.gather(rows), dst_offset=lo - self._bounds[-2])
            self._perm[lo:lo + m] = rows
            self._res_of[rows] = lo + np.arange(m, dtype=np.int64)
            cuts = np.nonzero(np.diff(tenant))[0] + 1
            for start, end in zip(np.concatenate([[0], cuts]), np.concatenate([cuts, [m]])):
                rl = self._ranges.setdefault(self.host.tenants[int(tenant[start])], [])
                if rl and rl[-1][1] == lo + int(start):
                    rl[-1][1] = lo + int(end)
                else:
                    rl.append([lo + int(start), lo + int(end)])
            self._n_res = lo + m
            self.appends += 1
        self._resident.update(self._buf, self._n_res - self._bounds[-2])
        self._seg_key = None

    def resident(self) -> Optional[ResidentIndex]:
        with self._lock:
            dirty = self._synced_upto != self.host.n_total or self._pending_tomb
            if not self._force_rebuild and not dirty:
                return self._resident
            n_new = int(self.host.alive[self._synced_upto:self.host.n_total].sum())
            need_rebuild = (
                self._force_rebuild or self._resident is None or self._buf is None
                or self._n_res + n_new > self._bounds[-2] + self._buf.shape[0]
                or (self._tomb + len(self._pending_tomb)) > self.MAX_TOMB_FRACTION * max(self._n_res, 1)
                or any(len(r) >= self.MAX_RANGES for r in self._ranges.values())
            )
            if need_rebuild:
                self._rebuild()
            else:
                self._apply_deltas()
            return self._resident

    def search_device(self, user_ids: Sequence[str], vectors: np.ndarray, top_k: int):
        limit = max(int(top_k), 1)
        if limit > N.MMR_MAX_K:
            raise N.NativeError(f"top_k {limit} > {N.MMR_MAX_K}: not supported by the resident-index kernels")
        with self._lock:
            res = self.resident()
            if res is None:
                return None
            ranges = [self._ranges.get(str(u)) or [] for u in user_ids]
            on_device = isinstance(vectors, torch.Tensor)
            if self._multi is not None:
                host_q = vectors.detach().float().cpu().numpy() if on_device else vectors
                s, r = self._multi.search_host(np.ascontiguousarray(host_q, dtype=np.float32), limit, ranges)
                return torch.from_numpy(s).to(self.devices[0]), torch.from_numpy(r).to(self.devices[0])
            if on_device:
                q = vectors.to(device=self.device, dtype=torch.float32).contiguous()
            else:
                q = torch.from_numpy(np.ascontiguousarray(vectors, dtype=np.float32)).to(self.device)
            return res.search_ranges(q, limit, ranges)

    def row_identity(self, resident_row: int) -> int:
        return int(self._perm[resident_row])

    def chunk_id_of(self, resident_row: int) -> str:
        return self.host.chunk_id_at(int(self._perm[resident_row]))

    def search(self, user_ids: Sequence[str], vectors: np.ndarray, top_k: int) -> List[List[Dict[str, Any]]]:
        limit = max(int(top_k), 1)
        if limit > N.MMR_MAX_K:
            raise N.NativeError(f"top_k {limit} > {N.MMR_MAX_K}: not supported by the resident-index kernels")
        with self._lock:
            res = self.resident()
            out: List[List[Dict[str, Any]]] = [[] for _ in user_ids]
            if res is None:
                return out
            ranges = [self._ranges.get(str(u)) for u in user_ids]
            live = [i for i, r in enumerate(ranges) if r]
            if not live:
                return out
            q = vectors if len(live) == len(ranges) else vectors[live]
            if q.dtype != np.float32 or not q.flags.c_contiguous:
                q = np.ascontiguousarray(q, dtype=np.float32)
            first = ranges[live[0]]
            if self._multi is not None:
                scores, rows = self._multi.search_host(q, limit, [ranges[i] for i in live])
            elif len(first) == 1 and all(ranges[i] == first for i in live):
                lo, hi = first[0]
                if self._seg_key != (lo, hi, self._n_res):
                    res.update(self._buf, self._n_res, seg_offsets=[lo, hi])
                    self._seg_key = (lo, hi, self._n_res)
                if len(live) == 1 and hasattr(res, "search_host_one"):
                    scores, rows = res.search_host_one(q, limit, 0)
                else:
                    scores, rows = res.search_host(q, limit, [0] * len(live))
            else:
                s_dev, r_dev = res.search_ranges(torch.from_numpy(q).to(self.device), limit, [ranges[i] for i in live])
                scores, rows = s_dev.cpu().numpy(), r_dev.cpu().numpy()
            one = np.float32(1.0)
            sims = (1.0 - (one - scores).astype(np.float64)).tolist()
            hit_rows = rows.tolist()
            host, perm = self.host, self._perm
            for j, i in enumerate(live):
                rr = hit_rows[j]
                n = len(rr) if rr[-1] >= 0 else rr.index(-1)
                hrows = [perm[r] for r in rr[:n]]
                ids, metas = host.hits_at(hrows)
                sj = sims[j]
                out[i] = [{"chunk_id": ids[p], "score": sj[p], "meta": metas[p]} for p in range(n)]
            return out


class B200Store:

    def __init__(self, db_path: Optional[str] = None, device: Any = "cuda:0", dtype: str = "bf16",
                 devices: Optional[Sequence[Any]] = None, query_precision: str = "rescore") -> None:
        N.lib()
        if not torch.cuda.is_available():
            raise N.NativeError("no CUDA device: B200Store has no CPU fallback")
        devs = [torch.device("cuda", d) if isinstance(d, int) else torch.device(d) for d in devices] if devices else None
        self._init_state(db_path, devs[0] if devs else torch.device(device), dtype, devs, query_precision)

    def _init_state(self, db_path: Optional[str], device: torch.device, dtype: str, devices=None,
                    query_precision: str = "rescore") -> None:
        self._device = device
        self._db_path = db_path
        if db_path:
            os.makedirs(db_path, exist_ok=True)

        def log(name):
            return DurableLog(db_path, name) if db_path else None

        self._text_table = _Collection("text_collection", device, dtype, log("text_collection"), query_precision, devices)
        self._image_table = _Collection("image_collection", device, dtype, log("image_collection"), query_precision, devices)
        self._versions = VersionFile(os.path.join(db_path, "index_versions.json") if db_path else None)
        self._sync()

    def _sync(self) -> None:
        self._text_table.refresh()
        self._image_table.refresh()

    def _collection(self, name: str) -> _Collection:
        return {"text_collection": self._text_table, "image_collection": self._image_table}[name]

    def load_arrow_ipc(self, collection: str, path: str) -> None:
        import pyarrow as pa
        import pyarrow.ipc as ipc

        self.load_arrow(collection, ipc.open_file(pa.memory_map(path, "r")).read_all())

    def persist(self) -> None:
        if not self._db_path:
            raise ValueError("B200Store was created without a db_path")
        for coll in (self._text_table, self._image_table):
            coll.persist()

    def upsert_text_vectors(self, rows: Iterable[VectorRow]) -> None:
        for user in self._text_table.upsert(rows):
            self._versions.bump(user)

    def upsert_image_vectors(self, rows: Iterable[VectorRow]) -> None:
        for user in self._image_table.upsert(rows):
            self._versions.bump(user)

    def get_index_version(self, user_id: str) -> int:
        return self._versions.get(user_id)

    def load_arrow(self, collection: str, table) -> None:
        for user in self._collection(collection).add_table(table):
            self._versions.bump(user)

    def search_text(self, user_id: str, query_vec: Sequence[float], top_k: int) -> List[Dict[str, Any]]:
        self._text_table.refresh()
        return self._text_table.search([user_id], _query_row(query_vec), top_k)[0]

    def search_image(self, user_id: str, query_vec: Sequence[float], top_k: int) -> List[Dict[str, Any]]:
        self._image_table.refresh()
        return self._image_table.search([user_id], _query_row(query_vec), top_k)[0]

    def search_text_batch(self, user_ids: Sequence[str], query_vecs, top_k: int) -> List[List[Dict[str, Any]]]:
        self._text_table.refresh()
        return self._text_table.search(list(user_ids), np.asarray(query_vecs, dtype=np.float32), top_k)

    def search_image_batch(self, user_ids: Sequence[str], query_vecs, top_k: int) -> List[List[Dict[str, Any]]]:
        self._image_table.refresh()
        return self._image_table.search(list(user_ids), np.asarray(query_vecs, dtype=np.float32), top_k)

    def fused_search_batch(self, user_ids: Sequence[str], text_vecs, image_vecs, top_k_text: int, top_k_image: int,
                           final_n: int, tau: float):
        self._sync()
        return _fused_batch(self, list(user_ids), text_vecs, image_vecs, top_k_text, top_k_image, final_n, tau)

    def fused_search_batch_rerank(self, user_ids: Sequence[str], queries: Sequence[str], text_vecs, image_vecs,
                                  top_k_text: int, top_k_image: int, rerank_topk: int, final_n: int, tau: float,
                                  cross_encoder, metadata_store):
        self._sync()
        return _fused_batch_rerank(self, list(user_ids), list(queries), text_vecs, image_vecs, top_k_text, top_k_image,
                                   rerank_topk, final_n, tau, cross_encoder, metadata_store)


def _query_row(query_vec) -> np.ndarray:
    if isinstance(query_vec, (list, tuple)):
        try:
            return np.frombuffer(array("f", query_vec), dtype=np.float32)[None, :]
        except (TypeError, OverflowError):
            pass
    return np.asarray(query_vec, dtype=np.float32)[None, :]


def _as_queries(v):
    return v if isinstance(v, torch.Tensor) else np.asarray(v, dtype=np.float32)


def _fused_batch_rerank(store: "B200Store", user_ids, queries, text_vecs, image_vecs, kt: int, ki: int, rerank_topk: int,
                        final_n: int, tau: float, cross_encoder, metadata_store):
    from .index import fuse_f64

    n = len(user_ids)
    t = store._text_table.search_device(user_ids, _as_queries(text_vecs), kt)
    i = store._image_table.search_device(user_ids, _as_queries(image_vecs), ki)
    if t is None and i is None:
        return [([], True) for _ in user_ids]
    dev = (t if t is not None else i)[0].device
    one = torch.tensor(1.0, dtype=torch.float32, device=dev)

    def py_scores(pair, k):
        if pair is None:
            return torch.zeros((n, max(k, 1)), dtype=torch.float64, device=dev), torch.zeros(n, dtype=torch.int32, device=dev), None
        s, r = pair
        return 1.0 - (one - s).double(), (r >= 0).sum(dim=1).to(torch.int32), r

    ts, tc, tr = py_scores(t, kt)
    is_, ic, ir = py_scores(i, ki)
    head = min(rerank_topk, ts.shape[1])
    tr_host = tr[:, :head].cpu().numpy() if tr is not None else np.full((n, 0), -1)
    cand_ids = [[store._text_table.chunk_id_of(int(r)) for r in row if r >= 0] for row in tr_host]
    flat = [c for row in cand_ids for c in row]
    bulk = getattr(metadata_store, "get_chunks", None)
    found = bulk(flat) if (bulk and flat) else {c: metadata_store.get_chunk(c) for c in flat}
    pairs, owner, broken = [], [], set()
    for b, row in enumerate(cand_ids):
        for c in row:
            chunk = found.get(c)
            if not chunk or not chunk.text:
                broken.add(b)
                break
        if b not in broken:
            for c in row:
                pairs.append((queries[b], found[c].text))
                owner.append(b)
    rr = torch.zeros((n, ts.shape[1]), dtype=torch.float64, device=dev)
    rc = torch.zeros(n, dtype=torch.int32, device=dev)
    if pairs:
        logits = cross_encoder.predict_device(pairs).to(dev).double()
        counts = np.bincount(np.asarray(owner), minlength=n)
        rows_idx = torch.as_tensor(owner, device=dev, dtype=torch.int64)
        pos = torch.as_tensor(np.concatenate([np.arange(c) for c in counts]) if len(owner) else [], device=dev, dtype=torch.int64)
        rr[rows_idx, pos] = logits
        rc = torch.as_tensor(counts, dtype=torch.int32, device=dev)
    out = fuse_f64(ts if t is not None else None, tc if t is not None else None, is_ if i is not None else None,
                   ic if i is not None else None, final_n, tau, rerank=rr if t is not None else None,
                   rerank_count=rc if t is not None else None)
    comb, index, low = out["combined"].cpu().numpy(), out["index"].cpu().numpy(), out["low_conf"].cpu().numpy()
    ts_h = ts.cpu().numpy() if t is not None else None
    is_h = is_.cpu().numpy() if i is not None else None
    tr_all = tr.cpu().numpy() if tr is not None else None
    ir_all = ir.cpu().numpy() if ir is not None else None
    rr_h, rc_h = rr.cpu().numpy(), rc.cpu().numpy()
    kt_eff = ts.shape[1] if t is not None else 0
    results = []
    for b in range(n):
        if b in broken:
            results.append(None)
            continue
        items = []
        for o in range(final_n):
            ix = int(index[b, o])
            if ix < 0:
                break
            if ix < kt_eff and t is not None:
                it = {"chunk_id": store._text_table.chunk_id_of(int(tr_all[b, ix])), "modality": "text",
                      "score": float(ts_h[b, ix])}
                if ix < rc_h[b]:
                    it["rerank_score"] = float(rr_h[b, ix])
            else:
                j = ix - kt_eff
                it = {"chunk_id": store._image_table.chunk_id_of(int(ir_all[b, j])), "modality": "image", "score": float(is_h[b, j])}
            it["combined_score"] = float(comb[b, o])
            items.append(it)
        results.append((items, bool(low[b])))
    return results


def _fused_batch(store: "B200Store", user_ids, text_vecs, image_vecs, kt: int, ki: int, final_n: int, tau: float):
    from .index import fuse

    t = store._text_table.search_device(user_ids, _as_queries(text_vecs), kt)
    i = store._image_table.search_device(user_ids, _as_queries(image_vecs), ki)
    if t is None and i is None:
        return [([], True) for _ in user_ids]
    out = fuse(t, i, final_n, tau)
    comb, score = out["combined"].cpu().numpy(), out["score"].cpu().numpy()
    rows, mod, low = out["rows"].cpu().numpy(), out["modality"].cpu().numpy(), out["low_conf"].cpu().numpy()
    results = []
    for b in range(len(user_ids)):
        items = []
        for o in range(final_n):
            if rows[b, o] < 0:
                break
            coll = store._text_table if mod[b, o] == 0 else store._image_table
            items.append({"chunk_id": coll.chunk_id_of(int(rows[b, o])), "modality": "text" if mod[b, o] == 0 else "image",
                          "score": float(score[b, o]), "combined_score": float(comb[b, o])})
# ... 3 lines not shown
```

Measured before the change: 724.7.

## Add int8 shadow index with provable error bounds to prune exact bf16 rescoring

Builds an int8 quantized copy of the rows with per-row scale, error bound and norm. Small-batch searches (B<=2, k<=32) on a single-GPU index scan this shadow first, then rescore from bf16 only the rows whose upper bound can still enter the top-k. If that cannot be proven, the search falls back to the exact scan. The aim is to roughly halve the bytes streamed per query, at the cost of extra memory, shadow maintenance on every update, and a fallback path when the bounds are loose.

```diff
diff --git a/include/mmr_b200.h b/include/mmr_b200.h
--- a/include/mmr_b200.h
+++ b/include/mmr_b200.h
@@ -8,7 +8,7 @@
 extern "C" {
 #endif
 
-#define MMR_ABI_VERSION 2
+#define MMR_ABI_VERSION 3
 
 enum mmr_status {
   MMR_OK = 0,
@@ -45,6 +45,13 @@
 int mmr_index_set_query_precision(mmr_index* index, int mode);
 int mmr_index_update(mmr_index* index, int64_t n_rows, const void* rows_dev, const int64_t* seg_offsets_host,
                      int32_t n_segments);
+
+int mmr_index_attach_shadow(mmr_index* index, int8_t* q8_dev, float* side_dev, int64_t cap_rows, void* stream);
+int mmr_index_shadow_refresh(mmr_index* index, int64_t lo, int64_t hi, void* stream);
+int mmr_index_shadow_refresh_rows(mmr_index* index, const int64_t* rows_dev, int64_t n, void* stream);
+int mmr_index_shadow_stats(const mmr_index* index, int64_t* searches, int64_t* fallbacks);
+int mmr_debug_shadow_bounds(const mmr_index* index, const float* queries_dev, int32_t B, int64_t row_begin,
+                            int64_t row_end, float* out_bound_dev, float* out_score_dev, void* stream);
 
 int mmr_convert_rows_f32(const float* src_dev, void* dst_dev, int dtype, int64_t n_rows, int dim, int normalize,
                          void* stream);
diff --git a/multimodal-rag-for-image-text-search_b200/_native.py b/multimodal-rag-for-image-text-search_b200/_native.py
--- a/multimodal-rag-for-image-text-search_b200/_native.py
+++ b/multimodal-rag-for-image-text-search_b200/_native.py
@@ -10,7 +10,7 @@
 MMR_OK = 0
 MMR_BF16, MMR_F32, MMR_F16 = 0, 1, 2
 MMR_MAX_K = 64
-ABI_VERSION = 2
+ABI_VERSION = 3
 MMR_QP_AUTO, MMR_QP_F32, MMR_QP_RESCORE = 0, 1, 2
 
 _i32, _i64, _sz, _p, _f64 = C.c_int32, C.c_int64, C.c_size_t, C.c_void_p, C.c_double
@@ -53,6 +53,11 @@
     ("mmr_device_sm_count", C.c_int, [C.c_int, C.POINTER(C.c_int)]),
     ("mmr_last_kernel", C.c_int, []),
     ("mmr_rescore_reruns", _i64, []),
+    ("mmr_index_attach_shadow", C.c_int, [_p, _p, _p, _i64, _p]),
+    ("mmr_index_shadow_refresh", C.c_int, [_p, _i64, _i64, _p]),
+    ("mmr_index_shadow_refresh_rows", C.c_int, [_p, _p, _i64, _p]),
+    ("mmr_index_shadow_stats", C.c_int, [_p, C.POINTER(_i64), C.POINTER(_i64)]),
+    ("mmr_debug_shadow_bounds", C.c_int, [_p, _p, _i32, _i64, _i64, _p, _p, _p]),
 ]
 
 
diff --git a/multimodal-rag-for-image-text-search_b200/csrc/aux_kernels.cuh b/multimodal-rag-for-image-text-search_b200/csrc/aux_kernels.cuh
--- a/multimodal-rag-for-image-text-search_b200/csrc/aux_kernels.cuh
+++ b/multimodal-rag-for-image-text-search_b200/csrc/aux_kernels.cuh
@@ -1,4 +1,6 @@
 #pragma once
+#include <float.h>
+
 #include "common.cuh"
 #include "topk.cuh"
 
@@ -43,6 +45,71 @@
   }
 }
 
+template <typename E, int D>
+__global__ void shadow_quantize_kernel(const E* __restrict__ rows, int8_t* __restrict__ q8, float4* __restrict__ side,
+                                       int64_t lo, int64_t n, const int64_t* __restrict__ ids, int64_t cap) {
+  constexpr int EPL = D / 32;
+  const int lane = threadIdx.x & 31;
+  const int64_t warps = int64_t(gridDim.x) * (blockDim.x >> 5);
+  for (int64_t i = int64_t(blockIdx.x) * (blockDim.x >> 5) + (threadIdx.x >> 5); i < n; i += warps) {
+    const int64_t row = ids ? ids[i] : lo + i;
+    if (row < 0 || row >= cap) continue;
+    const E* src = rows + row * D;
+    int8_t* dst = q8 + row * D;
+    float x[EPL];
+    float m = 0.f;
+    bool nan = false;
+    double ss = 0.0;
+#pragma unroll
+    for (int j = 0; j < EPL; ++j) {
+      x[j] = float(src[j * 32 + lane]);
+      nan |= x[j] != x[j];
+      m = fmaxf(m, fabsf(x[j]));
+      ss += double(x[j]) * double(x[j]);
+    }
+    nan = __any_sync(0xffffffffu, nan);
+#pragma unroll
+    for (int o = 16; o > 0; o >>= 1) {
+      m = fmaxf(m, __shfl_xor_sync(0xffffffffu, m, o));
+      ss += __shfl_xor_sync(0xffffffffu, ss, o);
+    }
+    const double xnorm = sqrt(ss);
+    float4 rec = make_float4(0.f, 0.f, 0.f, 0.f);
+    if (nan) {
+      rec.x = __int_as_float(0x7fffffff);
+    } else if (!(m <= FLT_MAX) || xnorm > 1e37) {
+      rec.y = INFINITY;
+    } else if (m > 0.f) {
+      const float s = m / 127.f;
+      double ee = 0.0, nn = 0.0;
+#pragma unroll
+      for (int j = 0; j < EPL; ++j) {
+        const float v = fminf(fmaxf(rintf(x[j] / s), -127.f), 127.f);
+        dst[j * 32 + lane] = int8_t(v);
+        const double xt = double(s) * double(v);
+        const double d = double(x[j]) - xt;
+        ee += d * d;
+        nn += xt * xt;
+      }
+#pragma unroll
+      for (int o = 16; o > 0; o >>= 1) {
+        ee += __shfl_xor_sync(0xffffffffu, ee, o);
+        nn += __shfl_xor_sync(0xffffffffu, nn, o);
+      }
+      constexpr double up = 1.0 + 1e-9;
+      const double e = sqrt(ee) * up;
+      rec.x = s;
+      rec.y = __double2float_ru((e + 512.0 * 5.9604644775390625e-08 * xnorm) * up);
+      rec.z = __double2float_ru(sqrt(nn) * up);
+      if (lane == 0) side[row] = rec;
+      continue;
+    }
+#pragma unroll
+    for (int j = 0; j < EPL; ++j) dst[j * 32 + lane] = 0;
+    if (lane == 0) side[row] = rec;
+  }
+}
+
 template <int KPL>
 __global__ void merge_shards_kernel(const float* __restrict__ scores, const int64_t* __restrict__ rows,
                                     int64_t score_stride, int64_t row_stride, int G, int B, int k,
diff --git a/multimodal-rag-for-image-text-search_b200/csrc/common.cuh b/multimodal-rag-for-image-text-search_b200/csrc/common.cuh
--- a/multimodal-rag-for-image-text-search_b200/csrc/common.cuh
+++ b/multimodal-rag-for-image-text-search_b200/csrc/common.cuh
@@ -48,6 +48,7 @@
   int enc_narrow_tiles = 1;
   int inline_query = 1;
   int mailbox = 0;
+  int shadow = 1;
 };
 inline Options& options() {
   static Options o;
diff --git a/multimodal-rag-for-image-text-search_b200/csrc/mmr_b200.cu b/multimodal-rag-for-image-text-search_b200/csrc/mmr_b200.cu
--- a/multimodal-rag-for-image-text-search_b200/csrc/mmr_b200.cu
+++ b/multimodal-rag-for-image-text-search_b200/csrc/mmr_b200.cu
@@ -19,6 +19,7 @@
 
 #include "aux_kernels.cuh"
 #include "common.cuh"
+#include "scan_shadow.cuh"
 #include "scan_stream.cuh"
 #ifdef MMR_WITH_UMMA
 #include "scan_umma2.cuh"
@@ -65,6 +66,11 @@
   void* d_ws = nullptr;
   size_t ws_bytes = 0;
   int cap_b = 0, cap_k = 0;
+  const int8_t* sh_q8 = nullptr;
+  const float4* sh_side = nullptr;
+  int64_t sh_cap = 0;
+  int64_t sh_valid = 0;
+  unsigned long long* sh_stats = nullptr;
 #ifdef MMR_WITH_UMMA
   mutable UmmaIndexState umma;
   mutable Umma2IndexState umma2;
@@ -104,6 +110,7 @@
   if (!strcmp(name, "MMR_ENC_NARROW_TILES")) return &o.enc_narrow_tiles;
   if (!strcmp(name, "MMR_INLINE_QUERY")) return &o.inline_query;
   if (!strcmp(name, "MMR_MAILBOX")) return &o.mailbox;
+  if (!strcmp(name, "MMR_SHADOW")) return &o.shadow;
   return nullptr;
 }
 static int parse_option(const char* name, const char* v, int dflt) {
@@ -112,7 +119,7 @@
   return atoi(v);
 }
 static const char* kOptionNames[] = {"MMR_PDL", "MMR_UMMA_MODE", "MMR_UMMA_PAIR", "MMR_UMMA_NOPROBE", "MMR_FORCE_FAMILY",
-                                     "MMR_UMMA_LOCKSTEP", "MMR_INLINE_QUERY", "MMR_MAILBOX", "MMR_UMMA_SKIP_EPI", "MMR_UMMA_FUSED_PROBE", "MMR_ENC_FUSE_LN", "MMR_ENC_ATT_MMA", "MMR_ENC_GEMM_SMEM_KB", "MMR_UMMA_STAGES", "MMR_ENC_NARROW_TILES"};
+                                     "MMR_UMMA_LOCKSTEP", "MMR_INLINE_QUERY", "MMR_MAILBOX", "MMR_UMMA_SKIP_EPI", "MMR_UMMA_FUSED_PROBE", "MMR_ENC_FUSE_LN", "MMR_ENC_ATT_MMA", "MMR_ENC_GEMM_SMEM_KB", "MMR_UMMA_STAGES", "MMR_ENC_NARROW_TILES", "MMR_SHADOW"};
 namespace {
 struct OptionsFromEnv {
   OptionsFromEnv() {
@@ -189,6 +196,11 @@
   if (n_rows < 0 || n_rows >= (int64_t(1) << 32)) return fail(MMR_ERR_INVALID, "bad n_rows");
   if (n_rows > 0 && rows_dev == nullptr) return fail(MMR_ERR_INVALID, "rows_dev is NULL");
   if ((reinterpret_cast<uintptr_t>(rows_dev) & 15) != 0) return fail(MMR_ERR_INVALID, "rows_dev must be 16-byte aligned");
+  if (rows_dev != ix->rows) {
+    ix->sh_q8 = nullptr;
+    ix->sh_side = nullptr;
+    ix->sh_cap = ix->sh_valid = 0;
+  }
   ix->n_rows = n_rows;
   ix->rows = rows_dev;
 #ifdef MMR_WITH_UMMA
@@ -216,6 +228,7 @@
   if (!ix) return MMR_OK;
   cudaSetDevice(ix->device);
   free_staging(ix);
+  if (ix->sh_stats) cudaFree(ix->sh_stats);
   delete ix;
   return MMR_OK;
 }
@@ -225,6 +238,108 @@
   if (mode != MMR_QP_AUTO && mode != MMR_QP_F32 && mode != MMR_QP_RESCORE)
     return fail(MMR_ERR_INVALID, "unknown query precision %d", mode);
   ix->query_precision = mode;
+  return MMR_OK;
+}
+
+template <typename E, int D>
+static void launch_quantize_t(const mmr_index* ix, int64_t lo, int64_t n, const int64_t* ids, cudaStream_t st) {
+  const int64_t blocks = std::min<int64_t>((n + 7) / 8, int64_t(ix->sm_count) * 16);
+  shadow_quantize_kernel<E, D><<<(unsigned)blocks, 256, 0, st>>>(static_cast<const E*>(ix->rows), const_cast<int8_t*>(ix->sh_q8),
+                                                                  const_cast<float4*>(ix->sh_side), lo, n, ids, ix->sh_cap);
+}
+
+static int shadow_quantize(const mmr_index* ix, int64_t lo, int64_t n, const int64_t* ids_dev, cudaStream_t st) {
+  if (n <= 0) return MMR_OK;
+  CUDA_TRY(cudaSetDevice(ix->device));
+  const int key = ix->dtype * 1000 + ix->dim;
+  switch (key) {
+    case MMR_BF16 * 1000 + 512: launch_quantize_t<__nv_bfloat16, 512>(ix, lo, n, ids_dev, st); break;
+    case MMR_BF16 * 1000 + 384: launch_quantize_t<__nv_bfloat16, 384>(ix, lo, n, ids_dev, st); break;
+    case MMR_F16 * 1000 + 512: launch_quantize_t<__half, 512>(ix, lo, n, ids_dev, st); break;
+    case MMR_F16 * 1000 + 384: launch_quantize_t<__half, 384>(ix, lo, n, ids_dev, st); break;
+    default: return fail(MMR_ERR_UNSUPPORTED, "the shadow needs bf16 or fp16 rows");
+  }
+  g_launches++;
+  CUDA_TRY(cudaGetLastError());
+  CUDA_TRY(cudaStreamSynchronize(st));
+  return MMR_OK;
+}
+
+extern "C" int mmr_index_attach_shadow(mmr_index* ix, int8_t* q8_dev, float* side_dev, int64_t cap_rows, void* stream) {
+  if (!ix) return fail(MMR_ERR_INVALID, "index is NULL");
+  if (ix->dtype == MMR_F32) return fail(MMR_ERR_UNSUPPORTED, "the shadow needs bf16 or fp16 rows");
+  if (!q8_dev || !side_dev) return fail(MMR_ERR_INVALID, "NULL buffer");
+  if ((reinterpret_cast<uintptr_t>(q8_dev) & 15) != 0 || (reinterpret_cast<uintptr_t>(side_dev) & 15) != 0)
+    return fail(MMR_ERR_INVALID, "shadow buffers must be 16-byte aligned");
+  if (cap_rows < ix->n_rows || cap_rows >= (int64_t(1) << 32))
+    return fail(MMR_ERR_INVALID, "cap_rows %lld must cover the %lld rows of the index", (long long)cap_rows, (long long)ix->n_rows);
+  CUDA_TRY(cudaSetDevice(ix->device));
+  if (!ix->sh_stats) {
+    CUDA_TRY(cudaMalloc(&ix->sh_stats, 2 * sizeof(unsigned long long)));
+    CUDA_TRY(cudaMemset(ix->sh_stats, 0, 2 * sizeof(unsigned long long)));
+  }
+  ix->sh_q8 = q8_dev;
+  ix->sh_side = reinterpret_cast<const float4*>(side_dev);
+  ix->sh_cap = cap_rows;
+  ix->sh_valid = 0;
+  int rc = shadow_quantize(ix, 0, ix->n_rows, nullptr, static_cast<cudaStream_t>(stream));
+  if (rc != MMR_OK) return rc;
+  ix->sh_valid = ix->n_rows;
+  return MMR_OK;
+}
+
+extern "C" int mmr_index_shadow_refresh(mmr_index* ix, int64_t lo, int64_t hi, void* stream) {
+  if (!ix) return fail(MMR_ERR_INVALID, "index is NULL");
+  if (!ix->sh_q8) return fail(MMR_ERR_INVALID, "the index has no shadow");
+  if (lo < 0 || hi < lo || hi > ix->sh_cap) return fail(MMR_ERR_INVALID, "bad row range [%lld, %lld)", (long long)lo, (long long)hi);
+  int rc = shadow_quantize(ix, lo, hi - lo, nullptr, static_cast<cudaStream_t>(stream));
+  if (rc != MMR_OK) return rc;
+  if (lo <= ix->sh_valid) ix->sh_valid = std::max(ix->sh_valid, hi);
+  return MMR_OK;
+}
+
+extern "C" int mmr_index_shadow_refresh_rows(mmr_index* ix, const int64_t* rows_dev, int64_t n, void* stream) {
+  if (!ix) return fail(MMR_ERR_INVALID, "index is NULL");
+  if (!ix->sh_q8) return fail(MMR_ERR_INVALID, "the index has no shadow");
+  if (n < 0 || (n > 0 && !rows_dev)) return fail(MMR_ERR_INVALID, "bad row list");
+  return shadow_quantize(ix, 0, n, rows_dev, static_cast<cudaStream_t>(stream));
+}
+
+extern "C" int mmr_index_shadow_stats(const mmr_index* ix, int64_t* searches, int64_t* fallbacks) {
+  if (!ix || !searches || !fallbacks) return fail(MMR_ERR_INVALID, "NULL argument");
+  unsigned long long h[2] = {0ull, 0ull};
+  if (ix->sh_stats) {
+    CUDA_TRY(cudaSetDevice(ix->device));
+    CUDA_TRY(cudaMemcpy(h, ix->sh_stats, sizeof(h), cudaMemcpyDeviceToHost));
+  }
+  *searches = int64_t(h[0]);
+  *fallbacks = int64_t(h[1]);
+  return MMR_OK;
+}
+
+extern "C" int mmr_debug_shadow_bounds(const mmr_index* ix, const float* queries_dev, int32_t B, int64_t row_begin,
+                                       int64_t row_end, float* out_bound_dev, float* out_score_dev, void* stream) {
+  if (!ix || !queries_dev || !out_bound_dev || !out_score_dev) return fail(MMR_ERR_INVALID, "NULL argument");
+  if (!ix->sh_q8) return fail(MMR_ERR_INVALID, "the index has no shadow");
+  if (B <= 0 || B > 65535 || row_begin < 0 || row_end > ix->sh_valid || row_end <= row_begin)
+    return fail(MMR_ERR_INVALID, "bad range");
+  cudaStream_t st = static_cast<cudaStream_t>(stream);
+  const int64_t n = row_end - row_begin;
+  const dim3 grid(unsigned(std::min<int64_t>((n + 7) / 8, int64_t(ix->sm_count) * 16)), unsigned(B));
+  const int key = ix->dtype * 1000 + ix->dim;
+#define MMR_BOUNDS(E_, D_) \
+  shadow_bounds_kernel<E_, D_><<<grid, 256, 0, st>>>(ix->rows, ix->sh_q8, ix->sh_side, queries_dev, B, row_begin, row_end, \
+                                                      out_bound_dev, out_score_dev)
+  switch (key) {
+    case MMR_BF16 * 1000 + 512: MMR_BOUNDS(__nv_bfloat16, 512); break;
+    case MMR_BF16 * 1000 + 384: MMR_BOUNDS(__nv_bfloat16, 384); break;
+    case MMR_F16 * 1000 + 512: MMR_BOUNDS(__half, 512); break;
+    case MMR_F16 * 1000 + 384: MMR_BOUNDS(__half, 384); break;
+    default: return fail(MMR_ERR_UNSUPPORTED, "the shadow needs bf16 or fp16 rows");
+  }
+#undef MMR_BOUNDS
+  g_launches++;
+  CUDA_TRY(cudaGetLastError());
   return MMR_OK;
 }
 
@@ -437,7 +552,7 @@
 static size_t workspace_bytes_for(const mmr_index* ix, int32_t B, int32_t k, int64_t n_ranges) {
   if (!ix || B <= 0 || k <= 0) return 0;
   const size_t kk = size_t(std::min<int32_t>(k, MMR_MAX_K));
-  const size_t uniform = size_t(ix->sm_count) * 8 * kk * 8;
+  const size_t uniform = size_t(ix->sm_count) * std::max(8 * kk, size_t(2 * SHADOW_KC)) * 8;
   const size_t items = size_t(varlen_item_cap(ix, n_ranges));
   const size_t varlen = align_up(items * K1_ITEM_NQ * kk * 8, 256) + align_up(items * sizeof(ScanItem), 256) +
                         align_up(size_t(B) * sizeof(QuerySlot), 256);
@@ -695,9 +810,104 @@
 }
 #endif
 
+static constexpr size_t WS_PROVEN = 8;
+
+template <typename E, int D, int NQ>
+static int launch_shadow_t(const ShadowParams& p, int grid, cudaStream_t st) {
+  using C = ShadowCfg<D>;
+  static bool attr_set[64] = {};
+  int dev = 0;
+  cudaGetDevice(&dev);
+  if (dev >= 0 && dev < 64 && !attr_set[dev]) {
+    CUDA_TRY(cudaFuncSetAttribute(shadow_scan_kernel<E, D, NQ>, cudaFuncAttributeMaxDynamicSharedMemorySize, C::SMEM_BYTES));
+    attr_set[dev] = true;
+  }
+  cudaLaunchConfig_t cfg = {};
+  cfg.gridDim = dim3(grid);
+  cfg.blockDim = dim3(C::THREADS);
+  cfg.dynamicSmemBytes = C::SMEM_BYTES;
+  cfg.stream = st;
+  cudaLaunchAttribute attr[1];
+  attr[0].id = cudaLaunchAttributeProgrammaticStreamSerialization;
+  attr[0].val.programmaticStreamSerializationAllowed = options().pdl ? 1 : 0;
+  cfg.attrs = attr;
+  cfg.numAttrs = 1;
+  CUDA_TRY(cudaLaunchKernelEx(&cfg, shadow_scan_kernel<E, D, NQ>, p));
+  g_launches++;
+  return MMR_OK;
+}
+
+template <typename E, int D>
+static int launch_shadow_ed(const ShadowParams& p, int grid, cudaStream_t st) {
+  return p.nq == 1 ? launch_shadow_t<E, D, 1>(p, grid, st) : launch_shadow_t<E, D, 2>(p, grid, st);
+}
+
+static bool shadow_applies(const mmr_index* ix, int B, int k, uint32_t r0, uint32_t r1) {
+  return ix->sh_q8 != nullptr && options().shadow && B <= 2 && k <= 32 && ix->dtype != MMR_F32 &&
+         int64_t(r1) - r0 > SHADOW_KC && int64_t(r1) <= ix->sh_valid;
+}
+
+static int search_uniform_shadow(const mmr_index* ix, QuerySrc q, int B, int k, uint32_t r0, uint32_t r1, float* out_s,
+                                 int64_t* out_r, uint8_t* ws, cudaStream_t st) {
+  if (q.dev == nullptr && !(q.host && can_inline(ix, B))) return fail(MMR_ERR_INVALID, "queries must be device-resident for this batch size");
+  ShadowParams p;
+  memset(&p, 0, offsetof(ShadowParams, qinline));
+  p.rows = ix->rows;
+  p.q8 = ix->sh_q8;
+  p.side = ix->sh_side;
+  p.queries = q.dev;
+  if (q.dev == nullptr) memcpy(p.qinline, q.host, size_t(B) * ix->dim * sizeof(float));
+  p.nq = B;
+  p.k = k;
+  p.row_begin = r0;
+  p.row_end = r1;
+  p.partial = reinterpret_cast<uint64_t*>(ws + WS_CTRL);
+  p.ticket = reinterpret_cast<unsigned int*>(ws);
+  p.proven = reinterpret_cast<unsigned int*>(ws + WS_PROVEN);
+  p.stats = ix->sh_stats;
+  p.out_scores = out_s;
+  p.out_rows = out_r;
+  p.row_base = ix->row_base;
+  const int64_t nchunks = (int64_t(r1) - r0 + MMR_SHADOW_ROWS - 1) / MMR_SHADOW_ROWS;
+  const int grid = int(std::min<int64_t>(ix->sm_count, std::max<int64_t>(1, (nchunks + 7) / 8)));
+  int rc = MMR_ERR_UNSUPPORTED;
+  const int key = ix->dtype * 1000 + ix->dim;
+  switch (key) {
+    case MMR_BF16 * 1000 + 512: rc = launch_shadow_ed<__nv_bfloat16, 512>(p, grid, st); break;
+    case MMR_BF16 * 1000 + 384: rc = launch_shadow_ed<__nv_bfloat16, 384>(p, grid, st); break;
+    case MMR_F16 * 1000 + 512: rc = launch_shadow_ed<__half, 512>(p, grid, st); break;
+    case MMR_F16 * 1000 + 384: rc = launch_shadow_ed<__half, 384>(p, grid, st); break;
+    default: return fail(MMR_ERR_UNSUPPORTED, "no shadow kernel for dtype %d dim %d", ix->dtype, ix->dim);
+  }
+  if (rc != MMR_OK) return rc;
+  StreamParams g;
+  memset(&g, 0, offsetof(StreamParams, qinline));
+  g.rows = ix->rows;
+  g.queries = q.dev;
+  if (q.dev == nullptr) memcpy(g.qinline, q.host, size_t(B) * ix->dim * sizeof(float));
+  g.nq = B;
+  g.k = k;
+  g.row_begin = r0;
+  g.row_end = r1;
+  g.partial = p.partial;
+  g.ticket = p.ticket;
+  g.out_scores = out_s;
+  g.out_rows = out_r;
+  g.row_base = ix->row_base;
+  g.skip_if = p.proven;
+  const int64_t k1_chunks = (int64_t(r1) - r0 + MMR_K1_ROWS - 1) / MMR_K1_ROWS;
+  const int k1_grid = int(std::min<int64_t>(ix->sm_count, std::max<int64_t>(1, (k1_chunks + K1_NW - 1) / K1_NW)));
+  rc = launch_stream(ix, g, B, 1, k1_grid, st);
+  if (rc != MMR_OK) return rc;
+  g_last_kernel = 4;
+  return MMR_OK;
+}
+
 static int search_uniform(const mmr_index* ix, QuerySrc q, int B, int k, uint32_t r0, uint32_t r1, float* out_s,
                           int64_t* out_r, uint8_t* ws, size_t ws_total, cudaStream_t st, const ExchangeInfo* xi = nullptr,
                           Completion* done = nullptr) {
+  if (xi == nullptr && shadow_applies(ix, B, k, r0, r1))
+    return search_uniform_shadow(ix, q, B, k, r0, r1, out_s, out_r, ws, st);
 #ifdef MMR_WITH_UMMA
   if (q.dev != nullptr && ix->query_precision != MMR_QP_F32 &&
       umma_preferred(ix->dtype, ix->dim, B, k, int64_t(r1) - r0)) {
@@ -893,7 +1103,7 @@
   if (uniform && can_inline(ix, B) && !uniform_takes_k2(ix, B, k, int64_t(r1) - r0)) {
     QuerySrc q;
     q.host = queries_host;
-    rc = search_uniform_stream(ix, q, B, k, r0, r1, box_s, box_r, static_cast<uint8_t*>(ix->d_ws), st, nullptr, &done);
+    rc = search_uniform(ix, q, B, k, r0, r1, box_s, box_r, static_cast<uint8_t*>(ix->d_ws), ix->ws_bytes, st, nullptr, &done);
   } else {
     memcpy(ix->h_q, queries_host, size_t(B) * ix->dim * 4);
     CUDA_TRY(cudaMemcpyAsync(ix->d_q, ix->h_q, size_t(B) * ix->dim * 4, cudaMemcpyHostToDevice, st));
diff --git a/multimodal-rag-for-image-text-search_b200/csrc/scan_shadow.cuh b/multimodal-rag-for-image-text-search_b200/csrc/scan_shadow.cuh
--- /dev/null
+++ b/multimodal-rag-for-image-text-search_b200/csrc/scan_shadow.cuh
@@ -0,0 +1,385 @@
+#pragma once
+#include <float.h>
+
+#include "common.cuh"
+#include "scan_stream.cuh"
+#include "topk.cuh"
+
+namespace mmr {
+
+constexpr int SHADOW_KC = 64;
+
+#ifndef MMR_SHADOW_ROWS
+#define MMR_SHADOW_ROWS 8
+#endif
+#ifndef MMR_SHADOW_STAGES
+#define MMR_SHADOW_STAGES 2
+#endif
+
+struct ShadowParams {
+  const void* rows;
+  const int8_t* q8;
+  const float4* side;
+  const float* queries;
+  int32_t nq;
+  int32_t k;
+  uint32_t row_begin, row_end;
+  uint64_t* partial;
+  unsigned int* ticket;
+  unsigned int* proven;
+  unsigned long long* stats;
+  float* out_scores;
+  int64_t* out_rows;
+  int64_t row_base;
+  float qinline[K1_INLINE_FLOATS];
+};
+
+template <int D>
+struct ShadowCfg {
+  static constexpr int R = MMR_SHADOW_ROWS;
+  static constexpr int NW = 8;
+  static constexpr int S = MMR_SHADOW_STAGES;
+  static constexpr int THREADS = NW * 32;
+  static constexpr int SIDE_OFF = R * D;
+  static constexpr int STAGE_BYTES = R * D + R * 16;
+  static constexpr int VECB = (D % 512 == 0) ? 16 : 4;
+  static constexpr int NV = D / (32 * VECB);
+  static constexpr int RPV = VECB / 4;
+  static constexpr int WPL = D / 128;
+  static constexpr int RING_BYTES = NW * S * STAGE_BYTES;
+  static constexpr int SMEM_BYTES = RING_BYTES + NW * S * 8 + 64;
+  static_assert(D % 128 == 0, "int8 rows are read as 32-bit words, 32 lanes wide");
+  static_assert(int64_t(D) * 127 * 32767 < (int64_t(1) << 31), "the int32 row sum could overflow");
+  static_assert(STAGE_BYTES % 16 == 0, "bulk copies move multiples of 16 bytes");
+};
+
+__device__ __forceinline__ void lds_u32(uint32_t addr, uint32_t& r) {
+  asm volatile("ld.shared.u32 %0, [%1];" : "=r"(r) : "r"(addr));
+}
+__device__ __forceinline__ float4 lds_f4(uint32_t addr) {
+  float4 v;
+  asm volatile("ld.shared.v4.f32 {%0,%1,%2,%3}, [%4];" : "=f"(v.x), "=f"(v.y), "=f"(v.z), "=f"(v.w) : "r"(addr));
+  return v;
+}
+
+template <typename E, int D>
+__device__ __forceinline__ void shadow_query(const float* __restrict__ qsrc, int lane, uint32_t (&qlo)[D / 128],
+                                             uint32_t (&qhi)[D / 128], float& s_q, float& e_q, float& nq) {
+  using C = ShadowCfg<D>;
+  float qk[D / 32];
+  const float nrm = k1_load_unit_query<E, D>(qsrc, lane, qk);
+  float qh[C::WPL * 4];
+  float m = 0.f;
+  bool bad = false;
+#pragma unroll
+  for (int w = 0; w < C::WPL; ++w)
+#pragma unroll
+    for (int b = 0; b < 4; ++b) {
+      const int t = w / C::RPV, j = w % C::RPV;
+      const int e = t * 32 * C::VECB + lane * C::VECB + 4 * j + b;
+      const float x = qsrc[e];
+      const float v = nrm > 0.f ? x / nrm : x;
+      qh[w * 4 + b] = v;
+      m = fmaxf(m, fabsf(v));
+      bad |= v != v;
+    }
+#pragma unroll
+  for (int o = 16; o > 0; o >>= 1) m = fmaxf(m, __shfl_xor_sync(0xffffffffu, m, o));
+  bad = __any_sync(0xffffffffu, bad) || !(m <= FLT_MAX);
+  s_q = bad ? __int_as_float(0x7fffffff) : m / 32767.f;
+  float ssd = 0.f, ssq = 0.f;
+#pragma unroll
+  for (int w = 0; w < C::WPL; ++w) {
+    int qi[4];
+#pragma unroll
+    for (int b = 0; b < 4; ++b) {
+      const float x = qh[w * 4 + b];
+      const float v = (s_q > 0.f) ? fminf(fmaxf(rintf(x / s_q), -32767.f), 32767.f) : 0.f;
+      qi[b] = int(v);
+      const float d = fmaf(-s_q, v, x);
+      ssd = fmaf(d, d, ssd);
+      ssq = fmaf(x, x, ssq);
+    }
+    qlo[w] = (uint32_t(qi[0]) & 0xFFFFu) | (uint32_t(qi[1]) << 16);
+    qhi[w] = (uint32_t(qi[2]) & 0xFFFFu) | (uint32_t(qi[3]) << 16);
+  }
+  ssd = warp_allreduce_sum(ssd);
+  ssq = warp_allreduce_sum(ssq);
+  e_q = __fsqrt_ru(__fmaf_ru(ssd, 1.001f, 1e-30f));
+  nq = __fsqrt_ru(__fmaf_ru(ssq, 1.001f, 1e-30f));
+}
+
+__device__ __forceinline__ float shadow_bound(int I, float4 sd, float s_q, float e_q, float nq) {
+  const float a = (sd.x * s_q) * __int2float_rn(I);
+  float slack = __fmaf_ru(2.3841858e-07f, fabsf(a), 1e-25f);
+  slack = __fmaf_ru(sd.z, e_q, slack);
+  slack = __fmaf_ru(sd.y, nq, slack);
+  return __fadd_ru(a, slack);
+}
+
+template <int D>
+__device__ __forceinline__ int shadow_row_dot(const int8_t* __restrict__ row, const uint32_t (&qlo)[D / 128],
+                                              const uint32_t (&qhi)[D / 128], int lane) {
+  using C = ShadowCfg<D>;
+  int acc = 0;
+#pragma unroll
+  for (int w = 0; w < C::WPL; ++w) {
+    const int t = w / C::RPV, j = w % C::RPV;
+    const uint32_t x = *reinterpret_cast<const uint32_t*>(row + t * 32 * C::VECB + lane * C::VECB + 4 * j);
+    acc = __dp2a_lo(int(qlo[w]), int(x), acc);
+    acc = __dp2a_hi(int(qhi[w]), int(x), acc);
+  }
+#pragma unroll
+  for (int o = 16; o > 0; o >>= 1) acc += __shfl_xor_sync(0xffffffffu, acc, o);
+  return acc;
+}
+
+template <typename E, int D, int NQ>
+__global__ void __launch_bounds__(ShadowCfg<D>::THREADS, 1) shadow_scan_kernel(const __grid_constant__ ShadowParams p) {
+  using C = ShadowCfg<D>;
+  constexpr int KPL = SHADOW_KC / 32;
+  extern __shared__ __align__(1024) uint8_t smem[];
+  uint64_t* bars = reinterpret_cast<uint64_t*>(smem + C::RING_BYTES);
+  __shared__ int s_last;
+  __shared__ uint64_t s_cand[NQ][SHADOW_KC];
+  __shared__ uint64_t s_resc[SHADOW_KC];
+  __shared__ unsigned int s_proven;
+
+  const int lane = threadIdx.x & 31;
+  const int warp = threadIdx.x >> 5;
+  asm volatile("griddepcontrol.launch_dependents;" ::: "memory");
+
+  const uint32_t ring0 = smem_u32(smem) + uint32_t(warp) * (C::S * C::STAGE_BYTES);
+  const uint32_t bar0 = smem_u32(bars) + uint32_t(warp) * (C::S * 8);
+  if (lane == 0) {
+#pragma unroll
+    for (int s = 0; s < C::S; ++s) mbar_init(bar0 + s * 8, 1);
+    fence_mbar_init();
+  }
+  __syncwarp();
+
+  const float* qbase = p.queries ? p.queries : p.qinline;
+  uint32_t qlo[NQ][C::WPL], qhi[NQ][C::WPL];
+  float s_q[NQ], e_q[NQ], n_q[NQ];
+#pragma unroll
+  for (int qi = 0; qi < NQ; ++qi)
+    shadow_query<E, D>(qbase + size_t(qi < p.nq ? qi : 0) * D, lane, qlo[qi], qhi[qi], s_q[qi], e_q[qi], n_q[qi]);
+
+  WarpTopK<KPL> list[NQ];
+  uint64_t thr[NQ];
+#pragma unroll
+  for (int qi = 0; qi < NQ; ++qi) {
+    list[qi].clear();
+    thr[qi] = 0ull;
+  }
+
+  const int first = blockIdx.x * C::NW + warp;
+  const int stride = gridDim.x * C::NW;
+  const uint32_t row_begin = p.row_begin, row_end = p.row_end;
+  const int nchunks = int((row_end - row_begin + C::R - 1) / C::R);
+  const uint8_t* q8 = reinterpret_cast<const uint8_t*>(p.q8);
+  auto issue = [&](int c, int s) {
+    const uint32_t r0 = row_begin + uint32_t(c) * C::R;
+    const uint32_t nr = min(uint32_t(C::R), row_end - r0);
+    const uint32_t bar = bar0 + s * 8;
+    mbar_arrive_expect_tx(bar, nr * (D + 16));
+    bulk_g2s(ring0 + s * C::STAGE_BYTES, q8 + size_t(r0) * D, nr * D, bar);
+    bulk_g2s(ring0 + s * C::STAGE_BYTES + C::SIDE_OFF, p.side + r0, nr * 16, bar);
+  };
+  int stage = 0;
+  uint32_t phase = 0;
+  if (lane == 0) {
+#pragma unroll
+    for (int j = 0; j < C::S; ++j) {
+      const int c = first + j * stride;
+      if (c < nchunks) issue(c, j);
+    }
+  }
+  constexpr int V = C::R * NQ;
+  constexpr int LPV = 32 / V;
+  const int vi = lane / LPV;
+  const int my_r = vi / NQ, myq = vi % NQ;
+  const float my_sq = NQ == 1 ? s_q[0] : (myq == 0 ? s_q[0] : s_q[NQ - 1]);
+  const float my_eq = NQ == 1 ? e_q[0] : (myq == 0 ? e_q[0] : e_q[NQ - 1]);
+  const float my_nq = NQ == 1 ? n_q[0] : (myq == 0 ? n_q[0] : n_q[NQ - 1]);
+  for (int c = first; c < nchunks; c += stride) {
+    const int s = stage;
+    mbar_wait(bar0 + s * 8, phase);
+    const uint32_t sbase = ring0 + s * C::STAGE_BYTES;
+    int acc[V];
+#pragma unroll
+    for (int i = 0; i < V; ++i) acc[i] = 0;
+#pragma unroll
+    for (int r = 0; r < C::R; ++r) {
+#pragma unroll
+      for (int t = 0; t < C::NV; ++t) {
+        uint32_t w[C::RPV];
+        const uint32_t addr = sbase + r * D + t * (32 * C::VECB) + lane * C::VECB;
+        if constexpr (C::VECB == 16) lds_v4(addr, reinterpret_cast<uint32_t(&)[4]>(w));
+        else lds_u32(addr, w[0]);
+#pragma unroll
+        for (int j = 0; j < C::RPV; ++j)
+#pragma unroll
+          for (int qi = 0; qi < NQ; ++qi) {
+            acc[r * NQ + qi] = __dp2a_lo(int(qlo[qi][t * C::RPV + j]), int(w[j]), acc[r * NQ + qi]);
+            acc[r * NQ + qi] = __dp2a_hi(int(qhi[qi][t * C::RPV + j]), int(w[j]), acc[r * NQ + qi]);
+          }
+      }
+    }
+    const float4 sd = lds_f4(sbase + C::SIDE_OFF + my_r * 16);
+    __syncwarp();
+    if (lane == 0) {
+      const int cn = c + C::S * stride;
+      if (cn < nchunks) {
+        fence_proxy_async();
+        issue(cn, s);
+      }
+    }
+    const int I = transpose_reduce<V>(acc, lane);
+    const uint32_t row = row_begin + uint32_t(c) * C::R + uint32_t(my_r);
+    const float u = shadow_bound(I, sd, my_sq, my_eq, my_nq);
+    const bool owner = (lane % LPV == 0) && row < row_end && u == u;
+    const uint64_t key = make_key(u, row);
+#pragma unroll
+    for (int qi = 0; qi < NQ; ++qi)
+      if (qi < p.nq) thr[qi] = list[qi].offer(key, owner && myq == qi, thr[qi], SHADOW_KC, lane);
+    if (++stage == C::S) {
+      stage = 0;
+      phase ^= 1u;
+    }
+  }
+
+  asm volatile("griddepcontrol.wait;" ::: "memory");
+  __syncthreads();
+  constexpr int KSLOTS = SHADOW_KC;
+  uint64_t* wk = reinterpret_cast<uint64_t*>(smem);
+#pragma unroll
+  for (int qi = 0; qi < NQ; ++qi)
+#pragma unroll
+    for (int j = 0; j < KPL; ++j) wk[(warp * NQ + qi) * KSLOTS + j * 32 + lane] = list[qi].key[j];
+  __syncthreads();
+  if (warp < p.nq) {
+    const int qi = warp;
+    WarpTopK<KPL> m;
+    m.clear();
+    uint64_t t = 0ull;
+    t = m.template merge_batched<4>(
+        [&](int i) -> uint64_t { return wk[((i % C::NW) * NQ + qi) * KSLOTS + i / C::NW]; }, C::NW * SHADOW_KC, t,
+        SHADOW_KC, lane);
+    m.store(p.partial + (size_t(blockIdx.x) * NQ + qi) * SHADOW_KC, SHADOW_KC, lane);
+  }
+  __threadfence();
+  __syncthreads();
+  if (threadIdx.x == 0) s_last = (atomicAdd(p.ticket, 1u) == gridDim.x - 1);
+  __syncthreads();
+  if (!s_last) return;
+  __threadfence();
+  const int nparts = gridDim.x;
+  for (int qi = 0; qi < p.nq; ++qi) {
+    WarpTopK<KPL> m;
+    m.clear();
+    uint64_t t = 0ull;
+    const int nmine = (nparts - warp + C::NW - 1) / C::NW;
+    t = m.template merge_batched<8>(
+        [&](int i) -> uint64_t {
+          const int pos = i / nmine, part = warp + (i % nmine) * C::NW;
+          return __ldcg(reinterpret_cast<const unsigned long long*>(p.partial) + (size_t(part) * NQ + qi) * SHADOW_KC + pos);
+        },
+        nmine * SHADOW_KC, t, SHADOW_KC, lane);
+    __syncthreads();
+#pragma unroll
+    for (int j = 0; j < KPL; ++j) wk[warp * KSLOTS + j * 32 + lane] = m.key[j];
+    __syncthreads();
+    if (warp == 0) {
+      WarpTopK<KPL> f;
+      f.clear();
+      uint64_t tf = 0ull;
+      tf = f.template merge_batched<4>([&](int i) -> uint64_t { return wk[(i % C::NW) * KSLOTS + i / C::NW]; },
+                                       C::NW * SHADOW_KC, tf, SHADOW_KC, lane);
+#pragma unroll
+      for (int j = 0; j < KPL; ++j) s_cand[qi][j * 32 + lane] = f.key[j];
+    }
+  }
+  if (threadIdx.x == 0) {
+    s_proven = 1u;
+    *p.ticket = 0u;
+  }
+  __syncthreads();
+
+  const int k = p.k;
+  const uint8_t* rows8 = reinterpret_cast<const uint8_t*>(p.rows);
+  constexpr int PER_WARP = SHADOW_KC / C::NW;
+  for (int qi = 0; qi < p.nq; ++qi) {
+    float qk[D / 32];
+    k1_load_unit_query<E, D>(qbase + size_t(qi) * D, lane, qk);
+    uint32_t w[PER_WARP][k1_row_words<E, D>()];
+#pragma unroll
+    for (int i = 0; i < PER_WARP; ++i) {
+      const uint64_t key = s_cand[qi][warp + i * C::NW];
+      if (key) k1_row_load<E, D>(rows8 + size_t(key_row(key)) * (D * sizeof(E)), lane, w[i]);
+    }
+#pragma unroll
+    for (int i = 0; i < PER_WARP; ++i) {
+      const int c = warp + i * C::NW;
+      const uint64_t key = s_cand[qi][c];
+      uint64_t rk = 0ull;
+      if (key) {
+        const float sc = k1_row_dot<E, D>(w[i], qk, lane);
+        if (sc == sc) rk = make_key(sc, key_row(key));
+      }
+      if (lane == 0) s_resc[c] = rk;
+    }
+    __syncthreads();
+    if (warp == 0) {
+      WarpTopK<1> m;
+      m.clear();
+      uint64_t kth = 0ull;
+      kth = m.template merge_batched<2>([&](int i) -> uint64_t { return s_resc[i]; }, SHADOW_KC, kth, k, lane);
+      if (lane < k) {
+        const uint64_t key = m.key[0];
+        const size_t o = size_t(qi) * k + lane;
+        p.out_scores[o] = key ? key_score(key) : -INFINITY;
+        p.out_rows[o] = key ? int64_t(key_row(key)) + p.row_base : int64_t(-1);
+      }
+      if (lane == 0) {
+        const uint64_t last = s_cand[qi][SHADOW_KC - 1];
+        const bool ok = kth != 0ull && (last == 0ull || key_score(kth) > key_score(last));
+        if (!ok) s_proven = 0u;
+      }
+    }
+    __syncthreads();
+  }
+  if (threadIdx.x == 0) {
+    *p.proven = s_proven;
+    atomicAdd(p.stats, 1ull);
+    if (!s_proven) atomicAdd(p.stats + 1, 1ull);
+  }
+}
+
+template <typename E, int D>
+__global__ void shadow_bounds_kernel(const void* __restrict__ rows, const int8_t* __restrict__ q8,
+                                     const float4* __restrict__ side, const float* __restrict__ queries, int B,
+                                     int64_t row_begin, int64_t row_end, float* __restrict__ out_u,
+                                     float* __restrict__ out_s) {
+  const int lane = threadIdx.x & 31;
+  const int b = blockIdx.y;
+  uint32_t qlo[D / 128], qhi[D / 128];
+  float s_q, e_q, nq;
+  shadow_query<E, D>(queries + size_t(b) * D, lane, qlo, qhi, s_q, e_q, nq);
+  float qk[D / 32];
+  k1_load_unit_query<E, D>(queries + size_t(b) * D, lane, qk);
+  const int64_t n = row_end - row_begin;
+  const int64_t warps = int64_t(gridDim.x) * (blockDim.x >> 5);
+  for (int64_t i = int64_t(blockIdx.x) * (blockDim.x >> 5) + (threadIdx.x >> 5); i < n; i += warps) {
+    const int64_t row = row_begin + i;
+    const int I = shadow_row_dot<D>(q8 + row * D, qlo, qhi, lane);
+    const float u = shadow_bound(I, side[row], s_q, e_q, nq);
+    const float sc = k1_row_score<E, D>(reinterpret_cast<const uint8_t*>(rows) + row * (D * sizeof(E)), qk, lane);
+    if (lane == 0) {
+      out_u[size_t(b) * n + i] = u;
+      out_s[size_t(b) * n + i] = sc;
+    }
+  }
+}
+
+}
diff --git a/multimodal-rag-for-image-text-search_b200/csrc/scan_stream.cuh b/multimodal-rag-for-image-text-search_b200/csrc/scan_stream.cuh
--- a/multimodal-rag-for-image-text-search_b200/csrc/scan_stream.cuh
+++ b/multimodal-rag-for-image-text-search_b200/csrc/scan_stream.cuh
@@ -66,6 +66,7 @@
   uint64_t peer_flag[MMR_MAX_PEERS];
   uint32_t* done_flag;
   uint32_t done_seq;
+  const unsigned int* skip_if;
   float qinline[K1_INLINE_FLOATS];
 };
 
@@ -94,16 +95,16 @@
   static constexpr int BYTES = 4;
 };
 
-template <int N, int OFF>
-__device__ __forceinline__ void transpose_reduce_step(float* v, int lane) {
+template <int N, int OFF, typename T>
+__device__ __forceinline__ void transpose_reduce_step(T* v, int lane) {
   if constexpr (OFF >= 1) {
     if constexpr (N > 1) {
       constexpr int H = N / 2;
       const bool upper = (lane & OFF) != 0;
 #pragma unroll
       for (int i = 0; i < H; ++i) {
-        const float send = upper ? v[i] : v[i + H];
-        const float keep = upper ? v[i + H] : v[i];
+        const T send = upper ? v[i] : v[i + H];
+        const T keep = upper ? v[i + H] : v[i];
         v[i] = keep + __shfl_xor_sync(0xffffffffu, send, OFF);
       }
       transpose_reduce_step<H, OFF / 2>(v, lane);
@@ -113,8 +114,8 @@
     }
   }
 }
-template <int V>
-__device__ __forceinline__ float transpose_reduce(float (&v)[V], int lane) {
+template <int V, typename T>
+__device__ __forceinline__ T transpose_reduce(T (&v)[V], int lane) {
   static_assert(V >= 1 && V <= 32 && (V & (V - 1)) == 0, "V must be a power of two <= 32");
   transpose_reduce_step<V, 16>(v, lane);
   return v[0];
@@ -158,6 +159,10 @@
   const int k = p.k;
 
   asm volatile("griddepcontrol.launch_dependents;" ::: "memory");
+  if (p.skip_if != nullptr) {
+    asm volatile("griddepcontrol.wait;" ::: "memory");
+    if (*reinterpret_cast<const volatile unsigned int*>(p.skip_if) != 0u) return;
+  }
   if (p.items != nullptr) asm volatile("griddepcontrol.wait;" ::: "memory");
 
   const uint32_t ring0 = smem_u32(smem) + uint32_t(warp) * (C::S * C::STAGE_BYTES);
@@ -437,7 +442,7 @@
 }
 
 template <typename E, int D>
-__device__ __forceinline__ void k1_load_unit_query(const float* __restrict__ qsrc, int lane, float (&q)[D / 32]) {
+__device__ __forceinline__ float k1_load_unit_query(const float* __restrict__ qsrc, int lane, float (&q)[D / 32]) {
   using C = StreamCfg<E, D, 1, 1>;
   float ss = 0.f;
 #pragma unroll
@@ -454,38 +459,56 @@
 #pragma unroll
     for (int e = 0; e < C::EPL; ++e) q[e] = q[e] / nrm;
   }
+  return nrm;
 }
 
 template <typename E, int D>
-__device__ __forceinline__ float k1_row_score(const uint8_t* __restrict__ row, const float (&q)[D / 32], int lane) {
+__host__ __device__ constexpr int k1_row_words() { return StreamCfg<E, D, 1, 1>::NV * StreamCfg<E, D, 1, 1>::RPV; }
+
+template <typename E, int D>
+__device__ __forceinline__ void k1_row_load(const uint8_t* __restrict__ row, int lane, uint32_t (&w)[k1_row_words<E, D>()]) {
   using C = StreamCfg<E, D, 1, 1>;
-  float acc = 0.f;
 #pragma unroll
   for (int t = 0; t < C::NV; ++t) {
-    uint32_t w[C::RPV];
     const uint8_t* src = row + lane * C::VECB + t * (32 * C::VECB);
     if constexpr (C::VECB == 16) {
       const uint4 v = __ldg(reinterpret_cast<const uint4*>(src));
-      w[0] = v.x; w[1] = v.y; w[2] = v.z; w[3] = v.w;
+      w[t * 4 + 0] = v.x; w[t * 4 + 1] = v.y; w[t * 4 + 2] = v.z; w[t * 4 + 3] = v.w;
     } else {
       const uint2 v = __ldg(reinterpret_cast<const uint2*>(src));
-      w[0] = v.x; w[1] = v.y;
-    }
+      w[t * 2 + 0] = v.x; w[t * 2 + 1] = v.y;
+    }
+  }
+}
+
+template <typename E, int D>
+__device__ __forceinline__ float k1_row_dot(const uint32_t (&w)[k1_row_words<E, D>()], const float (&q)[D / 32], int lane) {
+  using C = StreamCfg<E, D, 1, 1>;
+  float acc = 0.f;
+#pragma unroll
+  for (int t = 0; t < C::NV; ++t) {
 #pragma unroll
     for (int j = 0; j < C::RPV; ++j) {
       if constexpr (C::EB == 2) {
         float a, b;
-        ElemTraits<E>::unpack(w[j], a, b);
+        ElemTraits<E>::unpack(w[t * C::RPV + j], a, b);
         acc = fmaf(a, q[(t * C::RPV + j) * 2 + 0], acc);
         acc = fmaf(b, q[(t * C::RPV + j) * 2 + 1], acc);
       } else {
-        acc = fmaf(__uint_as_float(w[j]), q[t * C::RPV + j], acc);
+        acc = fmaf(__uint_as_float(w[t * C::RPV + j]), q[t * C::RPV + j], acc);
       }
     }
   }
 #pragma unroll
   for (int o = 16; o > 0; o >>= 1) acc += __shfl_xor_sync(0xffffffffu, acc, o);
   return acc;
+}
+
+template <typename E, int D>
+__device__ __forceinline__ float k1_row_score(const uint8_t* __restrict__ row, const float (&q)[D / 32], int lane) {
+  uint32_t w[k1_row_words<E, D>()];
+  k1_row_load<E, D>(row, lane, w);
+  return k1_row_dot<E, D>(w, q, lane);
 }
 
 template <typename E, int D, int KPL>
diff --git a/multimodal-rag-for-image-text-search_b200/index.py b/multimodal-rag-for-image-text-search_b200/index.py
--- a/multimodal-rag-for-image-text-search_b200/index.py
+++ b/multimodal-rag-for-image-text-search_b200/index.py
@@ -43,6 +43,7 @@
         self._ws: Optional[torch.Tensor] = None
         self._one: dict = {}
         self._ws_key = (0, 0, 0)
+        self._shadow: Optional[Tuple[torch.Tensor, torch.Tensor]] = None
         lib = N.lib()
         nseg = 0 if self.seg_offsets is None else len(self.seg_offsets) - 1
         segp = None if self.seg_offsets is None else self.seg_offsets.ctypes.data
@@ -108,8 +109,50 @@
         self.seg_offsets = None if seg_offsets is None else np.ascontiguousarray(seg_offsets, dtype=np.int64)
         nseg = 0 if self.seg_offsets is None else len(self.seg_offsets) - 1
         segp = None if self.seg_offsets is None else self.seg_offsets.ctypes.data
+        if rows.data_ptr() != self.rows.data_ptr():
+            self._shadow = None
         N.check(N.lib().mmr_index_update(self._handle, n, rows.data_ptr() if n else None, segp, nseg))
         self.rows, self.n_rows = rows, n
+
+    def enable_shadow(self, capacity_rows: Optional[int] = None) -> None:
+        cap = int(self.rows.shape[0]) if capacity_rows is None else int(capacity_rows)
+        if cap > int(self.rows.shape[0]):
+            raise ValueError("capacity_rows exceeds the rows buffer")
+        q8 = torch.empty((max(cap, 1), self.dim), dtype=torch.int8, device=self.device)
+        side = torch.empty((max(cap, 1), 4), dtype=torch.float32, device=self.device)
+        with torch.cuda.device(self.device):
+            N.check(N.lib().mmr_index_attach_shadow(self._handle, q8.data_ptr(), side.data_ptr(), cap,
+                                                    _stream_ptr(self.device)))
+        self._shadow = (q8, side)
+
+    def rows_written(self, lo: int, hi: int) -> None:
+        if self._shadow is not None and hi > lo:
+            with torch.cuda.device(self.device):
+                N.check(N.lib().mmr_index_shadow_refresh(self._handle, int(lo), int(hi), _stream_ptr(self.device)))
+
+    def rows_written_at(self, idx) -> None:
+        if self._shadow is None:
+            return
+        ids = torch.as_tensor(idx, dtype=torch.int64).to(self.device).contiguous()
+        if ids.numel():
+            with torch.cuda.device(self.device):
+                N.check(N.lib().mmr_index_shadow_refresh_rows(self._handle, ids.data_ptr(), ids.numel(),
+                                                              _stream_ptr(self.device)))
+
+    def shadow_stats(self) -> Tuple[int, int]:
+        a, b = C.c_int64(), C.c_int64()
+        N.check(N.lib().mmr_index_shadow_stats(self._handle, C.byref(a), C.byref(b)))
+        return int(a.value), int(b.value)
+
+    def debug_shadow_bounds(self, queries: torch.Tensor, row_begin: int, row_end: int) -> Tuple[torch.Tensor, torch.Tensor]:
+        q = queries.reshape(-1, self.dim).to(device=self.device, dtype=torch.float32).contiguous()
+        b, n = int(q.shape[0]), int(row_end - row_begin)
+        u = torch.empty((b, n), dtype=torch.float32, device=self.device)
+        sc = torch.empty((b, n), dtype=torch.float32, device=self.device)
+        with torch.cuda.device(self.device):
+            N.check(N.lib().mmr_debug_shadow_bounds(self._handle, q.data_ptr(), b, int(row_begin), int(row_end), u.data_ptr(),
+                                                    sc.data_ptr(), _stream_ptr(self.device)))
+        return u, sc
 
     def search_ranges(self, queries: torch.Tensor, k: int, ranges) -> Tuple[torch.Tensor, torch.Tensor]:
         if queries.dim() == 1:
diff --git a/multimodal-rag-for-image-text-search_b200/store.py b/multimodal-rag-for-image-text-search_b200/store.py
--- a/multimodal-rag-for-image-text-search_b200/store.py
+++ b/multimodal-rag-for-image-text-search_b200/store.py
@@ -244,6 +244,8 @@
             sh.set_query_precision(self.query_precision)
             self._shards.append(sh)
         self._resident = self._shards[-1]
+        if G == 1 and self.dtype != "f32" and hasattr(self._resident, "enable_shadow"):
+            self._resident.enable_shadow(cap)
         self._multi = MultiIndex(self._shards) if G > 1 else None
         self._ranges = {host.tenants[i]: [[int(seg[i]), int(seg[i + 1])]] for i in range(len(host.tenants)) if counts[i]}
         self.rebuilds += 1
@@ -260,6 +262,8 @@
             for g in np.unique(which):
                 idx = torch.as_tensor(tomb[which == g] - self._bounds[int(g)], dtype=torch.int64, device=self._bufs[int(g)].device)
                 self._bufs[int(g)].index_fill_(0, idx, float("nan"))
+                if G == 1 and hasattr(self._resident, "rows_written_at"):
+                    self._resident.rows_written_at(idx)
             self._tomb += len(self._pending_tomb)
             self._pending_tomb = []
         rows = self._pending_rows()
@@ -271,6 +275,8 @@
             m = int(rows.size)
             lo = self._n_res
             ResidentIndex.load_rows_into(self._buf, self.host.gather(rows), dst_offset=lo - self._bounds[-2])
+            if len(self._bufs) == 1 and hasattr(self._resident, "rows_written"):
+                self._resident.rows_written(lo, lo + m)
             self._perm[lo:lo + m] = rows
             self._res_of[rows] = lo + np.arange(m, dtype=np.int64)
             cuts = np.nonzero(np.diff(tenant))[0] + 1
```

Measured after the change: 1278 (median of 6 runs). 1.76x the previous value.
